# MartinErhardt/RoaringRegex

Hardware: AMD Instinct MI355X
Metric: GB/s input scanned (whole job), 256-state regex (higher is better)
Workload: dtype u32

## Files before the change

include/rrx.h:

```cpp
#ifndef RRX_H
#define RRX_H
#include <stddef.h>
#include <stdint.h>
#ifdef __cplusplus
extern "C" {
#endif

typedef struct rrx_regex rrx_regex;
typedef struct rrx_corpus rrx_corpus;

enum { RRX_OK = 0, RRX_ERR_PATTERN = 1, RRX_ERR_ARG = 2, RRX_ERR_HIP = 3, RRX_ERR_UNSUPPORTED = 4 };

enum { RRX_ENGINE_AUTO = 0, RRX_ENGINE_NFA = 1, RRX_ENGINE_DFA = 2, RRX_ENGINE_DFA_GLOBAL = 3 ,
       RRX_ENGINE_NFA_WAVE = 4 ,
       RRX_ENGINE_DFA2 = 5 ,
       RRX_ENGINE_NFA_BLOCK = 8 ,
       RRX_ENGINE_NFA_SPARSE = 10  };

int rrx_compile(const char *pattern, rrx_regex **out);
int rrx_compile_ex(const char *pattern, int engine, rrx_regex **out);
void rrx_free(rrx_regex *re);
const char *rrx_last_error(void);

uint32_t rrx_num_states(const rrx_regex *re);
int      rrx_set_class(const rrx_regex *re);
uint32_t rrx_ref_initial(const rrx_regex *re);
int      rrx_ref_is_final(const rrx_regex *re, uint32_t state);
uint32_t rrx_ref_row(const rrx_regex *re, uint32_t state, unsigned c, uint32_t *out, uint32_t cap);

int         rrx_engine(const rrx_regex *re);
const char *rrx_engine_name(const rrx_regex *re);
uint32_t    rrx_useful_states(const rrx_regex *re);
uint32_t    rrx_byte_classes(const rrx_regex *re);
int         rrx_table_order(const rrx_regex *re, double *conflict_before, double *conflict_after);
int         rrx_order_table(rrx_regex *re, const void *sample, uint32_t lanes, uint32_t bytes_per_lane);
enum { RRX_OPT_BACKGROUND_ORDER = 1, RRX_OPT_UNITS_PER_WORKGROUP = 2, RRX_OPT_SAMPLED_TABLE = 3, RRX_OPT_FLUSH_SLOTS = 4, RRX_OPT_SEARCH_ANCHORED = 5,
       RRX_OPT_ITEMS_STRIDE2 = 6 };
int         rrx_set_option(rrx_regex *re, int option, int64_t value);
int         rrx_learn_table(rrx_regex *re, const void *text, size_t nbytes);
int         rrx_sampled_table(const rrx_regex *re, uint32_t *table_states, uint32_t *open_transitions);
int         rrx_sampled_escapes(const rrx_regex *re, int device, uint64_t *lines);
uint32_t    rrx_words_per_set(const rrx_regex *re);
int         rrx_accepts_empty(const rrx_regex *re);
#define RRX_PROGRAM_SEARCH_FWD 6
#define RRX_PROGRAM_SEARCH_REV 7
#define RRX_PROGRAM_DFA2_ORDER 11
#define RRX_PROGRAM_SEARCH_LINE 9
#define RRX_PROGRAM_SEARCH_LINE2 14
#define RRX_PROGRAM_SAMPLED_DFA 12
#define RRX_PROGRAM_SAMPLED_DFA2 13
#define RRX_PROGRAM_DFA2_ITEMS 15
#define RRX_PROGRAM_CONTAINS_DFA 16
#define RRX_PROGRAM_CONTAINS_DFA2 17
#define RRX_PROGRAM_CONTAINS_DFA2_ITEMS 18
size_t rrx_program_words(const rrx_regex *re, int kind, uint32_t *out, size_t cap);

int    rrx_corpus_create(int device, const void *d_bytes, size_t nbytes, void *stream, rrx_corpus **out);
int    rrx_corpus_create_ex(int device, const void *d_bytes, size_t nbytes, uint32_t stripe_bytes, void *stream,
                            rrx_corpus **out);
uint32_t rrx_corpus_stripe_bytes(const rrx_corpus *c);
size_t rrx_corpus_num_lines(const rrx_corpus *c);
size_t rrx_corpus_num_bytes(const rrx_corpus *c);
void   rrx_corpus_free(rrx_corpus *c);
size_t rrx_corpus_bitmap_words(const rrx_corpus *c);
int rrx_match_corpus(const rrx_regex *re, const rrx_corpus *c, uint32_t *d_accept_bits, void *stream);
int rrx_match_device(const rrx_regex *re, int device, const void *d_bytes, size_t nbytes, uint32_t *d_accept_bits,
                     size_t cap_words, size_t *nlines, void *stream);
int rrx_bitmap_to_bytes(int device, const uint32_t *d_accept_bits, size_t nlines, uint8_t *d_accept, void *stream);

int rrx_search_corpus(const rrx_regex *re, const rrx_corpus *corpus, uint32_t *d_start, uint32_t *d_end, void *stream);
int         rrx_contains_corpus(const rrx_regex *re, const rrx_corpus *c, uint32_t *d_bits, void *stream);
const char *rrx_contains_engine_name(const rrx_regex *re);
uint32_t    rrx_contains_states(const rrx_regex *re);
int         rrx_bitmap_count(int device, const uint32_t *d_bits, size_t nlines, uint64_t *d_count, void *stream);
int rrx_search_all_count(const rrx_regex *re, const rrx_corpus *corpus, uint32_t *d_count, void *stream);
int rrx_search_all_fill(const rrx_regex *re, const rrx_corpus *corpus, const uint64_t *d_first, uint32_t *d_start,
                        uint32_t *d_end, void *stream);

int rrx_search_all(const rrx_regex *re, const rrx_corpus *corpus, uint64_t *d_first, uint32_t *d_start, uint32_t *d_end,
                   size_t cap, size_t *total, void *stream);

int rrx_match_extents(const rrx_regex *re, int device, const void *d_bytes, const uint64_t *d_off, size_t nitems,
                      uint32_t trim, uint8_t *d_accept, void *stream);

typedef struct rrx_items rrx_items;
int rrx_items_create(int device, const void *d_bytes, const uint64_t *d_off, size_t nitems, uint32_t trim, void *stream,
                     rrx_items **out);
size_t rrx_items_count(const rrx_items *items);
int rrx_items_stripe_wise(const rrx_items *items);
void rrx_items_free(rrx_items *items);
int rrx_match_items(const rrx_regex *re, const rrx_items *items, uint8_t *d_accept, void *stream);

int rrx_contains_extents(const rrx_regex *re, int device, const void *d_bytes, const uint64_t *d_off, size_t nitems, uint32_t trim,
                         uint32_t *d_bits, void *stream);
int rrx_contains_items(const rrx_regex *re, const rrx_items *items, uint32_t *d_bits, void *stream);

int rrx_match_string(const rrx_regex *re, int device, const void *d_bytes, size_t nbytes, uint8_t *d_accept, void *stream);

int rrx_match_host(const rrx_regex *re, int device, const void *bytes, size_t nbytes, uint8_t *accept, size_t cap,
                   size_t *nlines);
int rrx_match_cstr(const rrx_regex *re, int device, const char *text, int *accepted, size_t *len);

#ifdef __cplusplus
}
#endif
#endif
```

roaringregex_amd/__init__.py:

```python
import ctypes as C
import os

_HERE = os.path.dirname(os.path.abspath(__file__))
_SO = os.environ.get("RRX_LIB") or os.path.join(_HERE, "librrx.so")

ENGINE_AUTO, ENGINE_NFA, ENGINE_DFA, ENGINE_DFA_GLOBAL, ENGINE_NFA_WAVE, ENGINE_DFA2 = 0, 1, 2, 3, 4, 5
PROGRAM_SEARCH_FWD, PROGRAM_SEARCH_REV = 6, 7
ENGINE_NFA_BLOCK = 8
ENGINE_NFA_SPARSE = 10
PROGRAM_SEARCH_LINE = 9
PROGRAM_SEARCH_LINE2 = 14
PROGRAM_DFA2_ITEMS = 15
PROGRAM_DFA2_ORDER = 11
PROGRAM_SAMPLED_DFA = 12
PROGRAM_SAMPLED_DFA2 = 13
PROGRAM_CONTAINS_DFA, PROGRAM_CONTAINS_DFA2 = 16, 17
PROGRAM_CONTAINS_DFA2_ITEMS = 18
OPT_BACKGROUND_ORDER = 1
OPT_UNITS_PER_WORKGROUP = 2
OPT_SAMPLED_TABLE = 3
OPT_FLUSH_SLOTS = 4
OPT_SEARCH_ANCHORED = 5
OPT_ITEMS_STRIDE2 = 6

ABI_SYMBOLS = (
    "rrx_compile", "rrx_compile_ex", "rrx_free", "rrx_last_error",
    "rrx_num_states", "rrx_set_class", "rrx_ref_initial", "rrx_ref_is_final", "rrx_ref_row",
    "rrx_engine", "rrx_engine_name", "rrx_useful_states", "rrx_byte_classes", "rrx_table_order", "rrx_order_table", "rrx_set_option", "rrx_learn_table", "rrx_sampled_table", "rrx_sampled_escapes", "rrx_words_per_set", "rrx_accepts_empty",
    "rrx_program_words",
    "rrx_corpus_create", "rrx_corpus_create_ex", "rrx_corpus_stripe_bytes", "rrx_corpus_num_lines", "rrx_corpus_num_bytes", "rrx_corpus_free", "rrx_corpus_bitmap_words",
    "rrx_match_corpus", "rrx_match_device", "rrx_search_corpus", "rrx_search_all_count", "rrx_search_all_fill", "rrx_search_all", "rrx_bitmap_to_bytes",
    "rrx_match_extents", "rrx_items_create", "rrx_items_count", "rrx_items_stripe_wise", "rrx_items_free", "rrx_match_items",
    "rrx_match_string", "rrx_match_host", "rrx_match_cstr",
    "rrx_contains_corpus", "rrx_contains_engine_name", "rrx_contains_states", "rrx_bitmap_count",
    "rrx_contains_extents", "rrx_contains_items",
)


class RRegexError(RuntimeError):
    """The reference throws std::runtime_error (Parser.cpp:36,155); so do we."""


def _load():
    if not os.path.exists(_SO):
        raise ImportError(
            "roaringregex_amd: %s is missing — build it with `python -c 'import __graft_entry__ as g; g.build()'` "
            "(hipcc --offload-arch=gfx950).  There is no CPU fallback." % _SO)
    try:
        import torch
    except ImportError:
        pass
    L = C.CDLL(_SO)
    vp, u32, sz, i32 = C.c_void_p, C.c_uint32, C.c_size_t, C.c_int
    sig = {
        "rrx_compile": (i32, [C.c_char_p, C.POINTER(vp)]),
        "rrx_compile_ex": (i32, [C.c_char_p, i32, C.POINTER(vp)]),
        "rrx_free": (None, [vp]),
        "rrx_last_error": (C.c_char_p, []),
        "rrx_num_states": (u32, [vp]),
        "rrx_set_class": (i32, [vp]),
        "rrx_ref_initial": (u32, [vp]),
        "rrx_ref_is_final": (i32, [vp, u32]),
        "rrx_ref_row": (u32, [vp, u32, C.c_uint, vp, u32]),
        "rrx_engine": (i32, [vp]),
        "rrx_engine_name": (C.c_char_p, [vp]),
        "rrx_useful_states": (u32, [vp]),
        "rrx_byte_classes": (u32, [vp]),
        "rrx_table_order": (i32, [vp, C.POINTER(C.c_double), C.POINTER(C.c_double)]),
        "rrx_set_option": (i32, [vp, i32, C.c_int64]),
        "rrx_learn_table": (i32, [vp, vp, C.c_size_t]),
        "rrx_sampled_table": (i32, [vp, C.POINTER(C.c_uint32), C.POINTER(C.c_uint32)]),
        "rrx_sampled_escapes": (i32, [vp, i32, C.POINTER(C.c_uint64)]),
        "rrx_order_table": (i32, [vp, vp, u32, u32]),
        "rrx_words_per_set": (u32, [vp]),
        "rrx_accepts_empty": (i32, [vp]),
        "rrx_program_words": (sz, [vp, i32, vp, sz]),
        "rrx_corpus_create": (i32, [i32, vp, sz, vp, C.POINTER(vp)]),
        "rrx_corpus_create_ex": (i32, [i32, vp, sz, u32, vp, C.POINTER(vp)]),
        "rrx_corpus_stripe_bytes": (u32, [vp]),
        "rrx_corpus_num_lines": (sz, [vp]),
        "rrx_corpus_num_bytes": (sz, [vp]),
        "rrx_corpus_free": (None, [vp]),
        "rrx_corpus_bitmap_words": (sz, [vp]),
        "rrx_match_corpus": (i32, [vp, vp, vp, vp]),
        "rrx_match_device": (i32, [vp, i32, vp, sz, vp, sz, C.POINTER(sz), vp]),
        "rrx_bitmap_to_bytes": (i32, [i32, vp, sz, vp, vp]),
        "rrx_match_extents": (i32, [vp, i32, vp, vp, sz, u32, vp, vp]),
        "rrx_items_create": (i32, [i32, vp, vp, sz, u32, vp, C.POINTER(vp)]),
        "rrx_items_count": (sz, [vp]),
        "rrx_items_stripe_wise": (i32, [vp]),
        "rrx_items_free": (None, [vp]),
        "rrx_match_items": (i32, [vp, vp, vp, vp]),
        "rrx_match_string": (i32, [vp, i32, vp, sz, vp, vp]),
        "rrx_search_corpus": (i32, [vp, vp, vp, vp, vp]),
        "rrx_search_all_count": (i32, [vp, vp, vp, vp]),
        "rrx_search_all_fill": (i32, [vp, vp, vp, vp, vp, vp]),
        "rrx_search_all": (i32, [vp, vp, vp, vp, vp, sz, C.POINTER(sz), vp]),
        "rrx_match_host": (i32, [vp, i32, vp, sz, vp, sz, C.POINTER(sz)]),
        "rrx_match_cstr": (i32, [vp, i32, C.c_char_p, C.POINTER(i32), C.POINTER(sz)]),
        "rrx_contains_corpus": (i32, [vp, vp, vp, vp]),
        "rrx_contains_engine_name": (C.c_char_p, [vp]),
        "rrx_contains_states": (u32, [vp]),
        "rrx_bitmap_count": (i32, [i32, vp, sz, vp, vp]),
        "rrx_contains_extents": (i32, [vp, i32, vp, vp, sz, u32, vp, vp]),
        "rrx_contains_items": (i32, [vp, vp, vp, vp]),
    }
    for name, (res, args) in sig.items():
        f = getattr(L, name)
        f.restype, f.argtypes = res, args
    return L


_L = _load()


def _check(rc):
    if rc != 0:
        raise RRegexError(_L.rrx_last_error().decode("latin-1"))


class _on:

    def __init__(self, device, stream):
        import torch
        self._dev = torch.cuda.device(device)
        self._st = torch.cuda.stream(stream) if stream is not None else None

    def __enter__(self):
        self._dev.__enter__()
        if self._st is not None:
            self._st.__enter__()

    def __exit__(self, *exc):
        if self._st is not None:
            self._st.__exit__(*exc)
        return self._dev.__exit__(*exc)


def _stream_ptr(stream):
    if stream is None:
        import torch
        stream = torch.cuda.current_stream()
    return C.c_void_p(stream.cuda_stream)


def bitmap_count(bits, nlines, stream=None):
    import torch
    assert bits.is_cuda and bits.dtype in (torch.int32, torch.uint32) and bits.is_contiguous() and bits.numel() * 32 >= nlines
    with _on(bits.device.index, stream):
        count = torch.empty(1, dtype=torch.int64, device=bits.device)
        _check(_L.rrx_bitmap_count(bits.device.index, C.c_void_p(bits.data_ptr() if nlines else 0), nlines, C.c_void_p(count.data_ptr()),
                                   _stream_ptr(stream)))
        return int(count.item())


class Match:

    def __init__(self, buf, start, end):
        self._buf, self.start, self.end = buf, start, end

    def str(self):
        return self._buf[self.start:self.end]


class IteratorWrapper:

    def __init__(self, regex, text, device):
        self._re, self._text, self._device = regex, text, device
        self._consumed = False
        self._accepted = None

    def advance(self):
        if not self._consumed:
            acc, n = C.c_int(0), C.c_size_t(0)
            _check(_L.rrx_match_cstr(self._re._h, self._device, self._text, C.byref(acc), C.byref(n)))
            self._accepted, self._len = bool(acc.value), n.value
            self._consumed = True
        return self

    def value(self):
        if not self._consumed:
            return Match(self._text, 0, 0) if self._re.accepts_empty else None
        return Match(self._text, 0, self._len) if self._accepted else None

    def create_copy(self):
        c = IteratorWrapper(self._re, self._text, self._device)
        c.__dict__.update(self.__dict__)
        return c


class Corpus:

    def __init__(self, data, device=None, stream=None, stripe=0):
        import torch
        if isinstance(data, (bytes, bytearray, memoryview)):
            data = torch.frombuffer(bytearray(data), dtype=torch.uint8) if len(data) else torch.empty(0, dtype=torch.uint8)
        if not data.is_cuda:
            dev = torch.device("cuda", 0 if device is None else device)
            data = data.to(dev)
        assert data.dtype == torch.uint8 and data.is_contiguous()
        self.data = data
        self.device = data.device.index
        self._h = C.c_void_p()
        with _on(self.device, stream):
            _check(_L.rrx_corpus_create_ex(self.device, C.c_void_p(data.data_ptr() if data.numel() else 0), data.numel(),
                                           stripe, _stream_ptr(stream), C.byref(self._h)))

    def __del__(self):
        if getattr(self, "_h", None) and _L is not None:
            _L.rrx_corpus_free(self._h)
            self._h = None

    @property
    def num_lines(self):
        return _L.rrx_corpus_num_lines(self._h)

    @property
    def num_bytes(self):
        return _L.rrx_corpus_num_bytes(self._h)

    @property
    def stripe(self):
        return _L.rrx_corpus_stripe_bytes(self._h)


class Items:

    def __init__(self, data, offsets, trim=0, stream=None):
        import torch
        assert data.is_cuda and data.dtype == torch.uint8 and data.is_contiguous()
        assert offsets.is_cuda and offsets.dtype in (torch.int64, torch.uint64) and offsets.is_contiguous() and offsets.numel() >= 1
        self.data, self.offsets, self.trim = data, offsets, trim
        self.device = data.device.index
        self._h = C.c_void_p()
        with _on(self.device, stream):
            _check(_L.rrx_items_create(self.device, C.c_void_p(data.data_ptr() if data.numel() else 0), C.c_void_p(offsets.data_ptr()),
                                       offsets.numel() - 1, trim, _stream_ptr(stream), C.byref(self._h)))

    def __del__(self):
        if getattr(self, "_h", None) and _L is not None:
            _L.rrx_items_free(self._h)
            self._h = None

    @property
    def num_items(self):
        return _L.rrx_items_count(self._h)

    @property
    def stripe_wise(self):
        return bool(_L.rrx_items_stripe_wise(self._h))


class RRegex:

    def __init__(self, pattern, engine=ENGINE_AUTO, device=0):
        if isinstance(pattern, str):
            pattern = pattern.encode("latin-1")
        self.pattern = pattern
        self.device = device
        self._h = C.c_void_p()
        _check(_L.rrx_compile_ex(pattern, engine, C.byref(self._h)))

    def __del__(self):
        if getattr(self, "_h", None) and _L is not None:
            _L.rrx_free(self._h)
            self._h = None

    def get_acceptance_iter(self, text):
        if isinstance(text, str):
            text = text.encode("latin-1")
        return IteratorWrapper(self, text, self.device)

    def match_corpus_bits(self, corpus, out=None, stream=None):
        import torch
        nw = _L.rrx_corpus_bitmap_words(corpus._h)
        with _on(corpus.device, stream):
            if out is None:
                out = torch.empty(nw, dtype=torch.int32, device=corpus.data.device)
            assert out.is_cuda and out.dtype == torch.int32 and out.numel() >= nw
            _check(_L.rrx_match_corpus(self._h, corpus._h, C.c_void_p(out.data_ptr() if nw else 0), _stream_ptr(stream)))
        return out[:nw]

    def match_device_bits(self, data, cap_lines=None, out=None, stream=None):
        import torch
        assert data.is_cuda and data.dtype == torch.uint8 and data.is_contiguous()
        n = data.numel()
        if cap_lines is None:
            cap_lines = n + 1
        cap_words = (cap_lines + 31) // 32
        with _on(data.device.index, stream):
            if out is None:
                out = torch.empty(cap_words, dtype=torch.int32, device=data.device)
            assert out.is_cuda and out.dtype == torch.int32 and out.numel() >= cap_words
            nlines = C.c_size_t(0)
            _check(_L.rrx_match_device(self._h, data.device.index, C.c_void_p(data.data_ptr() if n else 0), n,
                                       C.c_void_p(out.data_ptr()), cap_words, C.byref(nlines), _stream_ptr(stream)))
        return out[:(nlines.value + 31) // 32], nlines.value

    def match_corpus(self, corpus, out=None, stream=None):
        import torch
        n = corpus.num_lines
        with _on(corpus.device, stream):
            bits = self.match_corpus_bits(corpus, stream=stream)
            if out is None:
                out = torch.empty(n, dtype=torch.uint8, device=corpus.data.device)
            assert out.is_cuda and out.dtype == torch.uint8 and out.numel() >= n
            _check(_L.rrx_bitmap_to_bytes(corpus.device, C.c_void_p(bits.data_ptr() if n else 0), n,
                                          C.c_void_p(out.data_ptr() if n else 0), _stream_ptr(stream)))
        return out[:n]

    def contains_corpus_bits(self, corpus, out=None, stream=None):
        import torch
        nw = _L.rrx_corpus_bitmap_words(corpus._h)
        with _on(corpus.device, stream):
            if out is None:
                out = torch.empty(nw, dtype=torch.int32, device=corpus.data.device)
            assert out.is_cuda and out.dtype == torch.int32 and out.numel() >= nw
            _check(_L.rrx_contains_corpus(self._h, corpus._h, C.c_void_p(out.data_ptr() if nw else 0), _stream_ptr(stream)))
        return out[:nw]

    def contains_corpus(self, corpus, out=None, stream=None):
        import torch
        n = corpus.num_lines
        with _on(corpus.device, stream):
            bits = self.contains_corpus_bits(corpus, stream=stream)
            if out is None:
                out = torch.empty(n, dtype=torch.uint8, device=corpus.data.device)
            assert out.is_cuda and out.dtype == torch.uint8 and out.numel() >= n
            _check(_L.rrx_bitmap_to_bytes(corpus.device, C.c_void_p(bits.data_ptr() if n else 0), n,
                                          C.c_void_p(out.data_ptr() if n else 0), _stream_ptr(stream)))
        return out[:n]

    def search_corpus(self, corpus, stream=None):
        import torch
        n = corpus.num_lines
        with _on(corpus.device, stream):
            start = torch.empty(n, dtype=torch.int32, device=corpus.data.device)
            end = torch.empty(n, dtype=torch.int32, device=corpus.data.device)
            _check(_L.rrx_search_corpus(self._h, corpus._h, C.c_void_p(start.data_ptr() if n else 0), C.c_void_p(end.data_ptr() if n else 0),
                                        _stream_ptr(stream)))
        return start, end

    def search_all(self, corpus, stream=None):
        import torch
        n = corpus.num_lines
        dev = corpus.data.device
        with _on(corpus.device, stream):
            count = torch.zeros(n, dtype=torch.int32, device=dev)
            _check(_L.rrx_search_all_count(self._h, corpus._h, C.c_void_p(count.data_ptr() if n else 0), _stream_ptr(stream)))
            inclusive = torch.cumsum(count, dim=0, dtype=torch.int64)
            first = inclusive - count
            total = int(inclusive[-1].item()) if n else 0
            start = torch.empty(total, dtype=torch.int32, device=dev)
            end = torch.empty(total, dtype=torch.int32, device=dev)
            if total:
                _check(_L.rrx_search_all_fill(self._h, corpus._h, C.c_void_p(first.data_ptr()), C.c_void_p(start.data_ptr() if total else 0),
                                              C.c_void_p(end.data_ptr() if total else 0), _stream_ptr(stream)))
        return count, first, start, end

    def search_all_fused(self, corpus, cap=None, stream=None):
        import torch
        n = corpus.num_lines
        dev = corpus.data.device
        with _on(corpus.device, stream):
            first = torch.empty(n + 1, dtype=torch.int64, device=dev)
            cap = int(cap) if cap is not None else 2 * n + 1024
            while True:
                start = torch.empty(cap, dtype=torch.int32, device=dev)
                end = torch.empty(cap, dtype=torch.int32, device=dev)
                total = C.c_size_t(0)
                _check(_L.rrx_search_all(self._h, corpus._h, C.c_void_p(first.data_ptr()), C.c_void_p(start.data_ptr() if cap else 0),
                                         C.c_void_p(end.data_ptr() if cap else 0), cap, C.byref(total), _stream_ptr(stream)))
                if total.value <= cap:
                    break
                cap = total.value
        return first, start[:total.value], end[:total.value]

    def match_items(self, items, out=None, stream=None):
        import torch
        n = items.num_items
        with _on(items.device, stream):
            if out is None:
                out = torch.empty(n, dtype=torch.uint8, device=items.data.device)
            assert out.is_cuda and out.dtype == torch.uint8 and out.numel() >= n
            _check(_L.rrx_match_items(self._h, items._h, C.c_void_p(out.data_ptr() if n else 0), _stream_ptr(stream)))
        return out[:n]

    def match_extents(self, data, offsets, trim=0, out=None, stream=None):
        import torch
        n = offsets.numel() - 1
        assert data.is_cuda and offsets.is_cuda and offsets.dtype in (torch.int64, torch.uint64)
        with _on(data.device.index, stream):
            if out is None:
                out = torch.empty(n, dtype=torch.uint8, device=data.device)
            _check(_L.rrx_match_extents(self._h, data.device.index, C.c_void_p(data.data_ptr() if data.numel() else 0),
                                        C.c_void_p(offsets.data_ptr()), n, trim, C.c_void_p(out.data_ptr() if n else 0),
                                        _stream_ptr(stream)))
        return out[:n]

    def contains_items_bits(self, items, out=None, stream=None):
        import torch
        n = items.num_items
        nw = (n + 31) // 32
        with _on(items.device, stream):
            if out is None:
                out = torch.empty(nw, dtype=torch.int32, device=items.data.device)
            assert out.is_cuda and out.dtype == torch.int32 and out.is_contiguous() and out.numel() >= nw
            _check(_L.rrx_contains_items(self._h, items._h, C.c_void_p(out.data_ptr() if nw else 0), _stream_ptr(stream)))
        return out[:nw]

    def contains_items(self, items, out=None, stream=None):
        import torch
        n = items.num_items
        with _on(items.device, stream):
            bits = self.contains_items_bits(items, stream=stream)
            if out is None:
                out = torch.empty(n, dtype=torch.uint8, device=items.data.device)
            assert out.is_cuda and out.dtype == torch.uint8 and out.numel() >= n
            _check(_L.rrx_bitmap_to_bytes(items.device, C.c_void_p(bits.data_ptr() if n else 0), n,
                                          C.c_void_p(out.data_ptr() if n else 0), _stream_ptr(stream)))
        return out[:n]

    def contains_extents_bits(self, data, offsets, trim=0, out=None, stream=None):
        import torch
        n = offsets.numel() - 1
        nw = (n + 31) // 32
        assert data.is_cuda and offsets.is_cuda and offsets.dtype in (torch.int64, torch.uint64) and offsets.is_contiguous()
        with _on(data.device.index, stream):
            if out is None:
                out = torch.empty(nw, dtype=torch.int32, device=data.device)
            assert out.is_cuda and out.dtype == torch.int32 and out.is_contiguous() and out.numel() >= nw
            _check(_L.rrx_contains_extents(self._h, data.device.index, C.c_void_p(data.data_ptr() if data.numel() else 0),
                                           C.c_void_p(offsets.data_ptr()), n, trim, C.c_void_p(out.data_ptr() if nw else 0),
                                           _stream_ptr(stream)))
        return out[:nw]

    def contains_extents(self, data, offsets, trim=0, out=None, stream=None):
        import torch
        n = offsets.numel() - 1
        with _on(data.device.index, stream):
            bits = self.contains_extents_bits(data, offsets, trim=trim, stream=stream)
            if out is None:
                out = torch.empty(n, dtype=torch.uint8, device=data.device)
            assert out.is_cuda and out.dtype == torch.uint8 and out.numel() >= n
            _check(_L.rrx_bitmap_to_bytes(data.device.index, C.c_void_p(bits.data_ptr() if n else 0), n,
                                          C.c_void_p(out.data_ptr() if n else 0), _stream_ptr(stream)))
        return out[:n]

    def match_string(self, data, stream=None):
        import torch
        assert data.is_cuda and data.dtype == torch.uint8
        with _on(data.device.index, stream):
            out = torch.zeros(1, dtype=torch.uint8, device=data.device)
            _check(_L.rrx_match_string(self._h, data.device.index, C.c_void_p(data.data_ptr() if data.numel() else 0), data.numel(),
                                       C.c_void_p(out.data_ptr()), _stream_ptr(stream)))
        return bool(out.item())

    def match_host(self, data):
        import numpy as np
        a = np.frombuffer(data, dtype=np.uint8) if not isinstance(data, np.ndarray) else np.ascontiguousarray(data, dtype=np.uint8)
        cap = len(a) + 1
        out = np.empty(cap, dtype=np.uint8)
        n = C.c_size_t(0)
        _check(_L.rrx_match_host(self._h, self.device, C.c_void_p(a.ctypes.data if len(a) else 0), len(a),
                                 C.c_void_p(out.ctypes.data), cap, C.byref(n)))
        return out[:n.value]

    @property
    def states_n(self):
        return _L.rrx_num_states(self._h)

    @property
    def set_class(self):
        return _L.rrx_set_class(self._h)

    @property
    def initial(self):
        return _L.rrx_ref_initial(self._h)

    def finals(self):
        return [s for s in range(self.states_n) if _L.rrx_ref_is_final(self._h, s)]

    def row(self, state, c):
        n = self.states_n
        buf = (C.c_uint32 * max(n, 1))()
        k = _L.rrx_ref_row(self._h, state, c, buf, n)
        return list(buf[:k])

    @property
    def engine(self):
        return _L.rrx_engine(self._h)

    @property
    def engine_name(self):
        return _L.rrx_engine_name(self._h).decode()

    @property
    def contains_engine_name(self):
        name = _L.rrx_contains_engine_name(self._h)
        if name is None:
            raise RRegexError(_L.rrx_last_error().decode("latin-1"))
        return name.decode()

    @property
    def contains_states(self):
        return _L.rrx_contains_states(self._h)

    @property
    def useful_states(self):
        return _L.rrx_useful_states(self._h)

    def order_table(self, sample, lanes, bytes_per_lane):
        import numpy as np
        a = np.ascontiguousarray(sample, dtype=np.uint8)
        assert a.size >= lanes * bytes_per_lane
        _check(_L.rrx_order_table(self._h, C.c_void_p(a.ctypes.data), lanes, bytes_per_lane))
        return self.table_order

    def set_background_order(self, enabled):
        _check(_L.rrx_set_option(self._h, OPT_BACKGROUND_ORDER, 1 if enabled else 0))

    def learn_table(self, text):
        import numpy as np
        a = np.frombuffer(text, dtype=np.uint8) if isinstance(text, (bytes, bytearray)) else np.ascontiguousarray(text, dtype=np.uint8)
        _check(_L.rrx_learn_table(self._h, C.c_void_p(a.ctypes.data), a.size))
        return self.sampled_table

    def set_sampled_table(self, enabled):
        _check(_L.rrx_set_option(self._h, OPT_SAMPLED_TABLE, 1 if enabled else 0))

    @property
    def sampled_table(self):
        n, o = C.c_uint32(0), C.c_uint32(0)
        return (n.value, o.value) if _L.rrx_sampled_table(self._h, C.byref(n), C.byref(o)) == 1 else None

    def sampled_escapes(self):
        n = C.c_uint64(0)
        _check(_L.rrx_sampled_escapes(self._h, self.device, C.byref(n)))
        return n.value

    @property
    def sampled_table_pending(self):
        return _L.rrx_sampled_table(self._h, None, None) == 2

    @property
    def sampled_table_retired(self):
        return _L.rrx_sampled_table(self._h, None, None) == 3

    def set_flush_slots(self, slots):
        _check(_L.rrx_set_option(self._h, OPT_FLUSH_SLOTS, int(slots)))

    def set_search_anchored(self, enabled):
        _check(_L.rrx_set_option(self._h, OPT_SEARCH_ANCHORED, 1 if enabled else 0))

    def set_items_stride2(self, enabled):
        _check(_L.rrx_set_option(self._h, OPT_ITEMS_STRIDE2, 1 if enabled else 0))

    def set_units_per_workgroup(self, units):
        _check(_L.rrx_set_option(self._h, OPT_UNITS_PER_WORKGROUP, int(units)))

    @property
    def table_order(self):
        b, a = C.c_double(0), C.c_double(0)
        return (b.value, a.value) if _L.rrx_table_order(self._h, C.byref(b), C.byref(a)) == 1 else None

    @property
    def table_order_pending(self):
        return _L.rrx_table_order(self._h, None, None) == 2

    @property
    def byte_classes(self):
        return _L.rrx_byte_classes(self._h)

    @property
    def words_per_set(self):
        return _L.rrx_words_per_set(self._h)

    def program(self, kind):
        import numpy as np
        n = _L.rrx_program_words(self._h, kind, None, 0)
        if not n:
            return None
        out = np.zeros(n, dtype=np.uint32)
        _L.rrx_program_words(self._h, kind, C.c_void_p(out.ctypes.data), n)
        return out

    @property
    def accepts_empty(self):
        return bool(_L.rrx_accepts_empty(self._h))
```

roaringregex_amd/csrc/abi.cpp:

```cpp
#include <hip/hip_runtime.h>

#include <atomic>
#include <cstdio>
#include <cstring>
#include <map>
#include <memory>
#include <mutex>
#include <string>
#include <thread>
#include <vector>

#include "../../include/rrx.h"
#include "device.hpp"
#include "frontend.hpp"
#include "lower.hpp"
#include "pack.hpp"
#include "plan.hpp"

using namespace rrx;

namespace {

thread_local std::string g_err;

int fail(int code, const std::string &msg) { g_err = msg; return code; }
int hip_fail(hipError_t e, const char *what) {
    return fail(RRX_ERR_HIP, std::string(what) + ": " + hipGetErrorString(e));
}
int launched(int e, const char *what) { return e ? hip_fail((hipError_t)e, what) : RRX_OK; }
#define HIP_TRY(expr) do { hipError_t e_ = (expr); if (e_ != hipSuccess) return hip_fail(e_, #expr); } while (0)

struct DeviceAlloc {
    int device = -1;
    void *p = nullptr;
    DeviceAlloc() = default;
    DeviceAlloc(DeviceAlloc &&o) noexcept : device(o.device), p(o.p) { o.p = nullptr; }
    ~DeviceAlloc() { reset(); }
    void reset() { if (p) { (void)hipSetDevice(device); (void)hipFree(p); p = nullptr; } }
    hipError_t alloc(int dev, size_t bytes) {
        reset(); device = dev;
        hipError_t e = hipSetDevice(dev);
        if (e == hipSuccess && (e = hipMalloc(&p, bytes)) != hipSuccess) p = nullptr;
        return e;
    }
};

template <class D> struct OnDevice { DeviceAlloc mem; D d; };

hipError_t upload(int device, const Image &img, DeviceAlloc &out, hipStream_t stream = nullptr) {
    const std::vector<uint8_t> &b = img.bytes;
    hipError_t e = out.alloc(device, b.size() + 16);
    if (e == hipSuccess) e = stream ? hipMemcpyAsync(out.p, b.data(), b.size(), hipMemcpyHostToDevice, stream) : hipMemcpy(out.p, b.data(), b.size(), hipMemcpyHostToDevice);
    if (e == hipSuccess && stream) e = hipStreamSynchronize(stream);
    if (e == hipSuccess) img.bind(out.p); else out.reset();
    return e;
}

struct TableSet {
    const char *const word;
    LineTables own;
    LineTables &lt;
    ItemsForms items;
    uint32_t found = ~0u;
    std::map<int, OnDevice<DeviceTables>> on_device;
    std::map<int, OnDevice<dev::LineDfaDevice>> items_on_device;
    std::map<int, OnDevice<dev::Dfa2Device>> items2_on_device;
    explicit TableSet(const char *w) : word(w), lt(own) {}
    TableSet(const char *w, LineTables &of) : word(w), lt(of) {}
};

struct Mailbox {
    volatile uint64_t *host = nullptr;
    uint64_t *dev = nullptr;
    int device = -1, slot = -1;
};
constexpr int kMailSlots = 64, kMailWords = 8;
struct MailPage { uint64_t *host = nullptr, *dev = nullptr; std::vector<int> free_slots; };
std::mutex g_mail_mu;
std::map<int, MailPage> g_mail;
int mailbox_acquire(int device, Mailbox *out) {
    std::lock_guard<std::mutex> lock(g_mail_mu);
    MailPage &pg = g_mail[device];
    if (!pg.host) {
        void *h = nullptr, *d = nullptr;
        hipError_t e = hipHostMalloc(&h, kMailSlots * kMailWords * sizeof(uint64_t), hipHostMallocMapped);
        if (e == hipSuccess) e = hipHostGetDevicePointer(&d, h, 0);
        if (e != hipSuccess) { if (h) (void)hipHostFree(h); return hip_fail(e, "hipHostMalloc(mailbox)"); }
        pg.host = static_cast<uint64_t *>(h); pg.dev = static_cast<uint64_t *>(d);
        for (int i = kMailSlots - 1; i >= 0; i--) pg.free_slots.push_back(i);
    }
    if (pg.free_slots.empty()) return fail(RRX_ERR_HIP, "more than 64 synchronous calls in flight on one device");
    out->slot = pg.free_slots.back(); pg.free_slots.pop_back();
    out->device = device;
    out->host = pg.host + (size_t)out->slot * kMailWords;
    out->dev = pg.dev + (size_t)out->slot * kMailWords;
    return RRX_OK;
}
void mailbox_release(const Mailbox &m) {
    if (m.slot < 0) return;
    std::lock_guard<std::mutex> lock(g_mail_mu);
    g_mail[m.device].free_slots.push_back(m.slot);
}
struct MailboxGuard {
    Mailbox m;
    hipStream_t stream = nullptr;
    bool queued = false;
    bool drained = false;
    ~MailboxGuard() {
        if (queued && !drained && hipStreamSynchronize(stream) != hipSuccess) { (void)hipGetLastError(); return; }
        mailbox_release(m);
    }
};

}

static uint32_t absorbing_accepting_state(const DfaProgram &d) {
    uint32_t found = ~0u;
    for (uint32_t s = 0; s < d.nstates; s++) {
        if (!d.accepting[s]) continue;
        if (found != ~0u) return ~0u;
        found = s;
    }
    if (found != ~0u)
        for (uint32_t k = 0; k < d.ncls; k++)
            if (d.next[(size_t)found * d.ncls + k] != found) return ~0u;
    return found;
}

struct rrx_regex : Programs {
    std::string pattern;
    std::vector<uint32_t> t2_row_slot, t2_col_slot;
    mutable TableOrderSearch t2_order;
    mutable Dfa2OrderStats t2_order_stats;
    std::atomic<int> opt_background_order{1};
    std::atomic<int> opt_search_anchored{1};
    std::atomic<int> opt_units_per_wg{0};
    std::atomic<int> opt_sampled_table{1};
    std::atomic<int> opt_flush_slots{0};
    int requested_engine = 0;
    mutable OnceTask sampled_build;
    mutable std::atomic<bool> sampled_ready{false};
    mutable DfaProgram sampled_dfa;
    mutable Dfa2Program sampled_dfa2;
    mutable SampledTableStats sampled_stats;
    mutable std::map<int, DeviceAlloc> sampled_escapes;
    mutable unsigned long long *h_sampled_seen = nullptr;
    mutable unsigned long long sampled_prev_lines = 0;
    mutable std::atomic<bool> sampled_retired{false};
    static constexpr uint32_t kSampledRelearns = 3;
    mutable uint32_t sampled_gen = 0;
    mutable std::vector<std::unique_ptr<OnceTask>> sampled_relearn;
    mutable std::map<int, OnDevice<dev::Dfa2Device>> sampled_on_device;
    bool sampled_eligible() const { return requested_engine == RRX_ENGINE_AUTO && engine == RRX_ENGINE_NFA && !has_dfa && has_nfa; }
    bool build_sampled(const uint8_t *text, uint32_t pieces, uint32_t piece_bytes, bool replace = false) const {
        const Reduced red = reduce(trimmed);
        DfaProgram d;
        Dfa2Program d2;
        SampledTableStats st;
        bool ok = false;
        for (uint32_t budget = 2048; budget >= 64 && !ok; budget /= 2) {
            if (!lower_dfa_sampled(red, text, pieces, piece_bytes, budget, d, &st)) return false;
            ok = lower_dfa2_that_fits(d, d2);
        }
        if (!ok || d.escaped.empty()) return false;
        if (st.sample_escapes * 50 > st.sample_lines) return false;
        if (replace) {
            std::lock_guard<std::mutex> launches(onepass_mu);
            std::lock_guard<std::mutex> lock(mu);
            for (auto &kv : sampled_on_device) kept.push_back(std::move(kv.second.mem));
            sampled_on_device.clear();
            sampled_dfa = std::move(d); sampled_dfa2 = std::move(d2); sampled_stats = st;
            sampled_gen++;
            sampled_prev_lines = 0;
            sampled_retired.store(false);
            return true;
        }
        std::lock_guard<std::mutex> lock(mu);
        sampled_dfa = std::move(d); sampled_dfa2 = std::move(d2); sampled_stats = st;
        sampled_ready.store(true, std::memory_order_release);
        return true;
    }
    void relearn_sampled(const uint8_t *sample, uint32_t pieces, uint32_t piece_bytes) const {
        OnceTask *task = nullptr;
        {
            std::lock_guard<std::mutex> launches(onepass_mu);
            if (!sampled_retired.load() || sampled_relearn.size() >= kSampledRelearns) return;
            if (!sampled_relearn.empty() && sampled_relearn.back()->state() != OnceTask::kDone) return;
            sampled_relearn.emplace_back(new OnceTask());
            task = sampled_relearn.back().get();
        }
        auto text = std::make_shared<std::vector<uint8_t>>(sample, sample + (size_t)pieces * piece_bytes);
        (void)task->start([this, text, pieces, piece_bytes]() { (void)build_sampled(text->data(), pieces, piece_bytes, true); },
                          opt_background_order.load() != 0);
    }
    int sampled_tables(int device, dev::Dfa2Device *out) const {
        std::lock_guard<std::mutex> lock(mu);
        const dev::Dfa2Device *d = nullptr;
        const int rc = upload_once(sampled_on_device, device, false, [&](Image &img, dev::Dfa2Device &t) { return pack_dfa2(sampled_dfa2, {}, {}, img, t); }, &d);
        if (!rc) *out = *d;
        return rc;
    }
    mutable std::vector<DeviceAlloc> kept;
    bool t2_order_applies() const {
        return match.has_dfa2 && dfa2_table_bytes(match.dfa2) * 2 > dev::kDfa2TableBudget;
    }
    void apply_t2_order(std::vector<uint32_t> &&rows, std::vector<uint32_t> &&cols, const Dfa2OrderStats &st) const {
        std::vector<int> up;
        { std::lock_guard<std::mutex> lock(mu); for (auto &kv : match_set.on_device) up.push_back(kv.first); }
        std::vector<std::pair<int, OnDevice<dev::Dfa2Device>>> done;
        for (int device : up) {
            Image img;
            OnDevice<dev::Dfa2Device> t;
            (void)pack_dfa2(match.dfa2, rows, cols, img, t.d);
            hipStream_t st2 = nullptr;
            bool ok = hipSetDevice(device) == hipSuccess && hipStreamCreateWithFlags(&st2, hipStreamNonBlocking) == hipSuccess &&
                      upload(device, img, t.mem, st2) == hipSuccess;
            if (st2) (void)hipStreamDestroy(st2);
            if (!ok) { (void)hipGetLastError(); continue; }
            done.emplace_back(device, std::move(t));
        }
        std::lock_guard<std::mutex> lock(mu);
        rrx_regex *self = const_cast<rrx_regex *>(this);
        self->t2_row_slot.swap(rows); self->t2_col_slot.swap(cols);
        t2_order_stats = st;
        for (auto &u : done) {
            auto it = match_set.on_device.find(u.first);
            if (it != match_set.on_device.end()) it->second.d.dfa2 = u.second.d;
            kept.push_back(std::move(u.second.mem));
        }
    }
    bool decide_t2_order(const uint8_t *sample, uint32_t lanes, uint32_t bytes_per_lane, bool now) const {
        if (t2_order.decided()) return false;
        if (!t2_order_applies() || !sample || lanes < 32) return t2_order.skip();
        if (!now && !opt_background_order.load()) return true;
        std::vector<uint8_t> copy(sample, sample + (size_t)lanes * bytes_per_lane);
        return t2_order.start(match.dfa2, std::move(copy), lanes, bytes_per_lane, !now,
                              [this](std::vector<uint32_t> &&r, std::vector<uint32_t> &&c, const Dfa2OrderStats &st) { apply_t2_order(std::move(r), std::move(c), st); });
    }
    dev::Dfa2Device dfa2_device(const DeviceTables *t) const { std::lock_guard<std::mutex> lock(mu); return t->dfa2; }
    mutable std::mutex mu;
    mutable TableSet match_set{"match", match}, contains_set{"contains"};
    mutable int search_state = 0;
    mutable SearchPlan search;
    mutable std::map<int, OnDevice<dev::SearchChunkDevice>> search_on_device;
    std::atomic<int> items_stride2{1};
    struct Scratch { DeviceAlloc mem; size_t cap = 0; };
    mutable std::mutex scratch_mu;
    mutable std::map<int, Scratch> scratch;
    int scratch_for(int device, size_t bytes, void **out) const {
        Scratch &sc = scratch[device];
        if (sc.cap < bytes) {
            sc.cap = 0;
            const size_t want = bytes < 4096 ? 4096 : bytes + bytes / 4;
            hipError_t e = sc.mem.alloc(device, want);
            if (e != hipSuccess) return hip_fail(e, "hipMalloc(single-string scratch)");
            sc.cap = want;
        }
        *out = sc.mem.p;
        return RRX_OK;
    }

    struct EventScratch {
        DeviceAlloc mem; size_t cap = 0; hipEvent_t last = nullptr; bool used = false;
        ~EventScratch() { if (last) { (void)hipSetDevice(mem.device); (void)hipEventSynchronize(last); (void)hipEventDestroy(last); } }
    };
    mutable std::mutex onepass_mu;
    mutable std::map<int, EventScratch> onepass_scratch;
    int onepass_for(int device, size_t bytes, void **out, hipStream_t stream) const {
        EventScratch &sc = onepass_scratch[device];
        if (!sc.last) {
            hipError_t e = hipEventCreateWithFlags(&sc.last, hipEventDisableTiming);
            if (e != hipSuccess) { sc.last = nullptr; return hip_fail(e, "hipEventCreate(scratch)"); }
        }
        if (sc.cap < bytes) {
            if (sc.mem.p) { (void)hipEventSynchronize(sc.last); sc.mem.reset(); sc.cap = 0; sc.used = false; }
            hipError_t e = sc.mem.alloc(device, bytes);
            if (e != hipSuccess) return hip_fail(e, "hipMalloc(one-pass scratch)");
            sc.cap = bytes;
        }
        if (sc.used) {
            hipError_t e = hipStreamWaitEvent(stream, sc.last, 0);
            if (e != hipSuccess) return hip_fail(e, "hipStreamWaitEvent(scratch)");
        }
        *out = sc.mem.p;
        return RRX_OK;
    }
    int onepass_done(int device, hipStream_t stream) const {
        EventScratch &sc = onepass_scratch[device];
        hipError_t e = hipEventRecord(sc.last, stream);
        if (e != hipSuccess) return hip_fail(e, "hipEventRecord(scratch)");
        sc.used = true;
        return RRX_OK;
    }

    ~rrx_regex() {
        t2_order.wait();
        sampled_build.wait();
        for (auto &task : sampled_relearn) task->wait();
        if (h_sampled_seen) {
            for (auto &kv : sampled_escapes) { (void)hipSetDevice(kv.first); (void)hipDeviceSynchronize(); }
            (void)hipHostFree(h_sampled_seen);
        }
    }
    template <class D, class Pack> int upload_once(std::map<int, OnDevice<D>> &cache, int device, bool keep_miss, Pack pack, const D **out) const {
        auto it = cache.find(device);
        if (it == cache.end()) {
            Image img;
            OnDevice<D> t;
            const bool packed = pack(img, t.d);
            const hipError_t e = packed ? upload(device, img, t.mem) : hipSuccess;
            if (!keep_miss && !packed) return fail(RRX_ERR_UNSUPPORTED, "automaton too large for the device tables of its engine");
            if (!keep_miss && e != hipSuccess) return hip_fail(e, "device table upload");
            it = cache.emplace(device, std::move(t)).first;
        }
        *out = it->second.mem.p ? &it->second.d : nullptr;
        return RRX_OK;
    }
    bool built(const TableSet &set) const { return &set == &match_set || build_contains() == RRX_OK; }
    const dev::Dfa2Device *items2_table(TableSet &set, int device) const {
        std::lock_guard<std::mutex> lock(mu);
        const dev::Dfa2Device *d = nullptr;
        if (built(set)) (void)upload_once(set.items2_on_device, device, true, [&](Image &img, dev::Dfa2Device &t) { return set.items.pack2(set.lt, img, t); }, &d);
        return d;
    }
    const dev::LineDfaDevice *items_table(TableSet &set, int device) const {
        std::lock_guard<std::mutex> lock(mu);
        const dev::LineDfaDevice *d = nullptr;
        if (built(set)) (void)upload_once(set.items_on_device, device, true, [&](Image &img, dev::LineDfaDevice &t) { return set.items.pack(set.lt, img, t); }, &d);
        return d;
    }

    int build_search() const {
        if (search_state == 0)
            search_state = plan_search(reduce(trimmed), opt_search_anchored.load() != 0, accepts_empty(), dev::search_chunks_lds_bytes, search) ? 1 : -1;
        return search_state == 1 ? RRX_OK
                                 : fail(RRX_ERR_UNSUPPORTED, "search tables too large for the device (the reverse DFA must fit 64 KiB of LDS, the forward "
                                                              "product table 65534 rows and 256 MiB)");
    }
    int search_tables(int device, const dev::SearchChunkDevice **out) const {
        std::lock_guard<std::mutex> lock(mu);
        int rc = build_search();
        if (rc) return rc;
        *out = nullptr;
        if (search.nullable) return RRX_OK;
        auto pack = [&](Image &img, dev::SearchChunkDevice &t) { pack_search(search.line2, search.fwd, search.rev, search.layout, img, t); return true; };
        return upload_once(search_on_device, device, false, pack, out);
    }

    mutable int contains_state = 0;
    int build_contains() const {
        if (contains_state == 0) {
            (void)build_search();
            LineTables &lt = contains_set.lt;
            contains_state = search.fwd.nstates != 0 && contains_dfa(search.fwd, lt.dfa) && lt.decide(requested_engine) ? 1 : -1;
            if (contains_state == 1) contains_set.found = absorbing_accepting_state(lt.dfa);
        }
        return contains_state == 1 ? RRX_OK
                                   : fail(RRX_ERR_UNSUPPORTED, search.fwd.nstates ? "contains table too large for the device (the global form holds 2^24 entries)"
                                                                                  : "no contains table: the forward search automaton does not determinise within the state budget");
    }
    int contains_tables(int device, const DeviceTables **out) const {
        std::lock_guard<std::mutex> lock(mu);
        const int rc = build_contains();
        return rc ? rc : upload_once(contains_set.on_device, device, false, [&](Image &img, DeviceTables &t) { contains_set.lt.pack({}, {}, img, t); return true; }, out);
    }

    int tables(int device, const DeviceTables **out) const {
        std::lock_guard<std::mutex> lock(mu);
        return upload_once(match_set.on_device, device, false, [&](Image &img, DeviceTables &t) {
            if (engine == RRX_ENGINE_NFA_BLOCK || engine == RRX_ENGINE_NFA_SPARSE) {
                const bool sparse = engine == RRX_ENGINE_NFA_SPARSE;
                pack_wave_nfa(nfa_block, trimmed, sparse ? dev::sparse_rows(nfa_block.W) : dev::wave_words_per_lane(nfa_block.W), sparse, img, t.block);
            } else if (engine == RRX_ENGINE_NFA_WAVE) {
                return pack_group_nfa(nfa_wave, trimmed, img, t.group);
            } else if (engine == RRX_ENGINE_NFA) {
                pack_lane_nfa(nfa, img, t.nfa);
            } else {
                match.pack(t2_row_slot, t2_col_slot, img, t);
            }
            return true;
        }, out);
    }
};

struct rrx_corpus {
    int device = 0;
    const uint8_t *d_bytes = nullptr;
    size_t nbytes = 0, nstripes = 0, nlines = 0;
    uint32_t stripe = 0;
    uint32_t *d_counts = nullptr;
    uint64_t *d_base = nullptr;
    bool has_high = false;
    uint8_t *h_sample = nullptr;
    uint32_t sample_lanes = 0;
    mutable std::mutex mu;
    mutable uint64_t *d_line_off = nullptr;
    mutable uint64_t *d_chunk_base = nullptr;
    mutable size_t nchunks = 0;
    mutable void *d_all_scratch = nullptr;
};

static constexpr uint32_t kSampleGroups = 8, kSampleBytes = 256;
static constexpr size_t kSampleMinCorpus = (size_t)64 << 20;

static constexpr size_t kLongStringBytes = 32 * 1024;
static constexpr size_t kLongStringBytesTable = 1024;
static constexpr uint32_t kLongNfaMaxBits = 256;

extern "C" {

const char *rrx_last_error(void) { return g_err.c_str(); }

int rrx_compile_ex(const char *pattern, int engine, rrx_regex **out) {
    if (!pattern || !out) return fail(RRX_ERR_ARG, "null argument");
    if (engine < RRX_ENGINE_AUTO || (engine > RRX_ENGINE_DFA2 && engine != RRX_ENGINE_NFA_BLOCK && engine != RRX_ENGINE_NFA_SPARSE)) return fail(RRX_ERR_ARG, "unknown engine");
    *out = nullptr;
    rrx_regex *re = new rrx_regex();
    try {
        re->pattern = pattern;
        re->requested_engine = engine;
        plan_engines(re->pattern, engine, *re);
    } catch (const PatternError &e) {
        delete re;
        return fail(RRX_ERR_PATTERN, e.what());
    } catch (const BudgetError &e) {
        delete re;
        return fail(RRX_ERR_UNSUPPORTED, e.what());
    } catch (const std::exception &e) {
        delete re;
        return fail(RRX_ERR_PATTERN, std::string("internal: ") + e.what());
    }
    if (!re->engine) {
        char msg[200];
        std::snprintf(msg, sizeof msg, "automaton too large for the requested engine (%u useful states)", re->trimmed.n);
        delete re;
        return fail(RRX_ERR_UNSUPPORTED, msg);
    }
    *out = re;
    return RRX_OK;
}
int rrx_compile(const char *pattern, rrx_regex **out) { return rrx_compile_ex(pattern, RRX_ENGINE_AUTO, out); }
void rrx_free(rrx_regex *re) { delete re; }

uint32_t rrx_num_states(const rrx_regex *re) { return re->ref.states_n; }
int rrx_set_class(const rrx_regex *re) { return re->ref.set_class(); }
uint32_t rrx_ref_initial(const rrx_regex *re) { return re->ref.initial; }
int rrx_ref_is_final(const rrx_regex *re, uint32_t s) { return s < re->ref.states_n && re->ref.is_final[s]; }
uint32_t rrx_ref_row(const rrx_regex *re, uint32_t state, unsigned c, uint32_t *out, uint32_t cap) {
    std::vector<uint32_t> r = re->ref.row(state, c);
    for (size_t i = 0; i < r.size() && i < cap; i++) out[i] = r[i];
    return (uint32_t)r.size();
}
int rrx_engine(const rrx_regex *re) { return re->engine; }
const char *rrx_engine_name(const rrx_regex *re) { return re->engine_name(); }
uint32_t rrx_useful_states(const rrx_regex *re) { return re->trimmed.n; }
int rrx_order_table(rrx_regex *re, const void *sample, uint32_t lanes, uint32_t bytes_per_lane) {
    if (!re || !sample || lanes < 32 || bytes_per_lane < 2) return fail(RRX_ERR_ARG, "sample: at least 32 lanes of 2 bytes");
    if (!re->decide_t2_order(static_cast<const uint8_t *>(sample), lanes, bytes_per_lane, true))
        return fail(RRX_ERR_ARG, "the table order has been decided already");
    return RRX_OK;
}
int rrx_table_order(const rrx_regex *re, double *conflict_before, double *conflict_after) {
    const TableOrderSearch::State st = re->t2_order.state();
    std::lock_guard<std::mutex> lock(re->mu);
    const bool profiled = st == TableOrderSearch::kDone && re->t2_row_slot.size() == re->match.dfa2.nstates && re->match.has_dfa2 && re->t2_order_stats.half_waves;
    if (conflict_before) *conflict_before = profiled ? re->t2_order_stats.before : 0.0;
    if (conflict_after) *conflict_after = profiled ? re->t2_order_stats.after : 0.0;
    return profiled ? 1 : st == TableOrderSearch::kRunning ? 2 : 0;
}
int rrx_learn_table(rrx_regex *re, const void *text, size_t nbytes) {
    if (!re || !text || nbytes < 2 || nbytes > ((size_t)1 << 30)) return fail(RRX_ERR_ARG, "a text sample of 2 bytes to 1 GiB");
    if (!re->sampled_eligible()) return fail(RRX_ERR_UNSUPPORTED, "a sampled table serves automata that AUTO leaves on the NFA lane engine");
    const uint8_t *p = static_cast<const uint8_t *>(text);
    bool built = false;
    if (!re->sampled_build.start([&]() { built = re->build_sampled(p, 1, (uint32_t)nbytes); }, false))
        return fail(RRX_ERR_ARG, "the sampled table has been decided already");
    return built ? RRX_OK : fail(RRX_ERR_UNSUPPORTED, "no sampled table for this automaton and text: none fits the device, or more than 2 % of the text's own lines leave it");
}
int rrx_sampled_table(const rrx_regex *re, uint32_t *table_states, uint32_t *open_transitions) {
    const OnceTask::State st = re->sampled_build.state();
    const bool ready = re->sampled_ready.load(std::memory_order_acquire);
    std::lock_guard<std::mutex> lock(re->mu);
    if (table_states) *table_states = ready ? re->sampled_dfa.nstates : 0;
    if (open_transitions) *open_transitions = ready ? re->sampled_stats.open_transitions : 0;
    return ready ? (re->sampled_retired.load() ? 3 : 1) : st == OnceTask::kRunning ? 2 : 0;
}
int rrx_sampled_escapes(const rrx_regex *re, int device, uint64_t *lines) {
    if (!re || !lines) return fail(RRX_ERR_ARG, "null argument");
    *lines = 0;
    std::lock_guard<std::mutex> lock(re->onepass_mu);
    auto it = re->sampled_escapes.find(device);
    if (it == re->sampled_escapes.end() || !it->second.p) return RRX_OK;
    HIP_TRY(hipSetDevice(device));
    unsigned long long v = 0;
    HIP_TRY(hipMemcpy(&v, it->second.p, sizeof v, hipMemcpyDeviceToHost));
    *lines = v;
    return RRX_OK;
}
int rrx_set_option(rrx_regex *re, int option, int64_t value) {
    if (!re) return fail(RRX_ERR_ARG, "null argument");
    if (option == RRX_OPT_BACKGROUND_ORDER) { re->opt_background_order.store(value ? 1 : 0); return RRX_OK; }
    if (option == RRX_OPT_FLUSH_SLOTS) {
        if (value != 0 && value != 1 && value != 2 && value != 4 && value != 8 && value != 16 && value != 32) return fail(RRX_ERR_ARG, "flush period: 0 (automatic) or 1, 2, 4, 8, 16, 32 slots");
        re->opt_flush_slots.store((int)value);
        return RRX_OK;
    }
    if (option == RRX_OPT_SAMPLED_TABLE) { re->opt_sampled_table.store(value ? 1 : 0); return RRX_OK; }
    if (option == RRX_OPT_ITEMS_STRIDE2) { re->items_stride2.store(value ? 1 : 0); return RRX_OK; }
    if (option == RRX_OPT_SEARCH_ANCHORED) {
        std::lock_guard<std::mutex> lock(re->mu);
        if (re->search_state != 0) return fail(RRX_ERR_ARG, "the search tables of this regex are built already");
        re->opt_search_anchored.store(value ? 1 : 0);
        return RRX_OK;
    }
    if (option == RRX_OPT_UNITS_PER_WORKGROUP) {
        if (value < 0 || value > 65536) return fail(RRX_ERR_ARG, "units per workgroup: 0 (off) or 16 ... 65536");
        re->opt_units_per_wg.store(value && value < 16 ? 16 : (int)value);
        return RRX_OK;
    }
    return fail(RRX_ERR_ARG, "unknown option");
}
uint32_t rrx_byte_classes(const rrx_regex *re) { return re->trimmed.ncls; }
uint32_t rrx_words_per_set(const rrx_regex *re) { return re->has_nfa ? re->nfa.W : re->has_wave ? re->nfa_wave.W : re->has_block ? re->nfa_block.W : 0; }
int rrx_accepts_empty(const rrx_regex *re) { return re->accepts_empty(); }

size_t rrx_program_words(const rrx_regex *re, int kind, uint32_t *out, size_t cap) {
    std::vector<uint32_t> w;
    if (kind == RRX_ENGINE_NFA && re->has_nfa) {
        append_words(w, re->nfa, false);
    } else if (kind == RRX_ENGINE_NFA_WAVE && re->has_wave) {
        append_words(w, re->nfa_wave, false);
    } else if ((kind == RRX_ENGINE_NFA_BLOCK || kind == RRX_ENGINE_NFA_SPARSE) && re->has_block) {
        append_words(w, re->nfa_block, true);
    } else if (kind == RRX_PROGRAM_SEARCH_LINE || kind == RRX_PROGRAM_SEARCH_LINE2 || kind == RRX_PROGRAM_SEARCH_FWD || kind == RRX_PROGRAM_SEARCH_REV) {
        std::lock_guard<std::mutex> lock(re->mu);
        if (re->build_search()) return 0;
        const SearchPlan &s = re->search;
        if (kind == RRX_PROGRAM_SEARCH_FWD) append_words(w, s.fwd);
        else if (kind == RRX_PROGRAM_SEARCH_REV) append_words(w, s.rev);
        else if (kind == RRX_PROGRAM_SEARCH_LINE && s.line.nrows) append_words(w, s.line, s.fwd);
        else if (kind == RRX_PROGRAM_SEARCH_LINE2 && s.line2.nrows) append_words(w, s.line2, s.layout);
    } else if (kind == RRX_PROGRAM_CONTAINS_DFA || kind == RRX_PROGRAM_CONTAINS_DFA2) {
        std::lock_guard<std::mutex> lock(re->mu);
        if (re->build_contains()) return 0;
        if (kind == RRX_PROGRAM_CONTAINS_DFA) append_words(w, re->contains_set.lt.dfa);
        else if (re->contains_set.lt.has_dfa2) append_words(w, re->contains_set.lt.dfa2);
    } else if (kind == RRX_PROGRAM_CONTAINS_DFA2_ITEMS || (kind == RRX_PROGRAM_DFA2_ITEMS && re->match.has_dfa2)) {
        TableSet &set = kind == RRX_PROGRAM_DFA2_ITEMS ? re->match_set : re->contains_set;
        std::lock_guard<std::mutex> lock(re->mu);
        if (re->built(set) && set.items.stride2(set.lt)) append_words(w, set.items.dfa2, true);
    } else if (kind == RRX_PROGRAM_DFA2_ORDER && re->match.has_dfa2) {
        std::lock_guard<std::mutex> lock(re->mu);
        if (re->t2_row_slot.size() != re->match.dfa2.nstates || re->t2_col_slot.size() != re->match.dfa2.ncols) return 0;
        w = {re->match.dfa2.nstates, re->match.dfa2.ncols};
        w.insert(w.end(), re->t2_row_slot.begin(), re->t2_row_slot.end());
        w.insert(w.end(), re->t2_col_slot.begin(), re->t2_col_slot.end());
    } else if (kind == RRX_PROGRAM_SAMPLED_DFA || kind == RRX_PROGRAM_SAMPLED_DFA2) {
        if (!re->sampled_ready.load(std::memory_order_acquire)) return 0;
        std::lock_guard<std::mutex> lock(re->mu);
        if (kind == RRX_PROGRAM_SAMPLED_DFA) append_words(w, re->sampled_dfa, true);
        else append_words(w, re->sampled_dfa2);
    } else if (kind == RRX_ENGINE_DFA2 && re->match.has_dfa2) {
        append_words(w, re->match.dfa2);
    } else if (kind == RRX_ENGINE_DFA && re->has_dfa) {
        append_words(w, re->match.dfa);
    }
    for (size_t i = 0; i < w.size() && i < cap; i++) out[i] = w[i];
    return w.size();
}

int rrx_corpus_create(int device, const void *d_bytes, size_t nbytes, void *stream, rrx_corpus **out) {
    return rrx_corpus_create_ex(device, d_bytes, nbytes, 0, stream, out);
}

int rrx_corpus_create_ex(int device, const void *d_bytes, size_t nbytes, uint32_t stripe_bytes, void *stream, rrx_corpus **out) {
    if (!out || (nbytes && !d_bytes)) return fail(RRX_ERR_ARG, "null argument");
    if (stripe_bytes && (stripe_bytes < dev::kMinStripe || stripe_bytes > dev::kMaxStripe || (stripe_bytes & (stripe_bytes - 1))))
        return fail(RRX_ERR_ARG, "stripe must be a power of two in [1024, 16384]");
    if (reinterpret_cast<uintptr_t>(d_bytes) & 15) return fail(RRX_ERR_ARG, "corpus base must be 16-byte aligned");
    *out = nullptr;
    HIP_TRY(hipSetDevice(device));
    rrx_corpus *c = new rrx_corpus();
    c->device = device;
    c->d_bytes = static_cast<const uint8_t *>(d_bytes);
    c->nbytes = nbytes;
    c->stripe = stripe_bytes ? stripe_bytes : dev::pick_stripe(nbytes);
    constexpr size_t kSample = (size_t)4 << 20;
    if (!stripe_bytes && nbytes >= 16 * kSample) {
        rrx_corpus *sample = nullptr;
        if (rrx_corpus_create_ex(device, d_bytes, kSample, dev::pick_stripe(kSample), stream, &sample) == RRX_OK && sample) {
            if (sample->nlines) c->stripe = dev::stripe_for_lines(nbytes, kSample / sample->nlines);
            rrx_corpus_free(sample);
        }
    }
    c->nstripes = (nbytes + c->stripe - 1) / c->stripe;
    hipError_t e = hipMalloc(reinterpret_cast<void **>(&c->d_counts), (c->nstripes + 1) * sizeof(uint32_t));
    if (e == hipSuccess) e = hipMalloc(reinterpret_cast<void **>(&c->d_base), (c->nstripes + 1 + dev::scan_scratch_words(c->nstripes)) * sizeof(uint64_t));
    if (e != hipSuccess) { rrx_corpus_free(c); return hip_fail(e, "hipMalloc(line index)"); }
    uint32_t *d_flags = c->d_counts + c->nstripes;
    e = hipMemsetAsync(d_flags, 0, sizeof(uint32_t), (hipStream_t)stream);
    if (e != hipSuccess) { rrx_corpus_free(c); return hip_fail(e, "hipMemsetAsync(flags)"); }
    int rc = dev::count_newlines_per_stripe(c->d_bytes, nbytes, c->stripe, c->d_counts, c->nstripes, d_flags, stream);
    if (!rc) rc = dev::scan_counts(c->d_counts, c->d_base, c->d_base + c->nstripes + 1, c->nstripes, stream);
    if (rc) { rrx_corpus_free(c); return hip_fail((hipError_t)rc, "line index launch"); }
    MailboxGuard mail;
    if (int mrc = mailbox_acquire(device, &mail.m)) { rrx_corpus_free(c); return mrc; }
    if (nbytes >= kSampleMinCorpus && c->nstripes >= 64 * kSampleGroups &&
        hipHostMalloc(reinterpret_cast<void **>(&c->h_sample), (size_t)kSampleGroups * 32 * kSampleBytes, hipHostMallocDefault) == hipSuccess) {
        c->sample_lanes = kSampleGroups * 32;
        for (uint32_t g = 0; g < kSampleGroups; g++) {
            const size_t first_stripe = (size_t)g * (c->nstripes / kSampleGroups);
            if (hipMemcpy2DAsync(c->h_sample + (size_t)g * 32 * kSampleBytes, kSampleBytes, c->d_bytes + first_stripe * c->stripe, c->stripe,
                                 kSampleBytes, 32, hipMemcpyDeviceToHost, (hipStream_t)stream) != hipSuccess) {
                (void)hipGetLastError();
                (void)hipStreamSynchronize((hipStream_t)stream);
                (void)hipHostFree(c->h_sample); c->h_sample = nullptr; c->sample_lanes = 0;
                break;
            }
        }
    }
    mail.stream = (hipStream_t)stream; mail.queued = true;
    rc = dev::mail_results(c->d_base + c->nstripes, d_flags, nbytes ? c->d_bytes + nbytes - 1 : nullptr, mail.m.dev, stream);
    if (rc) { rrx_corpus_free(c); return hip_fail((hipError_t)rc, "line index launch"); }
    e = hipStreamSynchronize((hipStream_t)stream);
    if (e != hipSuccess) { rrx_corpus_free(c); return hip_fail(e, "line index readback"); }
    mail.drained = true;
    const uint64_t total = mail.m.host[0];
    const uint32_t flags = (uint32_t)mail.m.host[1];
    const uint8_t last = nbytes ? (uint8_t)mail.m.host[2] : (uint8_t)'\n';
    c->has_high = (flags & 1u) != 0;
    c->nlines = (size_t)total + ((nbytes && last != '\n') ? 1 : 0);
    if (!stripe_bytes && c->nlines) {
        const uint32_t want = dev::stripe_for_lines(nbytes, nbytes / c->nlines);
        if (want != c->stripe) {
            rrx_corpus_free(c);
            return rrx_corpus_create_ex(device, d_bytes, nbytes, want, stream, out);
        }
    }
    *out = c;
    return RRX_OK;
}
size_t rrx_corpus_num_lines(const rrx_corpus *c) { return c->nlines; }
size_t rrx_corpus_num_bytes(const rrx_corpus *c) { return c->nbytes; }
uint32_t rrx_corpus_stripe_bytes(const rrx_corpus *c) { return c->stripe; }
void rrx_corpus_free(rrx_corpus *c) {
    if (!c) return;
    (void)hipSetDevice(c->device);
    if (c->d_counts) (void)hipFree(c->d_counts);
    if (c->d_base) (void)hipFree(c->d_base);
    if (c->d_line_off) (void)hipFree(c->d_line_off);
    if (c->d_chunk_base && c->d_chunk_base != c->d_base) (void)hipFree(c->d_chunk_base);
    if (c->d_all_scratch) (void)hipFree(c->d_all_scratch);
    if (c->h_sample) (void)hipHostFree(c->h_sample);
    delete c;
}

size_t rrx_corpus_bitmap_words(const rrx_corpus *c) { return (c->nlines + 31) / 32; }

static int match_corpus_sampled(const rrx_regex *re, const rrx_corpus *c, const DeviceTables *t, uint32_t *d_accept_bits, void *stream) {
    dev::Dfa2Device d2;
    int rc = re->sampled_tables(c->device, &d2);
    if (rc) return rc;
    hipStream_t st = (hipStream_t)stream;
    const size_t words = rrx_corpus_bitmap_words(c);
    const size_t wide_bytes = (2 * words * sizeof(uint32_t) + 15) & ~(size_t)15, esc_bytes = (words * sizeof(uint32_t) + 15) & ~(size_t)15;
    const size_t cap = std::max<size_t>(words / 2, 1024);
    std::lock_guard<std::mutex> lock(re->onepass_mu);
    void *buf = nullptr;
    rc = re->onepass_for(c->device, wide_bytes + esc_bytes + cap * sizeof(uint64_t), &buf, st);
    if (rc) return rc;
    uint32_t *wide = static_cast<uint32_t *>(buf);
    uint32_t *escaped = reinterpret_cast<uint32_t *>(static_cast<uint8_t *>(buf) + wide_bytes);
    uint64_t *list = reinterpret_cast<uint64_t *>(static_cast<uint8_t *>(buf) + wide_bytes + esc_bytes);
    DeviceAlloc &count = re->sampled_escapes[c->device];
    if (!count.p) HIP_TRY(count.alloc(c->device, 16));
    unsigned long long *total = static_cast<unsigned long long *>(count.p);
    constexpr uint32_t kSlots = rrx_regex::kSampledRelearns + 1;
    if (!re->h_sampled_seen && hipHostMalloc(reinterpret_cast<void **>(&re->h_sampled_seen), kSlots * sizeof(unsigned long long), hipHostMallocDefault) == hipSuccess)
        for (uint32_t k = 0; k < kSlots; k++) re->h_sampled_seen[k] = 0;
    unsigned long long *const seen = re->h_sampled_seen ? re->h_sampled_seen + (re->sampled_gen < kSlots ? re->sampled_gen : kSlots - 1) : nullptr;
    if (seen) {
        const unsigned long long esc_seen = seen[0];
        if (re->sampled_prev_lines >= 1024 && esc_seen * 20 > re->sampled_prev_lines) re->sampled_retired.store(true);
    }
    hipError_t he = hipMemsetAsync(wide, 0, wide_bytes, st);
    if (he == hipSuccess) he = hipMemsetAsync(total, 0, 16, st);
    int e = he != hipSuccess ? (int)he : dev::match_stripes_dfa2_two_bit(d2, c->d_bytes, c->nbytes, c->stripe, c->d_base, c->nstripes, wide, stream);
    if (!e) e = dev::split_two_bit(wide, c->nlines, d_accept_bits, escaped, total, list, cap, stream);
    if (!e) e = dev::recheck_escaped_nfa(t->nfa, c->d_bytes, c->nbytes, c->stripe, c->d_base, c->nstripes, escaped, c->nlines, list, total, cap, d_accept_bits, stream);
    if (!e && seen) {
        if (hipMemcpyAsync(seen, total, sizeof(unsigned long long), hipMemcpyDeviceToHost, st) != hipSuccess) (void)hipGetLastError();
        re->sampled_prev_lines = c->nlines;
    }
    const int rc2 = re->onepass_done(c->device, st);
    if (e) return hip_fail((hipError_t)e, "sampled-table launch");
    return rc2;
}

static int launch_line_tables(const rrx_regex *re, const rrx_corpus *c, const LineTables &lt, const DeviceTables *t, bool stride2_over_high, uint32_t *bits,
                              void *stream) {
    if (!lt.has_dfa2 || (c->has_high && !stride2_over_high)) return dev::match_stripes_dfa(t->line, c->has_high, c->d_bytes, c->nbytes, c->stripe, c->d_base, c->nstripes, bits, stream);
    const dev::Dfa2Device d2 = re->dfa2_device(t);
    const uint32_t flush_mask = re->opt_flush_slots.load() ? (uint32_t)re->opt_flush_slots.load() - 1u : dev::flush_mask_for(c->nbytes, c->nlines);
    return (c->has_high ? dev::match_stripes_dfa2_clean : dev::match_stripes_dfa2)(d2, c->d_bytes, c->nbytes, c->stripe, c->d_base, c->nstripes, bits, stream, flush_mask);
}

int rrx_match_corpus(const rrx_regex *re, const rrx_corpus *c, uint32_t *d_accept_bits, void *stream) {
    if (!re || !c || (c->nlines && !d_accept_bits)) return fail(RRX_ERR_ARG, "null argument");
    if (!re->t2_order.decided() && c->h_sample && !c->has_high) (void)re->decide_t2_order(c->h_sample, c->sample_lanes, kSampleBytes, false);
    const DeviceTables *t;
    int rc = re->tables(c->device, &t);
    if (rc) return rc;
    HIP_TRY(hipSetDevice(c->device));
    if (!c->nlines) return RRX_OK;
    if (re->sampled_eligible() && re->opt_sampled_table.load() && !c->has_high) {
        if (!re->sampled_build.decided() && c->h_sample) {
            auto text = std::make_shared<std::vector<uint8_t>>(c->h_sample, c->h_sample + (size_t)c->sample_lanes * kSampleBytes);
            const uint32_t pieces = c->sample_lanes;
            (void)re->sampled_build.start([re, text, pieces]() { (void)re->build_sampled(text->data(), pieces, kSampleBytes); },
                                          re->opt_background_order.load() != 0);
        }
        if (re->sampled_ready.load(std::memory_order_acquire) && re->sampled_retired.load() && c->h_sample)
            re->relearn_sampled(c->h_sample, c->sample_lanes, kSampleBytes);
        if (re->sampled_ready.load(std::memory_order_acquire) && !re->sampled_retired.load()) return match_corpus_sampled(re, c, t, d_accept_bits, stream);
    }
    HIP_TRY(hipMemsetAsync(d_accept_bits, 0, rrx_corpus_bitmap_words(c) * sizeof(uint32_t), (hipStream_t)stream));
    int e = re->engine == RRX_ENGINE_NFA_SPARSE
                ? dev::match_stripes_sparse_nfa(t->block, c->d_bytes, c->nbytes, c->stripe, c->d_base, c->nstripes, d_accept_bits, stream)
            : re->engine == RRX_ENGINE_NFA_BLOCK
                ? dev::match_stripes_wave_nfa(t->block, c->d_bytes, c->nbytes, c->stripe, c->d_base, c->nstripes, d_accept_bits, stream)
            : re->engine == RRX_ENGINE_NFA_WAVE
                ? dev::match_stripes_group_nfa(t->group, c->d_bytes, c->nbytes, c->stripe, c->d_base, c->nstripes, d_accept_bits, stream)
            : re->engine == RRX_ENGINE_NFA
                ? dev::match_stripes_nfa(t->nfa, c->d_bytes, c->nbytes, c->stripe, c->d_base, c->nstripes, d_accept_bits, stream)
            : (re->match.has_dfa2 && !c->has_high && re->opt_units_per_wg.load())
                ? dev::match_units_dfa2(re->dfa2_device(t), c->d_bytes, c->nbytes, c->stripe, c->d_base, c->nstripes, d_accept_bits, (uint32_t)re->opt_units_per_wg.load(), stream)
                : launch_line_tables(re, c, re->match, t, false, d_accept_bits, stream);
    return launched(e, "match_stripes launch");
}

int rrx_contains_corpus(const rrx_regex *re, const rrx_corpus *c, uint32_t *d_bits, void *stream) {
    if (!re || !c || (c->nlines && !d_bits)) return fail(RRX_ERR_ARG, "null argument");
    const DeviceTables *t;
    int rc = re->contains_tables(c->device, &t);
    if (rc) return rc;
    HIP_TRY(hipSetDevice(c->device));
    if (!c->nlines) return RRX_OK;
    HIP_TRY(hipMemsetAsync(d_bits, 0, rrx_corpus_bitmap_words(c) * sizeof(uint32_t), (hipStream_t)stream));
    return launched(launch_line_tables(re, c, re->contains_set.lt, t, true, d_bits, stream), "contains launch");
}
const char *rrx_contains_engine_name(const rrx_regex *re) {
    if (!re) { (void)fail(RRX_ERR_ARG, "null argument"); return nullptr; }
    std::lock_guard<std::mutex> lock(re->mu);
    return re->build_contains() ? nullptr : re->contains_set.lt.name();
}
uint32_t rrx_contains_states(const rrx_regex *re) {
    if (!re) { (void)fail(RRX_ERR_ARG, "null argument"); return 0; }
    std::lock_guard<std::mutex> lock(re->mu);
    return re->build_contains() ? 0 : re->contains_set.lt.dfa.nstates;
}
int rrx_bitmap_count(int device, const uint32_t *d_bits, size_t nlines, uint64_t *d_count, void *stream) {
    if (!d_count || (nlines && !d_bits)) return fail(RRX_ERR_ARG, "null argument");
    HIP_TRY(hipSetDevice(device));
    static_assert(sizeof(unsigned long long) == sizeof(uint64_t), "64-bit atomics");
    return launched(dev::bitmap_count(d_bits, nlines, reinterpret_cast<unsigned long long *>(d_count), stream), "bitmap_count launch");
}

int rrx_match_device(const rrx_regex *re, int device, const void *d_bytes, size_t nbytes, uint32_t *d_accept_bits, size_t cap_words,
                     size_t *nlines, void *stream) {
    if (!re || (nbytes && !d_bytes) || !nlines || (cap_words && !d_accept_bits)) return fail(RRX_ERR_ARG, "null argument");
    if (reinterpret_cast<uintptr_t>(d_bytes) & 15) return fail(RRX_ERR_ARG, "corpus base must be 16-byte aligned");
    *nlines = 0;
    HIP_TRY(hipSetDevice(device));
    if (!nbytes) return RRX_OK;
    hipStream_t st = static_cast<hipStream_t>(stream);
    const bool sampled = re->sampled_eligible() && re->opt_sampled_table.load() && re->sampled_ready.load(std::memory_order_acquire) && !re->sampled_retired.load();
    if ((re->engine != RRX_ENGINE_DFA && re->engine != RRX_ENGINE_NFA) || sampled) {
        rrx_corpus *c = nullptr;
        int rc = rrx_corpus_create(device, d_bytes, nbytes, stream, &c);
        if (rc) return rc;
        *nlines = c->nlines;
        if (rrx_corpus_bitmap_words(c) > cap_words) rc = fail(RRX_ERR_ARG, "accept bitmap too small for the number of strings");
        if (!rc) rc = rrx_match_corpus(re, c, d_accept_bits, stream);
        const hipError_t e = hipStreamSynchronize(st);
        if (!rc && e != hipSuccess) rc = hip_fail(e, "match_device");
        rrx_corpus_free(c);
        return rc;
    }
    const DeviceTables *t;
    int rc = re->tables(device, &t);
    if (rc) return rc;
    const uint8_t *bytes = static_cast<const uint8_t *>(d_bytes);
    const uint32_t stripe = dev::pick_stripe(nbytes);
    const size_t nstripes = (nbytes + stripe - 1) / stripe;
    const size_t counts_bytes = ((nstripes + 2) * sizeof(uint32_t) + 15) & ~(size_t)15;
    const size_t base_bytes = (nstripes + 1 + dev::scan_scratch_words(nstripes)) * sizeof(uint64_t);
    const size_t slab_bytes = dev::onepass_slab_words(nstripes, stripe) * sizeof(uint32_t);
    std::lock_guard<std::mutex> lock(re->onepass_mu);
    void *buf = nullptr;
    rc = re->onepass_for(device, counts_bytes + base_bytes + slab_bytes, &buf, st);
    if (rc) return rc;
    uint32_t *d_counts = static_cast<uint32_t *>(buf);
    uint64_t *d_base = reinterpret_cast<uint64_t *>(static_cast<uint8_t *>(buf) + counts_bytes);
    uint32_t *d_slabs = reinterpret_cast<uint32_t *>(static_cast<uint8_t *>(buf) + counts_bytes + base_bytes);
    MailboxGuard mail;
    rc = mailbox_acquire(device, &mail.m);
    if (rc) return rc;
    if (cap_words) HIP_TRY(hipMemsetAsync(d_accept_bits, 0, cap_words * sizeof(uint32_t), st));
    int e = re->engine == RRX_ENGINE_NFA ? dev::match_onepass_nfa(t->nfa, bytes, nbytes, stripe, nstripes, d_counts, d_slabs, stream)
            : re->match.has_dfa2         ? dev::match_onepass_dfa2(re->dfa2_device(t), bytes, nbytes, stripe, nstripes, d_counts, d_slabs, stream)
                                         : dev::match_onepass_dfa(t->line, bytes, nbytes, stripe, nstripes, d_counts, d_slabs, stream);
    if (!e) e = dev::scan_counts(d_counts, d_base, d_base + nstripes + 1, nstripes, stream);
    if (!e) e = dev::compact_streams(d_counts, d_base, nstripes, stripe, d_slabs, d_accept_bits, cap_words, stream);
    mail.stream = st; mail.queued = true;
    if (!e) e = dev::mail_results(d_base + nstripes, nullptr, bytes + nbytes - 1, mail.m.dev, stream);
    if (e) return hip_fail((hipError_t)e, "one-pass launch");
    const hipError_t he = hipStreamSynchronize(st);
    if (he != hipSuccess) return hip_fail(he, "one-pass readback");
    mail.drained = true;
    *nlines = (size_t)mail.m.host[0] + ((uint8_t)mail.m.host[2] != '\n' ? 1 : 0);
    if ((*nlines + 31) / 32 > cap_words) return fail(RRX_ERR_ARG, "accept bitmap too small for the number of strings");
    return RRX_OK;
}

static int line_offsets(const rrx_corpus *c, void *stream) {
    {
        std::lock_guard<std::mutex> lock(c->mu);
        if (!c->d_line_off) {
            uint64_t *off = nullptr;
            HIP_TRY(hipMalloc(reinterpret_cast<void **>(&off), (c->nlines + 1) * sizeof(uint64_t)));
            const uint64_t past = (uint64_t)c->nbytes + 1;
            hipError_t he = hipMemcpyAsync(off + c->nlines, &past, sizeof past, hipMemcpyHostToDevice, (hipStream_t)stream);
            if (he == hipSuccess) he = hipStreamSynchronize((hipStream_t)stream);
            int le = he == hipSuccess ? dev::build_line_offsets(c->d_bytes, c->nbytes, c->stripe, c->d_base, c->nstripes, off, stream) : 0;
            if (he == hipSuccess && !le) he = hipStreamSynchronize((hipStream_t)stream);
            if (he != hipSuccess || le) { (void)hipFree(off); return he != hipSuccess ? hip_fail(he, "line offsets") : hip_fail((hipError_t)le, "line_offsets launch"); }
            c->d_line_off = off;
        }
    }
    return RRX_OK;
}

static int chunk_index(const rrx_corpus *c, void *stream) {
    std::lock_guard<std::mutex> lock(c->mu);
    if (c->d_chunk_base) return RRX_OK;
    const size_t chunk = dev::search_chunk_bytes();
    c->nchunks = (c->nbytes + chunk - 1) / chunk;
    if (c->stripe == chunk) { c->d_chunk_base = c->d_base; return RRX_OK; }
    uint32_t *counts = nullptr;
    uint64_t *base = nullptr;
    hipError_t e = hipMalloc(reinterpret_cast<void **>(&counts), (c->nchunks + 1) * sizeof(uint32_t));
    if (e == hipSuccess) e = hipMalloc(reinterpret_cast<void **>(&base), (c->nchunks + 1 + dev::scan_scratch_words(c->nchunks)) * sizeof(uint64_t));
    if (e == hipSuccess) e = hipMemsetAsync(counts + c->nchunks, 0, sizeof(uint32_t), (hipStream_t)stream);
    int le = 0;
    if (e == hipSuccess) le = dev::count_newlines_per_stripe(c->d_bytes, c->nbytes, (uint32_t)chunk, counts, c->nchunks, counts + c->nchunks, stream);
    if (e == hipSuccess && !le) le = dev::scan_counts(counts, base, base + c->nchunks + 1, c->nchunks, stream);
    if (e == hipSuccess && !le) e = hipStreamSynchronize((hipStream_t)stream);
    if (counts) (void)hipFree(counts);
    if (e != hipSuccess || le) { if (base) (void)hipFree(base); return e != hipSuccess ? hip_fail(e, "search chunk index") : hip_fail((hipError_t)le, "search chunk index launch"); }
    c->d_chunk_base = base;
    return RRX_OK;
}

static int search_begin(const rrx_regex *re, const rrx_corpus *c, void *stream, const dev::SearchChunkDevice **ct) {
    const int rc = re->search_tables(c->device, ct);
    if (rc) return rc;
    HIP_TRY(hipSetDevice(c->device));
    return c->nlines && *ct ? chunk_index(c, stream) : RRX_OK;
}

int rrx_search_corpus(const rrx_regex *re, const rrx_corpus *c, uint32_t *d_start, uint32_t *d_end, void *stream) {
    if (!re || !c || (c->nlines && (!d_start || !d_end))) return fail(RRX_ERR_ARG, "null argument");
    const dev::SearchChunkDevice *ct;
    int rc = search_begin(re, c, stream, &ct);
    if (rc || !c->nlines) return rc;
    if (!ct) {
        HIP_TRY(hipMemsetAsync(d_start, 0, c->nlines * sizeof(uint32_t), (hipStream_t)stream));
        HIP_TRY(hipMemsetAsync(d_end, 0, c->nlines * sizeof(uint32_t), (hipStream_t)stream));
        return RRX_OK;
    }
    return launched(dev::search_chunks(*ct, c->has_high, c->d_bytes, c->nbytes, c->d_chunk_base, c->nchunks, c->nlines, d_start, d_end, stream), "search_chunks launch");
}

int rrx_search_all_count(const rrx_regex *re, const rrx_corpus *c, uint32_t *d_count, void *stream) {
    if (!re || !c || (c->nlines && !d_count)) return fail(RRX_ERR_ARG, "null argument");
    const dev::SearchChunkDevice *ct;
    int rc = search_begin(re, c, stream, &ct);
    if (rc || !c->nlines) return rc;
    if (!ct) {
        rc = line_offsets(c, stream);
        if (rc) return rc;
        return launched(dev::empty_matches(c->d_line_off, c->nlines, d_count, nullptr, nullptr, nullptr, stream), "empty_matches launch");
    }
    return launched(dev::search_chunks_count(*ct, c->has_high, c->d_bytes, c->nbytes, c->d_chunk_base, c->nchunks, d_count, stream), "search_chunks_count launch");
}

int rrx_search_all_fill(const rrx_regex *re, const rrx_corpus *c, const uint64_t *d_first, uint32_t *d_start, uint32_t *d_end, void *stream) {
    if (!re || !c || (c->nlines && (!d_first || !d_start || !d_end))) return fail(RRX_ERR_ARG, "null argument");
    const dev::SearchChunkDevice *ct;
    int rc = search_begin(re, c, stream, &ct);
    if (rc || !c->nlines) return rc;
    if (!ct) {
        rc = line_offsets(c, stream);
        if (rc) return rc;
        return launched(dev::empty_matches(c->d_line_off, c->nlines, nullptr, d_first, d_start, d_end, stream), "empty_matches launch");
    }
    return launched(dev::search_chunks_fill(*ct, c->has_high, c->d_bytes, c->nbytes, c->d_chunk_base, c->nchunks, d_first, d_start, d_end, stream), "search_chunks_fill launch");
}

int rrx_search_all(const rrx_regex *re, const rrx_corpus *c, uint64_t *d_first, uint32_t *d_start, uint32_t *d_end, size_t cap, size_t *total,
                   void *stream) {
    if (!re || !c || !total || !d_first || (cap && (!d_start || !d_end))) return fail(RRX_ERR_ARG, "null argument");
    *total = 0;
    const dev::SearchChunkDevice *ct;
    int rc = search_begin(re, c, stream, &ct);
    if (rc) return rc;
    hipStream_t st = (hipStream_t)stream;
    if (!c->nlines) { HIP_TRY(hipMemsetAsync(d_first, 0, sizeof(uint64_t), st)); HIP_TRY(hipStreamSynchronize(st)); return RRX_OK; }
    if (ct) {
        const size_t sb = dev::search_all_scratch_bytes(c->nchunks);
        {
            std::lock_guard<std::mutex> lock(c->mu);
            if (!c->d_all_scratch) HIP_TRY(hipMalloc(&c->d_all_scratch, sb));
        }
        HIP_TRY(hipMemsetAsync(c->d_all_scratch, 0, sb, st));
        int e = dev::search_chunks_all(*ct, c->has_high, c->d_bytes, c->nbytes, c->d_chunk_base, c->nchunks, c->nlines, d_first, d_start, d_end, cap,
                                       c->d_all_scratch, stream);
        if (e) return hip_fail((hipError_t)e, "search_chunks_all launch");
        uint64_t tail[2] = {0, 0};
        HIP_TRY(hipMemcpyAsync(tail, static_cast<uint8_t *>(c->d_all_scratch) + c->nchunks * sizeof(uint64_t), sizeof tail, hipMemcpyDeviceToHost, st));
        HIP_TRY(hipStreamSynchronize(st));
        if (tail[1] >> 32) return fail(RRX_ERR_HIP, "search_all: a chunk's match count was never published (look-back gave up)");
        *total = (size_t)tail[0];
        return RRX_OK;
    }
    rc = line_offsets(c, stream);
    if (rc) return rc;
    uint32_t *d_count = nullptr;
    HIP_TRY(hipMalloc(reinterpret_cast<void **>(&d_count), (c->nlines + 1) * sizeof(uint32_t)));
    uint64_t *d_sums = nullptr;
    hipError_t he = hipMalloc(reinterpret_cast<void **>(&d_sums), dev::scan_scratch_words(c->nlines) * sizeof(uint64_t));
    if (he != hipSuccess) { (void)hipFree(d_count); return hip_fail(he, "hipMalloc"); }
    auto done = [&](int code) { (void)hipFree(d_count); (void)hipFree(d_sums); return code; };
    int e = dev::empty_matches(c->d_line_off, c->nlines, d_count, nullptr, nullptr, nullptr, stream);
    if (!e) e = dev::scan_counts(d_count, d_first, d_sums, c->nlines, stream);
    if (e) return done(hip_fail((hipError_t)e, "empty_matches / scan launch"));
    he = hipMemsetAsync(d_first, 0, sizeof(uint64_t), st);
    uint64_t tot = 0;
    if (he == hipSuccess) he = hipMemcpyAsync(&tot, d_first + c->nlines, sizeof tot, hipMemcpyDeviceToHost, st);
    if (he == hipSuccess) he = hipStreamSynchronize(st);
    if (he != hipSuccess) return done(hip_fail(he, "search_all scan"));
    *total = (size_t)tot;
    if (tot && cap) {
        e = dev::empty_matches(c->d_line_off, c->nlines, nullptr, d_first, d_start, d_end, stream, cap);
        if (e) rc = hip_fail((hipError_t)e, "empty_matches launch");
        if (!rc) { he = hipStreamSynchronize(st); if (he != hipSuccess) rc = hip_fail(he, "search_all fill"); }
    }
    return done(rc);
}

int rrx_bitmap_to_bytes(int device, const uint32_t *d_bits, size_t nlines, uint8_t *d_accept, void *stream) {
    if (nlines && (!d_bits || !d_accept)) return fail(RRX_ERR_ARG, "null argument");
    if (reinterpret_cast<uintptr_t>(d_accept) & 15) return fail(RRX_ERR_ARG, "byte buffer must be 16-byte aligned");
    HIP_TRY(hipSetDevice(device));
    return launched(dev::expand_bits(d_bits, nlines, d_accept, stream), "expand_bits launch");
}

static constexpr size_t kItemsStripesMin = (size_t)1 << 16;
static constexpr size_t kItemsStripesMinBytes = (size_t)8 << 20;
static int extents_lanes(const rrx_regex *re, const TableSet &set, const DeviceTables *t, const uint8_t *b, const uint64_t *d_off, size_t nitems,
                         uint32_t trim, dev::ItemVerdicts out, void *stream, const uint32_t *only_if = nullptr) {
    int e = &set == &re->contains_set ? dev::contains_extents_dfa(t->dfa, set.lt.global, set.found, b, d_off, nitems, trim, out.bits, stream, only_if)
            : re->engine == RRX_ENGINE_NFA_SPARSE ? dev::match_extents_sparse_nfa(t->block, b, d_off, nitems, trim, out.bytes, stream)
            : re->engine == RRX_ENGINE_NFA_BLOCK ? dev::match_extents_wave_nfa(t->block, b, d_off, nitems, trim, out.bytes, stream)
            : re->engine == RRX_ENGINE_NFA_WAVE ? dev::match_extents_group_nfa(t->group, b, d_off, nitems, trim, out.bytes, stream)
            : re->engine == RRX_ENGINE_NFA ? dev::match_extents_nfa(t->nfa, b, d_off, nitems, trim, out.bytes, stream)
                                         : dev::match_extents_dfa(t->dfa, b, d_off, nitems, trim, out.bytes, stream, only_if);
    return e ? hip_fail((hipError_t)e, (std::string(set.word) + "_extents launch").c_str()) : RRX_OK;
}
struct ItemsTable { const dev::LineDfaDevice *items1 = nullptr; const dev::Dfa2Device *items2 = nullptr; };
static ItemsTable pick_items_table(const rrx_regex *re, TableSet &set, int device, uint32_t trim) {
    ItemsTable t;
    if (trim == 1 && re->items_stride2.load()) t.items2 = re->items2_table(set, device);
    if (!t.items2) t.items1 = re->items_table(set, device);
    return t;
}
static int items_extent_bound(const void *d_bytes, const uint64_t *d_off, size_t nitems, void *stream, size_t *out) {
    size_t bound = 0;
    hipDeviceptr_t abase = nullptr;
    size_t asize = 0;
    if (hipMemGetAddressRange(&abase, &asize, const_cast<void *>(d_bytes)) == hipSuccess && abase)
        bound = (size_t)(static_cast<const uint8_t *>(abase) + asize - static_cast<const uint8_t *>(d_bytes));
    else (void)hipGetLastError();
    const size_t plausible = std::max<size_t>(nitems * 128, (size_t)16 << 20);
    if (!bound || bound > plausible) {
        uint64_t first = 0, last = 0;
        HIP_TRY(hipMemcpyAsync(&first, d_off, sizeof first, hipMemcpyDeviceToHost, (hipStream_t)stream));
        HIP_TRY(hipMemcpyAsync(&last, d_off + nitems, sizeof last, hipMemcpyDeviceToHost, (hipStream_t)stream));
        HIP_TRY(hipStreamSynchronize((hipStream_t)stream));
        const size_t extent = last > first ? (size_t)last : 0;
        bound = bound ? std::min(bound, extent) : extent;
    }
    *out = bound;
    return RRX_OK;
}
static int extents_batch(const rrx_regex *re, TableSet &set, const DeviceTables *t, int device, const void *d_bytes, const uint64_t *d_off, size_t nitems,
                         uint32_t trim, bool stripes_ok, dev::ItemVerdicts out, void *stream) {
    const uint8_t *b = static_cast<const uint8_t *>(d_bytes);
    ItemsTable it;
    if (stripes_ok && trim <= 1 && nitems >= kItemsStripesMin) it = pick_items_table(re, set, device, trim);
    const bool items = it.items1 || it.items2;
    size_t bound = 0;
    if (items) {
        const int rc = items_extent_bound(d_bytes, d_off, nitems, stream, &bound);
        if (rc) return rc;
    }
    if (!items || bound < kItemsStripesMinBytes) return extents_lanes(re, set, t, b, d_off, nitems, trim, out, stream);
    hipStream_t st = (hipStream_t)stream;
    std::lock_guard<std::mutex> lock(re->onepass_mu);
    void *buf = nullptr;
    const size_t ib = dev::items_index_bytes(bound, nitems);
    int rc = re->onepass_for(device, ib + dev::items_result_bytes(nitems), &buf, st);
    if (rc) return rc;
    uint32_t *d_flag = nullptr;
    int le = dev::items_index_build(bound, d_off, nitems, trim, buf, &d_flag, stream, b, kItemsStripesMinBytes);
    if (!le) le = it.items2 ? dev::items_match2(*it.items2, b, bound, nitems, buf, static_cast<uint8_t *>(buf) + ib, out, stream, d_off, d_flag)
                            : dev::items_match(*it.items1, b, bound, nitems, trim, buf, static_cast<uint8_t *>(buf) + ib, out, stream, d_off, d_flag);
    if (!le) rc = extents_lanes(re, set, t, b, d_off, nitems, trim, out, stream, d_flag);
    const int rc2 = re->onepass_done(device, st);
    if (le) return hip_fail((hipError_t)le, (std::string(set.word) + "_items_stripes launch").c_str());
    return rc ? rc : rc2;
}
static bool match_stripes_ok(const rrx_regex *re, const uint8_t *d_accept) { return re->engine == RRX_ENGINE_DFA && !(reinterpret_cast<uintptr_t>(d_accept) & 15); }
int rrx_match_extents(const rrx_regex *re, int device, const void *d_bytes, const uint64_t *d_off, size_t nitems, uint32_t trim,
                      uint8_t *d_accept, void *stream) {
    if (!re || (nitems && (!d_off || !d_accept))) return fail(RRX_ERR_ARG, "null argument");
    const DeviceTables *t;
    int rc = re->tables(device, &t);
    if (rc) return rc;
    HIP_TRY(hipSetDevice(device));
    return extents_batch(re, re->match_set, t, device, d_bytes, d_off, nitems, trim, match_stripes_ok(re, d_accept), d_accept, stream);
}

struct rrx_items {
    int device = 0;
    const uint8_t *d_bytes = nullptr;
    const uint64_t *d_off = nullptr;
    size_t nitems = 0, nbytes = 0;
    uint64_t first = 0;
    uint32_t trim = 0;
    bool stripes = false;
    DeviceAlloc d_index;
    mutable std::mutex mu;
    DeviceAlloc d_result;
};
int rrx_items_create(int device, const void *d_bytes, const uint64_t *d_off, size_t nitems, uint32_t trim, void *stream, rrx_items **out) {
    if (!out || (nitems && (!d_bytes || !d_off))) return fail(RRX_ERR_ARG, "null argument");
    *out = nullptr;
    HIP_TRY(hipSetDevice(device));
    std::unique_ptr<rrx_items> it(new rrx_items());
    it->device = device; it->d_bytes = static_cast<const uint8_t *>(d_bytes); it->d_off = d_off; it->nitems = nitems; it->trim = trim;
    hipStream_t st = (hipStream_t)stream;
    if (nitems && trim <= 1) {
        uint64_t first = 0, last = 0;
        hipError_t e = hipMemcpyAsync(&first, d_off, sizeof first, hipMemcpyDeviceToHost, st);
        if (e == hipSuccess) e = hipMemcpyAsync(&last, d_off + nitems, sizeof last, hipMemcpyDeviceToHost, st);
        if (e == hipSuccess) e = hipStreamSynchronize(st);
        if (e != hipSuccess) return hip_fail(e, "items offsets readback");
        it->first = first;
        if (last > first && !(reinterpret_cast<uintptr_t>(it->d_bytes + first) & 15)) {
            it->nbytes = (size_t)(last - first);
            e = it->d_index.alloc(device, dev::items_index_bytes(it->nbytes, nitems));
            if (e == hipSuccess) e = it->d_result.alloc(device, dev::items_result_bytes(nitems));
            if (e != hipSuccess) return hip_fail(e, "hipMalloc(items index)");
            uint32_t *d_flag = nullptr;
            int le = dev::items_index_build(it->nbytes, d_off, nitems, trim, it->d_index.p, &d_flag, stream);
            uint32_t degenerate = 1;
            if (!le) { e = hipMemcpyAsync(&degenerate, d_flag, sizeof degenerate, hipMemcpyDeviceToHost, st); if (e == hipSuccess) e = hipStreamSynchronize(st); }
            if (le || e != hipSuccess) return le ? hip_fail((hipError_t)le, "items index launch") : hip_fail(e, "items index");
            it->stripes = degenerate == 0;
        }
    }
    *out = it.release();
    return RRX_OK;
}
size_t rrx_items_count(const rrx_items *it) { return it ? it->nitems : 0; }
int rrx_items_stripe_wise(const rrx_items *it) { return it && it->stripes ? 1 : 0; }
void rrx_items_free(rrx_items *it) { delete it; }

static int items_batch(const rrx_regex *re, TableSet &set, const DeviceTables *t, const rrx_items *it, bool stripes_ok, dev::ItemVerdicts out, void *stream) {
    const ItemsTable tab = it->stripes && stripes_ok ? pick_items_table(re, set, it->device, it->trim) : ItemsTable();
    if (!tab.items1 && !tab.items2) return extents_lanes(re, set, t, it->d_bytes, it->d_off, it->nitems, it->trim, out, stream);
    std::lock_guard<std::mutex> lock(it->mu);
    const int le = tab.items2 ? dev::items_match2(*tab.items2, it->d_bytes + it->first, it->nbytes, it->nitems, it->d_index.p, it->d_result.p, out, stream)
                              : dev::items_match(*tab.items1, it->d_bytes + it->first, it->nbytes, it->nitems, it->trim, it->d_index.p, it->d_result.p, out, stream);
    return le ? hip_fail((hipError_t)le, (std::string(set.word) + "_items launch").c_str()) : RRX_OK;
}
int rrx_match_items(const rrx_regex *re, const rrx_items *it, uint8_t *d_accept, void *stream) {
    if (!re || !it || (it->nitems && !d_accept)) return fail(RRX_ERR_ARG, "null argument");
    if (!it->nitems) return RRX_OK;
    const DeviceTables *t;
    int rc = re->tables(it->device, &t);
    if (rc) return rc;
    HIP_TRY(hipSetDevice(it->device));
    return items_batch(re, re->match_set, t, it, match_stripes_ok(re, d_accept), d_accept, stream);
}

int rrx_contains_extents(const rrx_regex *re, int device, const void *d_bytes, const uint64_t *d_off, size_t nitems, uint32_t trim,
                         uint32_t *d_bits, void *stream) {
    if (!re || (nitems && (!d_off || !d_bits))) return fail(RRX_ERR_ARG, "null argument");
    const DeviceTables *t;
    int rc = re->contains_tables(device, &t);
    if (rc) return rc;
    HIP_TRY(hipSetDevice(device));
    if (!nitems) return RRX_OK;
    return extents_batch(re, re->contains_set, t, device, d_bytes, d_off, nitems, trim, true, d_bits, stream);
}
int rrx_contains_items(const rrx_regex *re, const rrx_items *it, uint32_t *d_bits, void *stream) {
    if (!re || !it || (it->nitems && !d_bits)) return fail(RRX_ERR_ARG, "null argument");
    const DeviceTables *t;
    int rc = re->contains_tables(it->device, &t);
    if (rc) return rc;
    HIP_TRY(hipSetDevice(it->device));
    if (!it->nitems) return RRX_OK;
    return items_batch(re, re->contains_set, t, it, true, d_bits, stream);
}

struct LongStringPlan {
    enum Kind { kOneItem, kLongDfa, kLongNfa } kind = kOneItem;
    uint32_t chunk = 0, nchunks = 0;
    size_t scratch_bytes = 2 * sizeof(uint64_t);
};
static LongStringPlan long_string_plan(const rrx_regex *re, const DeviceTables *t, size_t nbytes) {
    LongStringPlan p;
    if (re->engine == RRX_ENGINE_DFA && nbytes >= kLongStringBytesTable && t->dfa.nstates && t->dfa.nstates <= dev::kLongMaxStates) {
        p.kind = LongStringPlan::kLongDfa;
        p.scratch_bytes = dev::long_scratch_bytes(t->dfa.nstates, nbytes, &p.chunk);
    } else if (re->engine == RRX_ENGINE_NFA && nbytes >= kLongStringBytes && t->nfa.nbits <= kLongNfaMaxBits) {
        p.kind = LongStringPlan::kLongNfa;
        p.scratch_bytes = dev::long_nfa_scratch_bytes(t->nfa, nbytes, &p.chunk, &p.nchunks);
    }
    return p;
}
static int match_string_with(const rrx_regex *re, int device, const DeviceTables *t, const LongStringPlan &plan, const uint8_t *d_bytes, size_t nbytes,
                             uint8_t *d_accept, uint8_t *scratch, hipStream_t st) {
    if (plan.kind == LongStringPlan::kLongDfa) {
        return launched(dev::match_long_dfa(t->dfa, d_bytes, nbytes, plan.chunk, scratch, d_accept, st), "match_long launch");
    }
    if (plan.kind == LongStringPlan::kLongNfa) {
        return launched(dev::match_long_nfa(t->nfa, d_bytes, nbytes, plan.chunk, plan.nchunks, scratch, d_accept, st), "match_long_nfa launch");
    }
    const uint64_t off[2] = {0, nbytes};
    uint64_t *d_off = reinterpret_cast<uint64_t *>(scratch);
    hipError_t e = hipMemcpyAsync(d_off, off, sizeof off, hipMemcpyHostToDevice, st);
    if (e == hipSuccess) e = hipStreamSynchronize(st);
    if (e != hipSuccess) return hip_fail(e, "extent upload");
    return rrx_match_extents(re, device, d_bytes, d_off, 1, 0, d_accept, st);
}

int rrx_match_string(const rrx_regex *re, int device, const void *d_bytes, size_t nbytes, uint8_t *d_accept, void *stream) {
    if (!re || (nbytes && !d_bytes) || !d_accept) return fail(RRX_ERR_ARG, "null argument");
    const DeviceTables *t;
    int rc = re->tables(device, &t);
    if (rc) return rc;
    HIP_TRY(hipSetDevice(device));
    std::lock_guard<std::mutex> lock(re->scratch_mu);
    void *scratch = nullptr;
    const LongStringPlan plan = long_string_plan(re, t, nbytes);
    rc = re->scratch_for(device, plan.scratch_bytes, &scratch);
    if (rc) return rc;
    rc = match_string_with(re, device, t, plan, static_cast<const uint8_t *>(d_bytes), nbytes, d_accept, static_cast<uint8_t *>(scratch),
                           static_cast<hipStream_t>(stream));
    const hipError_t e = hipStreamSynchronize(static_cast<hipStream_t>(stream));
    if (!rc && e != hipSuccess) rc = hip_fail(e, "match_string");
    return rc;
}

static int match_host_chunk(const rrx_regex *re, int device, uint8_t *d_text, size_t len, hipStream_t st, uint32_t *d_bits,
                            uint8_t *d_acc, uint8_t *accept, size_t cap, size_t line_off, size_t *nlines_out) {
    rrx_corpus *c = nullptr;
    int rc = rrx_corpus_create(device, d_text, len, st, &c);
    if (rc) return rc;
    const size_t n = c->nlines;
    rc = rrx_match_corpus(re, c, d_bits, st);
    if (!rc) rc = rrx_bitmap_to_bytes(device, d_bits, n, d_acc, st);
    if (!rc && line_off < cap) {
        const size_t take = n < cap - line_off ? n : cap - line_off;
        hipError_t e = hipMemcpyAsync(accept + line_off, d_acc, take, hipMemcpyDeviceToHost, st);
        if (e != hipSuccess) rc = hip_fail(e, "accept readback");
    }
    hipError_t e = hipStreamSynchronize(st);
    if (!rc && e != hipSuccess) rc = hip_fail(e, "chunk sync");
    rrx_corpus_free(c);
    *nlines_out = n;
    return rc;
}

int rrx_match_host(const rrx_regex *re, int device, const void *bytes, size_t nbytes, uint8_t *accept, size_t cap, size_t *nlines) {
    if (!re || (nbytes && !bytes) || !nlines) return fail(RRX_ERR_ARG, "null argument");
    HIP_TRY(hipSetDevice(device));
    *nlines = 0;
    if (!nbytes) return RRX_OK;
    const uint8_t *host = static_cast<const uint8_t *>(bytes);
    const size_t kChunk = (size_t)256 << 20;
    const size_t buf_bytes = (nbytes < kChunk ? nbytes : kChunk) + 64;
    const size_t max_lines = buf_bytes;
    uint8_t *d_text[2] = {nullptr, nullptr}, *d_acc[2] = {nullptr, nullptr};
    uint32_t *d_bits[2] = {nullptr, nullptr};
    hipStream_t st[2] = {nullptr, nullptr};
    const int nbuf = nbytes > kChunk ? 2 : 1;
    int rc = RRX_OK;
    hipError_t e = hipSuccess;
    for (int i = 0; i < nbuf && e == hipSuccess; i++) {
        e = hipMalloc(reinterpret_cast<void **>(&d_text[i]), buf_bytes);
        if (e == hipSuccess) e = hipMalloc(reinterpret_cast<void **>(&d_acc[i]), max_lines + 64);
        if (e == hipSuccess) e = hipMalloc(reinterpret_cast<void **>(&d_bits[i]), (max_lines / 32 + 4) * sizeof(uint32_t));
        if (e == hipSuccess) e = hipStreamCreate(&st[i]);
    }
    if (e != hipSuccess) rc = hip_fail(e, "pipeline buffers");

    std::vector<size_t> cuts{0};
    while (!rc && cuts.back() < nbytes) {
        size_t lo = cuts.back(), hi = lo + kChunk < nbytes ? lo + kChunk : nbytes;
        if (hi < nbytes) {
            size_t q = hi;
            while (q > lo && host[q - 1] != '\n') q--;
            if (q == lo) { rc = fail(RRX_ERR_UNSUPPORTED, "a single line longer than 256 MiB: use rrx_corpus_create on a device buffer"); break; }
            hi = q;
        }
        cuts.push_back(hi);
    }
    const size_t nchunks = cuts.size() - 1;
    size_t line_off = 0;
    if (!rc) {
        e = hipMemcpyAsync(d_text[0], host, cuts[1] - cuts[0], hipMemcpyHostToDevice, st[0]);
        if (e != hipSuccess) rc = hip_fail(e, "chunk upload");
    }
    for (size_t i = 0; i < nchunks && !rc; i++) {
        const int cur = (int)(i & 1) % nbuf, nxt = (int)((i + 1) & 1) % nbuf;
        if (i + 1 < nchunks) {
            e = hipMemcpyAsync(d_text[nxt], host + cuts[i + 1], cuts[i + 2] - cuts[i + 1], hipMemcpyHostToDevice, st[nxt]);
            if (e != hipSuccess) { rc = hip_fail(e, "chunk upload"); break; }
        }
        size_t n = 0;
        rc = match_host_chunk(re, device, d_text[cur], cuts[i + 1] - cuts[i], st[cur], d_bits[cur], d_acc[cur], accept, cap, line_off, &n);
        line_off += n;
    }
    for (int i = 0; i < nbuf; i++) if (st[i]) (void)hipStreamSynchronize(st[i]);
    for (int i = 0; i < 2; i++) {
        if (d_text[i]) (void)hipFree(d_text[i]);
        if (d_acc[i]) (void)hipFree(d_acc[i]);
        if (d_bits[i]) (void)hipFree(d_bits[i]);
        if (st[i]) (void)hipStreamDestroy(st[i]);
    }
    *nlines = line_off;
    return rc;
}

int rrx_match_cstr(const rrx_regex *re, int device, const char *text, int *accepted, size_t *len) {
    if (!re || !text || !accepted) return fail(RRX_ERR_ARG, "null argument");
    const size_t n = std::strlen(text);
    if (len) *len = n;
    const DeviceTables *t;
    int rc = re->tables(device, &t);
    if (rc) return rc;
    HIP_TRY(hipSetDevice(device));
    std::lock_guard<std::mutex> lock(re->scratch_mu);
    const size_t acc_at = (n + 15) & ~(size_t)15, scratch_at = acc_at + 16;
    void *buf = nullptr;
    const LongStringPlan plan = long_string_plan(re, t, n);
    rc = re->scratch_for(device, scratch_at + plan.scratch_bytes, &buf);
    if (rc) return rc;
    uint8_t *d = static_cast<uint8_t *>(buf);
    hipError_t e = n ? hipMemcpy(d, text, n, hipMemcpyHostToDevice) : hipSuccess;
    if (e != hipSuccess) return hip_fail(e, "text upload");
    rc = match_string_with(re, device, t, plan, d, n, d + acc_at, d + scratch_at, nullptr);
    uint8_t a = 0;
    if (!rc) { e = hipMemcpy(&a, d + acc_at, 1, hipMemcpyDeviceToHost); if (e != hipSuccess) rc = hip_fail(e, "accept readback"); }
    *accepted = a;
    return rc;
}

}
```

roaringregex_amd/csrc/device.hpp:

```cpp
#pragma once
#include <cstddef>
#include <cstdint>

namespace rrx {
namespace dev {

#ifndef RRX_THREADS
#define RRX_THREADS 1024
#endif
constexpr int kThreads = RRX_THREADS;
constexpr uint32_t kMinStripe = 512, kMaxStripe = 16384, kMinAutoStripe = 2048;
constexpr size_t kTargetLanes = (size_t)1 << 21;
inline uint32_t pick_stripe(size_t nbytes) {
    uint32_t s = kMinStripe;
    while (s < kMinAutoStripe && nbytes / s > ((size_t)1 << 18)) s *= 2;
    while (s < kMaxStripe && nbytes / s > kTargetLanes) s *= 2;
    return s;
}
inline uint32_t stripe_for_lines(size_t nbytes, size_t avg_line) {
    uint32_t want = pick_stripe(nbytes);
    while (want < kMaxStripe && avg_line * 16 > want && nbytes / (2 * (size_t)want) >= ((size_t)1 << 18)) want *= 2;
    while (want > 1024 && (avg_line + 1) * 128 < want) want /= 2;
    return want;
}
constexpr int kRound = 128;
constexpr int kMaxNfaWords = 16;
constexpr uint32_t kWideColumns = 129;
constexpr uint32_t kWideMaxStates = 127;
constexpr uint32_t kClassedMaxEntries = 16384;

struct NfaMasks {
    uint32_t init[kMaxNfaWords], fin[kMaxNfaWords], chain[kMaxNfaWords], self[kMaxNfaWords], excm[kMaxNfaWords];
    uint32_t cgrp[kMaxNfaWords], ctgt[kMaxNfaWords];
};

struct NfaDevice {
    uint32_t W = 0, nbits = 0, any_exc = 0, any_carry = 0, any_self = 0;
    NfaMasks masks;
    const uint32_t *B = nullptr;
    const uint32_t *X = nullptr;
};

constexpr uint32_t kGroupMaxBits = 8192;
struct GroupNfaDevice {
    uint32_t G = 0, K = 0, nbits = 0, n_exc = 0, ncls = 0;
    uint32_t exc_mode = 0;
    uint32_t self_slots = 0;
    uint32_t b_slots = 0;
    uint32_t exc_slots = 0;
    const uint32_t *masks = nullptr;
    const uint32_t *Bcls = nullptr;
    const uint8_t *cls = nullptr;
    const uint16_t *xidx = nullptr;
    const uint32_t *X = nullptr;
};
inline bool group_geometry(uint32_t nbits, uint32_t *G, uint32_t *K) {
    static const uint32_t forms[][2] = {{8, 3}, {8, 4}, {16, 3}, {16, 4}, {32, 3}, {32, 4}, {32, 5}, {32, 8}};
    for (const auto &f : forms)
        if (nbits <= f[0] * f[1] * 32u) { *G = f[0]; *K = f[1]; return true; }
    return false;
}

constexpr uint32_t kBlockMaxBits = 65536;
struct WaveNfaDevice {
    uint32_t WL = 0, nbits = 0;
    uint32_t self_words = 0, exc_words = 0;
    const uint32_t *masks = nullptr;
    const uint32_t *Bbyte = nullptr;
    const uint32_t *xoff = nullptr;
    const uint32_t *xtgt = nullptr;
    uint32_t ncls = 0;
    const uint32_t *Bcls = nullptr;
    const uint8_t *cls = nullptr;
};

struct DfaDevice {
    uint32_t nstates = 0, ncls = 0, start = 0;
    const uint8_t *cls = nullptr;
    const uint16_t *next = nullptr;
    const uint8_t *acc = nullptr;
};

constexpr size_t kPlainDfaLdsBudget = 64 * 1024;

struct LineDfaDevice {
    uint32_t nrows = 0;
    uint32_t stride = 0;
    uint32_t start_off = 0;
    uint32_t wide = 0;
    uint32_t rep_log2 = 0;
    uint32_t in_global = 0;
    const uint32_t *table = nullptr;
    const uint8_t *cls = nullptr;
};

struct Dfa2Device {
    uint32_t nrows = 0, stride = 0, start_off = 0, rep_log2 = 0;
    const uint16_t *P = nullptr;
    const uint32_t *T2 = nullptr;
};
constexpr uint32_t kDfa2PStride = 130;
constexpr uint32_t kDfa2PBytes = 128 * kDfa2PStride * 2;
constexpr uint32_t kDfa2PItemsBytes = (129 * kDfa2PStride * 2 + 15) & ~15u;
constexpr uint32_t kDfa2RegionBytes = 46 * 1024;
constexpr uint32_t kDfa2MaxTable = kDfa2RegionBytes - 4 * 1024;
constexpr uint32_t kDfa2TableBudget = 30 * 1024;


int match_stripes_dfa(const LineDfaDevice &p, bool clamp_high, const uint8_t *bytes, size_t nbytes, uint32_t stripe,
                      const uint64_t *stripe_base, size_t nstripes, uint32_t *accept_bits, void *stream);
uint32_t flush_mask_for(size_t nbytes, size_t nlines);
int match_stripes_dfa2(const Dfa2Device &p, const uint8_t *bytes, size_t nbytes, uint32_t stripe, const uint64_t *stripe_base,
                       size_t nstripes, uint32_t *accept, void *stream, uint32_t flush_mask = 31u);
int match_stripes_dfa2_clean(const Dfa2Device &p, const uint8_t *bytes, size_t nbytes, uint32_t stripe, const uint64_t *stripe_base,
                             size_t nstripes, uint32_t *accept, void *stream, uint32_t flush_mask = 31u);
int match_units_dfa2(const Dfa2Device &p, const uint8_t *bytes, size_t nbytes, uint32_t stripe, const uint64_t *stripe_base,
                     size_t nstripes, uint32_t *accept, uint32_t units_per_wg, void *stream);
int match_stripes_dfa2_two_bit(const Dfa2Device &p, const uint8_t *bytes, size_t nbytes, uint32_t stripe, const uint64_t *stripe_base,
                               size_t nstripes, uint32_t *wide_bits, void *stream);
int split_two_bit(const uint32_t *wide, size_t nlines, uint32_t *accept_bits, uint32_t *escaped_bits, unsigned long long *escaped_total, uint64_t *list,
                  size_t cap, void *stream);

size_t onepass_slab_words(size_t nstripes, uint32_t stripe);
int match_onepass_dfa2(const Dfa2Device &p, const uint8_t *bytes, size_t nbytes, uint32_t stripe, size_t nstripes, uint32_t *counts,
                       uint32_t *slabs, void *stream);
int match_onepass_dfa(const LineDfaDevice &p, const uint8_t *bytes, size_t nbytes, uint32_t stripe, size_t nstripes, uint32_t *counts,
                      uint32_t *slabs, void *stream);
int compact_streams(const uint32_t *counts, const uint64_t *stripe_base, size_t nstripes, uint32_t stripe, const uint32_t *slabs,
                    uint32_t *accept_bits, size_t cap_words, void *stream);
int match_extents_dfa(const DfaDevice &p, const uint8_t *bytes, const uint64_t *off, size_t nitems, uint32_t trim,
                      uint8_t *accept, void *stream, const uint32_t *only_if = nullptr);

int count_newlines_per_stripe(const uint8_t *bytes, size_t nbytes, uint32_t stripe, uint32_t *counts, size_t nstripes, uint32_t *flags, void *stream);
int scan_counts(const uint32_t *counts, uint64_t *base, uint64_t *chunk_sums, size_t n, void *stream);
size_t scan_scratch_words(size_t n);
int expand_bits(const uint32_t *bits, size_t nlines, uint8_t *out, void *stream);
int bitmap_count(const uint32_t *bits, size_t nlines, unsigned long long *count, void *stream);
int mail_results(const uint64_t *total, const uint32_t *flags, const uint8_t *last_byte, uint64_t *mail, void *stream);
int build_line_offsets(const uint8_t *bytes, size_t nbytes, uint32_t stripe, const uint64_t *stripe_base, size_t nstripes,
                       uint64_t *line_off, void *stream);
int empty_matches(const uint64_t *line_off, size_t nlines, uint32_t *count, const uint64_t *first, uint32_t *match_start, uint32_t *match_end,
                  void *stream, size_t cap = ~(size_t)0);

constexpr uint32_t kItemColumns = 131, kItemEndColumn = 129;
size_t items_index_bytes(size_t nbytes, size_t nitems);
size_t items_result_bytes(size_t nitems);
int items_index_build(size_t nbytes, const uint64_t *off, size_t nitems, uint32_t trim, void *index, uint32_t **flag, void *stream,
                      const uint8_t *resolve_base = nullptr, size_t min_bytes = 0);
struct ItemVerdicts {
    uint8_t *bytes = nullptr;
    uint32_t *bits = nullptr;
    ItemVerdicts(uint8_t *b) : bytes(b) {}
    ItemVerdicts(uint32_t *w) : bits(w) {}
};
int items_match2(const Dfa2Device &p, const uint8_t *bytes, size_t nbytes, size_t nitems, const void *index, void *result, ItemVerdicts out, void *stream,
                 const uint64_t *resolve_off = nullptr, const uint32_t *skip_if = nullptr);
int items_match(const LineDfaDevice &p, const uint8_t *bytes, size_t nbytes, size_t nitems, uint32_t trim, const void *index, void *result,
                ItemVerdicts out, void *stream, const uint64_t *resolve_off = nullptr, const uint32_t *skip_if = nullptr);

int contains_extents_dfa(const DfaDevice &p, bool in_global, uint32_t found, const uint8_t *bytes, const uint64_t *off, size_t nitems, uint32_t trim,
                         uint32_t *bits, void *stream, const uint32_t *only_if = nullptr);
int copy_result_bits(const uint32_t *result, size_t nitems, uint32_t *bits, void *stream);

constexpr uint32_t kLongMaxStates = 254;
constexpr uint32_t kLongGroup = 128;
size_t long_scratch_bytes(uint32_t nstates, size_t nbytes, uint32_t *chunk);
int match_long_dfa(const DfaDevice &p, const uint8_t *bytes, size_t nbytes, uint32_t chunk, void *scratch, uint8_t *accept,
                   void *stream);

constexpr uint32_t kSearchP8Stride = 132, kSearchP8Bytes = 128 * kSearchP8Stride;
constexpr uint32_t kSearchP16Stride = 130, kSearchP16Bytes = 128 * kSearchP16Stride * 2;
struct SearchChunkDevice {
    uint32_t nrows = 0, ncols2 = 0, row_bytes = 0, base_row = 0, in_global = 0;
    uint32_t start_row = 0, skip_row = 0;
    uint32_t nr = 0, ncls = 0, start_r = 0;
    const uint8_t *P8 = nullptr;
    const uint16_t *P16 = nullptr;
    const uint16_t *T2 = nullptr, *T2_all = nullptr;
    const uint32_t *G2 = nullptr, *G2_all = nullptr;
    const uint16_t *rev = nullptr;
    const uint8_t *cls = nullptr;
};
constexpr size_t kSearchChunkLdsBudget = 160 * 1024;
size_t search_chunk_bytes();
size_t search_chunks_lds_bytes(const SearchChunkDevice &p);
int search_chunks(const SearchChunkDevice &p, bool clean, const uint8_t *bytes, size_t nbytes, const uint64_t *chunk_base, size_t nchunks, size_t nlines,
                  uint32_t *match_start, uint32_t *match_end, void *stream);
int search_chunks_count(const SearchChunkDevice &p, bool clean, const uint8_t *bytes, size_t nbytes, const uint64_t *chunk_base, size_t nchunks,
                        uint32_t *count, void *stream);
int search_chunks_fill(const SearchChunkDevice &p, bool clean, const uint8_t *bytes, size_t nbytes, const uint64_t *chunk_base, size_t nchunks,
                       const uint64_t *first, uint32_t *match_start, uint32_t *match_end, void *stream);
size_t search_all_scratch_bytes(size_t nchunks);
int search_chunks_all(const SearchChunkDevice &p, bool clean, const uint8_t *bytes, size_t nbytes, const uint64_t *chunk_base, size_t nchunks, size_t nlines,
                      uint64_t *first, uint32_t *match_start, uint32_t *match_end, size_t cap, void *scratch, void *stream);

int match_stripes_nfa(const NfaDevice &p, const uint8_t *bytes, size_t nbytes, uint32_t stripe, const uint64_t *stripe_base,
                      size_t nstripes, uint32_t *accept_bits, void *stream);
int match_onepass_nfa(const NfaDevice &p, const uint8_t *bytes, size_t nbytes, uint32_t stripe, size_t nstripes, uint32_t *counts,
                      uint32_t *slabs, void *stream);
int recheck_escaped_nfa(const NfaDevice &p, const uint8_t *bytes, size_t nbytes, uint32_t stripe, const uint64_t *stripe_base, size_t nstripes,
                        const uint32_t *escaped_bits, size_t nlines, const uint64_t *list, const unsigned long long *escaped_total, size_t cap,
                        uint32_t *accept_bits, void *stream);
int match_extents_nfa(const NfaDevice &p, const uint8_t *bytes, const uint64_t *off, size_t nitems, uint32_t trim,
                      uint8_t *accept, void *stream);
size_t long_nfa_scratch_bytes(const NfaDevice &p, size_t nbytes, uint32_t *chunk, uint32_t *nchunks);
int match_long_nfa(const NfaDevice &p, const uint8_t *bytes, size_t nbytes, uint32_t chunk, uint32_t nchunks, void *scratch, uint8_t *accept,
                   void *stream);

int match_stripes_group_nfa(const GroupNfaDevice &p, const uint8_t *bytes, size_t nbytes, uint32_t stripe, const uint64_t *stripe_base,
                            size_t nstripes, uint32_t *accept_bits, void *stream);
int match_extents_group_nfa(const GroupNfaDevice &p, const uint8_t *bytes, const uint64_t *off, size_t nitems, uint32_t trim,
                            uint8_t *accept, void *stream);

uint32_t wave_words_per_lane(uint32_t words);
uint32_t sparse_rows(uint32_t words);
int match_stripes_sparse_nfa(const WaveNfaDevice &p, const uint8_t *bytes, size_t nbytes, uint32_t stripe, const uint64_t *stripe_base,
                             size_t nstripes, uint32_t *accept_bits, void *stream);
int match_extents_sparse_nfa(const WaveNfaDevice &p, const uint8_t *bytes, const uint64_t *off, size_t nitems, uint32_t trim,
                             uint8_t *accept, void *stream);
int match_stripes_wave_nfa(const WaveNfaDevice &p, const uint8_t *bytes, size_t nbytes, uint32_t stripe, const uint64_t *stripe_base,
                           size_t nstripes, uint32_t *accept_bits, void *stream);
int match_extents_wave_nfa(const WaveNfaDevice &p, const uint8_t *bytes, const uint64_t *off, size_t nitems, uint32_t trim,
                           uint8_t *accept, void *stream);

}
}
```

roaringregex_amd/csrc/kernels_index.hip:

```cpp
#include "kernels_common.hpp"

namespace rrx {
namespace dev {
namespace {

__global__ void mail_results_kernel(const uint64_t *__restrict__ total, const uint32_t *__restrict__ flags, const uint8_t *__restrict__ last_byte,
                                    uint64_t *__restrict__ mail) {
    if (threadIdx.x || blockIdx.x) return;
    mail[0] = line_of(*total);
    mail[1] = flags ? *flags : 0u;
    mail[2] = last_byte ? *last_byte : (uint64_t)'\n';
    __threadfence_system();
}

__global__ __launch_bounds__(256) void count_newlines_kernel(const uint8_t *__restrict__ bytes, size_t nbytes, uint32_t stripe,
                                                              uint32_t *__restrict__ counts, size_t nstripes,
                                                              uint32_t *__restrict__ flags) {
    const size_t g = (size_t)blockIdx.x * 256 + threadIdx.x;
    if (g >= nstripes) return;
    const size_t start = g * (size_t)stripe;
    const size_t end = start + stripe < nbytes ? start + stripe : nbytes;
    const uint4 *src = reinterpret_cast<const uint4 *>(bytes + start);
    const int units = (int)((end - start) / 16);
    uint32_t cnt = 0, high = 0;
    int u = 0;
    for (; u + 4 <= units; u += 4) {
        uint4 v[4];
#pragma unroll
        for (int i = 0; i < 4; i++) v[i] = src[u + i];
#pragma unroll
        for (int i = 0; i < 4; i++) {
            const uint32_t w[4] = {v[i].x, v[i].y, v[i].z, v[i].w};
#pragma unroll
            for (int j = 0; j < 4; j++) {
                uint32_t x = w[j] ^ 0x0a0a0a0au;
                uint32_t z = ~(((x & 0x7f7f7f7fu) + 0x7f7f7f7fu) | x | 0x7f7f7f7fu);
                cnt += __popc(z);
                high |= w[j];
            }
        }
    }
    for (size_t p = start + (size_t)u * 16; p < end; p++) { cnt += bytes[p] == '\n'; high |= bytes[p]; }
    counts[g] = cnt | (bytes[end - 1] == '\n' ? kEndsOnNewline : 0u);
    if (high & 0x80808080u) atomicOr(flags, 1u);
}

__global__ __launch_bounds__(256) void count_newlines_wave_kernel(const uint8_t *__restrict__ bytes, size_t nbytes, uint32_t stripe,
                                                                   uint32_t *__restrict__ counts, size_t nstripes,
                                                                   uint32_t *__restrict__ flags) {
    const int lane = threadIdx.x & 63;
    const size_t nwaves = (size_t)gridDim.x * 4;
    uint32_t high = 0;
    for (size_t g = ((size_t)blockIdx.x * 256 + threadIdx.x) >> 6; g < nstripes; g += nwaves) {
        const size_t start = g * (size_t)stripe;
        const size_t end = start + stripe < nbytes ? start + stripe : nbytes;
        uint32_t cnt = 0, last = 0;
        if (end - start == stripe) {
            const uint4 *src = reinterpret_cast<const uint4 *>(bytes + start) + lane;
            const int n = (int)(stripe >> 10);
            for (int i = 0; i < n; i += 4) {
                uint4 v[4];
#pragma unroll
                for (int k = 0; k < 4; k++)
                    if (i + k < n) v[k] = src[(size_t)(i + k) * 64];
#pragma unroll
                for (int k = 0; k < 4; k++) {
                    if (i + k < n) {
                        const uint32_t w[4] = {v[k].x, v[k].y, v[k].z, v[k].w};
#pragma unroll
                        for (int j = 0; j < 4; j++) {
                            const uint32_t x = w[j] ^ 0x0a0a0a0au;
                            const uint32_t z = ~(((x & 0x7f7f7f7fu) + 0x7f7f7f7fu) | x | 0x7f7f7f7fu);
                            cnt += __popc(z);
                            high |= w[j];
                        }
                        last = v[k].w >> 24;
                    }
                }
            }
            last = __shfl(last, 63, 64);
        } else {
            for (size_t p = start + lane; p < end; p += 64) { const uint32_t b = bytes[p]; cnt += b == '\n'; high |= b; }
            last = bytes[end - 1];
        }
#pragma unroll
        for (int d = 32; d; d >>= 1) cnt += __shfl_xor(cnt, d, 64);
        if (lane == 0) counts[g] = cnt | (last == '\n' ? kEndsOnNewline : 0u);
    }
    if (__ballot((high & 0x80808080u) != 0) && lane == 0) atomicOr(flags, 1u);
}

__global__ __launch_bounds__(256) void expand_bits_kernel(const uint32_t *__restrict__ bits, size_t nlines, uint8_t *__restrict__ out) {
    const size_t w = (size_t)blockIdx.x * 256 + threadIdx.x;
    if (w * 32 >= nlines) return;
    const uint32_t v = bits[w];
    if (w * 32 + 32 <= nlines) {
        uint4 o[2];
        uint32_t *p = reinterpret_cast<uint32_t *>(o);
#pragma unroll
        for (int j = 0; j < 8; j++) {
            uint32_t n = (v >> (4 * j)) & 0xfu;
            p[j] = (n & 1u) | ((n & 2u) << 7) | ((n & 4u) << 14) | ((n & 8u) << 21);
        }
        uint4 *dst = reinterpret_cast<uint4 *>(out + w * 32);
        dst[0] = o[0]; dst[1] = o[1];
    } else {
        for (size_t i = w * 32; i < nlines; i++) out[i] = (uint8_t)((v >> (i & 31)) & 1u);
    }
}

constexpr int kScanChunk = 4096;
__global__ __launch_bounds__(256) void scan_chunk_sums_kernel(const uint32_t *__restrict__ counts, size_t n, uint64_t *__restrict__ sums) {
    __shared__ uint64_t part[4];
    const size_t lo = (size_t)blockIdx.x * kScanChunk;
    uint64_t s = 0;
    for (size_t i = lo + threadIdx.x; i < lo + kScanChunk && i < n; i += 256) s += counts[i] & kCountMask;
#pragma unroll
    for (int d = 32; d; d >>= 1) s += __shfl_down(s, d, 64);
    if ((threadIdx.x & 63) == 0) part[threadIdx.x >> 6] = s;
    __syncthreads();
    if (threadIdx.x == 0) sums[blockIdx.x] = part[0] + part[1] + part[2] + part[3];
}
template <int NW>
__device__ __forceinline__ uint64_t block_exclusive_scan(uint64_t v, uint64_t *wave_tot, uint64_t &total) {
    const int lane = threadIdx.x & 63, wave = threadIdx.x >> 6;
    uint64_t inc = v;
#pragma unroll
    for (int d = 1; d < 64; d <<= 1) {
        const uint64_t o = __shfl_up(inc, d, 64);
        if (lane >= d) inc += o;
    }
    if (lane == 63) wave_tot[wave] = inc;
    __syncthreads();
    uint64_t off = 0, tot = 0;
#pragma unroll
    for (int w = 0; w < NW; w++) {
        const uint64_t t = wave_tot[w];
        if (w < wave) off += t;
        tot += t;
    }
    total = tot;
    return off + inc - v;
}
__global__ __launch_bounds__(1024) void scan_sums_kernel(uint64_t *__restrict__ sums, size_t nchunks, uint64_t *__restrict__ total) {
    __shared__ uint64_t wave_tot[16];
    const size_t per = (nchunks + 1023) / 1024;
    const size_t lo = threadIdx.x * per < nchunks ? threadIdx.x * per : nchunks, hi = lo + per < nchunks ? lo + per : nchunks;
    uint64_t s = 0;
    for (size_t i = lo; i < hi; i++) s += sums[i];
    uint64_t all;
    uint64_t run = block_exclusive_scan<16>(s, wave_tot, all);
    if (threadIdx.x == 0) *total = all;
    for (size_t i = lo; i < hi; i++) { uint64_t v = sums[i]; sums[i] = run; run += v; }
}
__global__ __launch_bounds__(256) void scan_chunks_kernel(const uint32_t *__restrict__ counts, size_t n, const uint64_t *__restrict__ sums,
                                                           uint64_t *__restrict__ base) {
    __shared__ uint64_t wave_tot[4];
    constexpr int kPer = kScanChunk / 256;
    const size_t lo = (size_t)blockIdx.x * kScanChunk + (size_t)threadIdx.x * kPer;
    uint32_t c[kPer];
    uint32_t before = 0;
    if (lo + kPer <= n) {
        const uint4 *src = reinterpret_cast<const uint4 *>(counts + lo);
#pragma unroll
        for (int k = 0; k < kPer / 4; k++) { const uint4 v = src[k]; c[4 * k] = v.x; c[4 * k + 1] = v.y; c[4 * k + 2] = v.z; c[4 * k + 3] = v.w; }
    } else {
#pragma unroll
        for (int k = 0; k < kPer; k++) c[k] = lo + k < n ? counts[lo + k] : 0u;
    }
    if (lo && lo < n) before = counts[lo - 1];
    uint64_t s = 0;
#pragma unroll
    for (int k = 0; k < kPer; k++) s += c[k] & kCountMask;
    uint64_t all;
    uint64_t run = sums[blockIdx.x] + block_exclusive_scan<4>(s, wave_tot, all);
#pragma unroll
    for (int k = 0; k < kPer; k++) {
        if (lo + k < n) {
            const bool fresh = lo + k == 0 || ((k ? c[k - 1] : before) & kEndsOnNewline);
            base[lo + k] = run | (fresh ? kFreshStripe : 0);
        }
        run += c[k] & kCountMask;
    }
}

__global__ __launch_bounds__(256) void line_offsets_kernel(const uint8_t *__restrict__ bytes, size_t nbytes, uint32_t stripe,
                                                           const uint64_t *__restrict__ stripe_base, size_t nstripes,
                                                           uint64_t *__restrict__ line_off) {
    const size_t g = (size_t)blockIdx.x * blockDim.x + threadIdx.x;
    if (g >= nstripes) return;
    const size_t start = g * (size_t)stripe, end = start + stripe < nbytes ? start + stripe : nbytes;
    uint64_t line = line_of(stripe_base[g]);
    if (g == 0) line_off[0] = 0;
    size_t pos = start;
    for (; pos + 16 <= end; pos += 16) {
        const uint4 v = *reinterpret_cast<const uint4 *>(bytes + pos);
        const uint32_t w[4] = {v.x, v.y, v.z, v.w};
#pragma unroll
        for (int j = 0; j < 4; j++) {
            const uint32_t x = w[j] ^ 0x0a0a0a0au;
            uint32_t hit = (x - 0x01010101u) & ~x & 0x80808080u;
            while (hit) {
                const int k = (__ffs((int)hit) - 1) >> 3;
                if (((w[j] >> (8 * k)) & 0xffu) == '\n') line_off[++line] = pos + 4 * j + k + 1;
                hit &= hit - 1;
            }
        }
    }
    for (; pos < end; pos++)
        if (bytes[pos] == '\n') line_off[++line] = pos + 1;
}

template <bool FILL>
__global__ __launch_bounds__(256) void empty_matches_kernel(const uint64_t *__restrict__ line_off, size_t nlines, uint32_t *__restrict__ count,
                                                            const uint64_t *__restrict__ first, uint32_t *__restrict__ match_start,
                                                            uint32_t *__restrict__ match_end, uint64_t cap) {
    const size_t i = (size_t)blockIdx.x * blockDim.x + threadIdx.x;
    if (i >= nlines) return;
    const uint64_t len = line_off[i + 1] - 1 - line_off[i];
    if (!FILL) { count[i] = (uint32_t)(len + 1); return; }
    const uint64_t slot = first[i];
    for (uint64_t k = 0; k <= len && slot + k < cap; k++) { match_start[slot + k] = (uint32_t)k; match_end[slot + k] = (uint32_t)k; }
}

}

int count_newlines_per_stripe(const uint8_t *bytes, size_t nbytes, uint32_t stripe, uint32_t *counts, size_t nstripes, uint32_t *flags,
                              void *stream) {
    if (!nstripes) return 0;
    if (stripe % 1024 == 0 && stripe >= 4096) {
        size_t blocks = (nstripes + 3) / 4;
        if (blocks > 8192) blocks = 8192;
        hipLaunchKernelGGL(count_newlines_wave_kernel, dim3((unsigned)blocks), dim3(256), 0, (hipStream_t)stream, bytes, nbytes, stripe, counts, nstripes, flags);
        return (int)hipGetLastError();
    }
    size_t blocks = (nstripes + 255) / 256;
    hipLaunchKernelGGL(count_newlines_kernel, dim3((unsigned)blocks), dim3(256), 0, (hipStream_t)stream, bytes, nbytes, stripe, counts, nstripes, flags);
    return (int)hipGetLastError();
}
int expand_bits(const uint32_t *bits, size_t nlines, uint8_t *out, void *stream) {
    if (!nlines) return 0;
    size_t words = (nlines + 31) / 32, blocks = (words + 255) / 256;
    hipLaunchKernelGGL(expand_bits_kernel, dim3((unsigned)blocks), dim3(256), 0, (hipStream_t)stream, bits, nlines, out);
    return (int)hipGetLastError();
}
int scan_counts(const uint32_t *counts, uint64_t *base, uint64_t *chunk_sums, size_t n, void *stream) {
    const size_t nchunks = (n + kScanChunk - 1) / kScanChunk;
    hipStream_t st = (hipStream_t)stream;
    if (nchunks) hipLaunchKernelGGL(scan_chunk_sums_kernel, dim3((unsigned)nchunks), dim3(256), 0, st, counts, n, chunk_sums);
    hipLaunchKernelGGL(scan_sums_kernel, dim3(1), dim3(1024), 0, st, chunk_sums, nchunks, base + n);
    if (nchunks) hipLaunchKernelGGL(scan_chunks_kernel, dim3((unsigned)nchunks), dim3(256), 0, st, counts, n, chunk_sums, base);
    return (int)hipGetLastError();
}
size_t scan_scratch_words(size_t n) { return (n + kScanChunk - 1) / kScanChunk + 1; }
__global__ __launch_bounds__(256) void bitmap_count_kernel(const uint32_t *__restrict__ bits, size_t nlines, unsigned long long *__restrict__ count) {
    const size_t words = (nlines + 31) / 32;
    const uint32_t tail = (uint32_t)(nlines & 31u);
    unsigned long long n = 0;
    for (size_t w = (size_t)blockIdx.x * 256 + threadIdx.x; w < words; w += (size_t)gridDim.x * 256) {
        uint32_t v = bits[w];
        if (w + 1 == words && tail) v &= (1u << tail) - 1u;
        n += (uint32_t)__popc(v);
    }
    for (int d = 32; d > 0; d >>= 1) n += __shfl_down(n, d, 64);
    if ((threadIdx.x & 63) == 0 && n) atomicAdd(count, n);
}
int bitmap_count(const uint32_t *bits, size_t nlines, unsigned long long *count, void *stream) {
    hipError_t e = hipMemsetAsync(count, 0, sizeof *count, (hipStream_t)stream);
    if (e != hipSuccess || !nlines) return (int)e;
    size_t blocks = ((nlines + 31) / 32 + 255) / 256;
    if (blocks > 2048) blocks = 2048;
    hipLaunchKernelGGL(bitmap_count_kernel, dim3((unsigned)blocks), dim3(256), 0, (hipStream_t)stream, bits, nlines, count);
    return (int)hipGetLastError();
}
int mail_results(const uint64_t *total, const uint32_t *flags, const uint8_t *last_byte, uint64_t *mail, void *stream) {
    hipLaunchKernelGGL(mail_results_kernel, dim3(1), dim3(64), 0, (hipStream_t)stream, total, flags, last_byte, mail);
    return (int)hipGetLastError();
}
int build_line_offsets(const uint8_t *bytes, size_t nbytes, uint32_t stripe, const uint64_t *stripe_base, size_t nstripes,
                       uint64_t *line_off, void *stream) {
    if (!nstripes) return 0;
    hipLaunchKernelGGL(line_offsets_kernel, dim3((unsigned)((nstripes + 255) / 256)), dim3(256), 0, (hipStream_t)stream, bytes, nbytes, stripe,
                       stripe_base, nstripes, line_off);
    return (int)hipGetLastError();
}
int empty_matches(const uint64_t *line_off, size_t nlines, uint32_t *count, const uint64_t *first, uint32_t *match_start, uint32_t *match_end,
                  void *stream, size_t cap) {
    if (!nlines) return 0;
    const dim3 grid((unsigned)((nlines + 255) / 256));
    if (first) hipLaunchKernelGGL(empty_matches_kernel<true>, grid, dim3(256), 0, (hipStream_t)stream, line_off, nlines, count, first, match_start, match_end, (uint64_t)cap);
    else hipLaunchKernelGGL(empty_matches_kernel<false>, grid, dim3(256), 0, (hipStream_t)stream, line_off, nlines, count, first, match_start, match_end, (uint64_t)cap);
    return (int)hipGetLastError();
}

}
}
```

roaringregex_amd/csrc/kernels_table.hip:

```cpp
#include "table_engines.hpp"

namespace rrx {
namespace dev {
namespace {

struct NoPhaseHook { __device__ __forceinline__ void operator()(int) const {} __device__ __forceinline__ void round(int) const {} };
enum { kPhaseEntry = 0, kPhaseTablesLoaded, kPhaseFirstRound, kPhaseMainDone, kPhaseFollowDone, kPhaseWindowOut, kPhases };
typedef uint32_t u32x4 __attribute__((ext_vector_type(4)));
template <bool ASM>
__device__ __forceinline__ void feed_load(uint4 (&buf)[kRound / 16], const uint4 *p) {
    static_assert(kRound / 16 == 8, "eight slots");
    if constexpr (!ASM) {
#pragma unroll
        for (int i = 0; i < 8; i++) buf[i] = load_text(p + i);
    } else {
        u32x4 a, b, c, d, e, f, g, h;
        asm volatile("global_load_dwordx4 %0, %8, off\n\t"
                     "global_load_dwordx4 %1, %8, off offset:16\n\t"
                     "global_load_dwordx4 %2, %8, off offset:32\n\t"
                     "global_load_dwordx4 %3, %8, off offset:48\n\t"
                     "global_load_dwordx4 %4, %8, off offset:64\n\t"
                     "global_load_dwordx4 %5, %8, off offset:80\n\t"
                     "global_load_dwordx4 %6, %8, off offset:96\n\t"
                     "global_load_dwordx4 %7, %8, off offset:112\n\t"
                     "s_waitcnt vmcnt(0)"
                     : "=&v"(a), "=&v"(b), "=&v"(c), "=&v"(d), "=&v"(e), "=&v"(f), "=&v"(g), "=&v"(h)
                     : "v"(p)
                     : "memory");
        const u32x4 t[8] = {a, b, c, d, e, f, g, h};
#pragma unroll
        for (int i = 0; i < 8; i++) buf[i] = make_uint4(t[i].x, t[i].y, t[i].z, t[i].w);
    }
}
template <bool ONEPASS, class PhaseHook, bool FEED_ASM = false, int KB = 1, bool CLEAN = ONEPASS>
__device__ __forceinline__ void dfa2_stripe(const Dfa2 &eng, const size_t g, const uint64_t window_word, uint32_t *const stage, const uint32_t stage_words,
                                            const uint8_t *__restrict__ bytes, const size_t nbytes, const uint32_t stripe,
                                            const uint64_t *__restrict__ stripe_base, uint32_t *__restrict__ accept_bits,
                                            uint32_t *__restrict__ counts, uint32_t *__restrict__ slabs, const uint32_t slab_row, PhaseHook &phase,
                                            const uint32_t flush_mask = 31u) {
    const size_t start = g * (size_t)stripe;
    if (start < nbytes) {
    const size_t stripe_end = start + stripe;
    const size_t my_end = stripe_end < nbytes ? stripe_end : nbytes;
    bool fresh = true;
    typename std::conditional<ONEPASS, LocalResults, ResultsT<true>>::type res;
    if constexpr (ONEPASS) {
        res.begin(slabs + g, slab_row);
    } else {
        const uint64_t my_base = stripe_base[g];
        fresh = (my_base & kFreshStripe) != 0;
        res.begin_staged(line_of(my_base) * KB, window_word, !fresh, accept_bits, stage);
        res.stage_words = stage_words;
        res.drop_mask = (1u << KB) - 1u;
    }
    Dfa2::State st = fresh ? eng.fresh() : eng.skipping();
    auto clean = [](uint32_t w) -> uint32_t {
        if (CLEAN && __builtin_amdgcn_ballot_w64((w & 0x80808080u) != 0)) {
            const uint32_t hi = (w & 0x80808080u) >> 7;
            w &= ~(hi * 0xffu);
        }
        return w;
    };

    size_t pos = start;
    const uint4 *src = reinterpret_cast<const uint4 *>(bytes + start);
    constexpr int kSlots = kRound / 16;
    const int rounds = (int)((my_end - start) / kRound);
    uint4 buf[kSlots];
    if (rounds > 0) feed_load<FEED_ASM>(buf, src);
    uint32_t last_word = 0;
    bool ahead = false;
    for (int r = 0; r < rounds; r++) {
        if (r == 1) phase(kPhaseFirstRound);
        phase.round(r);
#pragma unroll
        for (int i = 0; i < kSlots; i++) {
            if (CLEAN && __builtin_expect(__builtin_amdgcn_ballot_w64(((buf[i].x | buf[i].y | buf[i].z | buf[i].w) & 0x80808080u) != 0) != 0, 0)) {
                eng.consume_dword(st, clean(buf[i].x), res.bits);
                eng.consume_dword(st, clean(buf[i].y), res.bits);
                eng.consume_dword(st, clean(buf[i].z), res.bits);
                eng.consume_dword(st, clean(buf[i].w), res.bits);
            } else {
                eng.consume_dword(st, buf[i].x, res.bits);
                eng.consume_dword(st, buf[i].y, res.bits);
                if (KB == 2 && (res.bits >> 15)) res.flush();
                eng.consume_dword(st, buf[i].z, res.bits);
                eng.consume_dword(st, buf[i].w, res.bits);
            }
            if ((((uint32_t)r * kSlots + (uint32_t)i) & flush_mask) == flush_mask) res.flush();
            else if (res.bits >> 15) res.flush();
        }
        if (r + 1 < rounds) {
            feed_load<FEED_ASM>(buf, src + (r + 1) * kSlots);
        } else {
            last_word = buf[kSlots - 1].w;
            if (start + (size_t)(rounds + 1) * kRound <= nbytes) {
                feed_load<FEED_ASM>(buf, src + (r + 1) * kSlots);
                ahead = true;
            }
        }
    }
    pos += (size_t)rounds * kRound;
    phase(kPhaseMainDone);
    auto byte_at = [&](size_t q) -> uint32_t { const uint32_t b = bytes[q]; return (CLEAN && b >= 0x80u) ? 0u : b; };

    bool closed_by_end_of_data = false;
    for (; pos + 2 <= my_end; pos += 2) {
        uint32_t lines, verdicts;
        eng.step2(st, byte_at(pos), byte_at(pos + 1), lines, verdicts);
        res.bits = (res.bits << lines) | verdicts;
        if (res.bits >> (31 - 2 * KB)) res.flush();
    }
    if (pos < my_end) {
        const uint32_t b = byte_at(pos);
        uint32_t lines, verdicts;
        eng.step2(st, b, '\n', lines, verdicts);
        if (b == '\n') res.push(KB, verdicts >> KB);
        else { res.push(KB, verdicts); closed_by_end_of_data = true; }
        pos++;
    }
    res.flush();
    const uint32_t newlines = res.seen - (closed_by_end_of_data ? 1u : 0u);

    if (ONEPASS && res.seen == 0) fresh = g == 0 || bytes[start - 1] == '\n';
    const bool started = fresh || res.seen > 0;
    bool followed = false;
    const bool whole_rounds = rounds > 0 && start + (size_t)rounds * kRound == my_end;
    const uint32_t last_byte = whole_rounds ? last_word >> 24 : (uint32_t)bytes[my_end - 1];
    if (!closed_by_end_of_data && started && last_byte != '\n') {
        uint32_t lines = 0, verdicts = 0;
        if (ahead && pos == start + (size_t)(rounds + 1) * kRound - kRound) {
    #pragma unroll
            for (int i = 0; i < kSlots; i++) {
                if (!lines) {
                    const uint32_t w[4] = {clean(buf[i].x), clean(buf[i].y), clean(buf[i].z), clean(buf[i].w)};
#pragma unroll
                    for (int k = 0; k < 8; k++)
                        if (!lines) eng.step2(st, (w[k >> 1] >> (16 * (k & 1))) & 0xffu, (w[k >> 1] >> (16 * (k & 1) + 8)) & 0xffu, lines, verdicts);
                    pos += 16;
                }
            }
        }
        while (pos + 16 <= nbytes && !lines) {
            const uint4 v = *reinterpret_cast<const uint4 *>(bytes + pos);
            const uint32_t w[4] = {clean(v.x), clean(v.y), clean(v.z), clean(v.w)};
#pragma unroll
            for (int k = 0; k < 8; k++)
                if (!lines) eng.step2(st, (w[k >> 1] >> (16 * (k & 1))) & 0xffu, (w[k >> 1] >> (16 * (k & 1) + 8)) & 0xffu, lines, verdicts);
            pos += 16;
        }
        for (; pos + 2 <= nbytes && !lines; pos += 2) eng.step2(st, byte_at(pos), byte_at(pos + 1), lines, verdicts);
        if (!lines) eng.step2(st, pos < nbytes ? byte_at(pos) : '\n', '\n', lines, verdicts);
        res.push(KB, lines == 2 * KB ? verdicts >> KB : verdicts);
        followed = true;
    }
    res.finish();
    phase(kPhaseFollowDone);
    if (ONEPASS)
        counts[g] = newlines | ((followed || closed_by_end_of_data) ? kExtraResult : 0u) | (last_byte == '\n' ? kEndsOnNewline : 0u);
    }
}

template <bool ONEPASS, class PhaseHook = NoPhaseHook, int KB = 1, bool CLEAN = ONEPASS>
__device__ __forceinline__ void dfa2_body(const Dfa2Device &prog, const uint8_t *__restrict__ bytes, size_t nbytes, uint32_t stripe,
                                          const uint64_t *__restrict__ stripe_base, uint32_t *__restrict__ accept_bits,
                                          uint32_t *__restrict__ counts, uint32_t *__restrict__ slabs, PhaseHook phase = PhaseHook(),
                                          uint32_t flush_mask = 31u) {
    phase(kPhaseEntry);
    __shared__ __attribute__((aligned(16))) struct {
        uint8_t t2_and_stage[kDfa2RegionBytes];
        uint16_t p[kDfa2PBytes / 2];
    } lds;
    Dfa2 eng;
    eng.load(prog, lds.p, lds.t2_and_stage);
    const uint32_t stage_off = (uint32_t)((Dfa2::lds_bytes(prog) + 15) & ~(size_t)15);
    uint32_t *const stage = reinterpret_cast<uint32_t *>(lds.t2_and_stage + stage_off);
    const uint32_t stage_words = (kDfa2RegionBytes - stage_off) / 4;
    if (!ONEPASS)
        for (uint32_t i = threadIdx.x; i < stage_words; i += kThreads) stage[i] = 0;
    __syncthreads();
    phase(kPhaseTablesLoaded);

    const size_t g0 = (size_t)blockIdx.x * kThreads;
    uint64_t window_word = 0;
    if (!ONEPASS) window_word = (line_of(stripe_base[g0]) * KB) >> 5;
    dfa2_stripe<ONEPASS, PhaseHook, false, KB, CLEAN>(eng, g0 + threadIdx.x, window_word, stage, stage_words, bytes, nbytes, stripe, stripe_base, accept_bits, counts, slabs,
                         gridDim.x * kThreads, phase, flush_mask);
    if (!ONEPASS) {
        __syncthreads();
        for (uint32_t i = threadIdx.x; i < stage_words; i += kThreads) {
            const uint32_t v = stage[i];
            if (v) atomicOr(&accept_bits[window_word + i], v);
        }
    }
    phase(kPhaseWindowOut);
}
template <class PhaseHook = NoPhaseHook>
__device__ __forceinline__ void dfa2_units_body(const Dfa2Device &prog, const uint8_t *__restrict__ bytes, size_t nbytes, uint32_t stripe,
                                                const uint64_t *__restrict__ stripe_base, uint32_t *__restrict__ accept_bits, uint32_t units_per_wg,
                                                PhaseHook phase = PhaseHook()) {
    phase(kPhaseEntry);
    __shared__ __attribute__((aligned(16))) struct {
        uint8_t t2_and_stage[kDfa2RegionBytes];
        uint16_t p[kDfa2PBytes / 2];
    } lds;
    Dfa2 eng;
    eng.load(prog, lds.p, lds.t2_and_stage);
    const uint32_t stage_off = (uint32_t)((Dfa2::lds_bytes(prog) + 15) & ~(size_t)15);
    uint32_t *const stage = reinterpret_cast<uint32_t *>(lds.t2_and_stage + stage_off);
    const uint32_t stage_words = (kDfa2RegionBytes - stage_off) / 4 - 1;
    uint32_t &next_unit = stage[stage_words];
    for (uint32_t i = threadIdx.x; i < stage_words; i += kThreads) stage[i] = 0;
    if (threadIdx.x == 0) next_unit = kThreads / 64;
    __syncthreads();
    phase(kPhaseTablesLoaded);
    const size_t g_wg = (size_t)blockIdx.x * units_per_wg * 64;
    const uint64_t window_word = line_of(stripe_base[g_wg]) >> 5;
    uint32_t unit = __builtin_amdgcn_readfirstlane(threadIdx.x >> 6);
    while (unit < units_per_wg) {
        uint32_t lane;
        asm volatile("v_and_b32 %0, 63, %1" : "=v"(lane) : "v"(threadIdx.x));
        dfa2_stripe<false, PhaseHook, true>(eng, g_wg + (size_t)unit * 64 + lane, window_word, stage, stage_words, bytes, nbytes, stripe, stripe_base, accept_bits,
                           nullptr, nullptr, 0u, phase);
        uint32_t ticket = 0;
        if (__builtin_amdgcn_mbcnt_hi(~0u, __builtin_amdgcn_mbcnt_lo(~0u, 0u)) == 0) ticket = atomicAdd(&next_unit, 1u);
        unit = __builtin_amdgcn_readfirstlane(ticket);
    }
    __syncthreads();
    for (uint32_t i = threadIdx.x; i < stage_words; i += kThreads) {
        const uint32_t v = stage[i];
        if (v) atomicOr(&accept_bits[window_word + i], v);
    }
    phase(kPhaseWindowOut);
}
__global__ __launch_bounds__(kThreads) __attribute__((amdgpu_waves_per_eu(8, 8))) void match_units2_kernel(
    Dfa2Device prog, const uint8_t *__restrict__ bytes, size_t nbytes, uint32_t stripe, const uint64_t *__restrict__ stripe_base,
    uint32_t *__restrict__ accept_bits, uint32_t units_per_wg) {
    dfa2_units_body(prog, bytes, nbytes, stripe, stripe_base, accept_bits, units_per_wg);
}
__global__ __launch_bounds__(kThreads) void match_stripes2_kernel(Dfa2Device prog, const uint8_t *__restrict__ bytes, size_t nbytes,
                                                                   uint32_t stripe, const uint64_t *__restrict__ stripe_base,
                                                                   uint32_t *__restrict__ accept_bits, uint32_t flush_mask) {
    dfa2_body<false>(prog, bytes, nbytes, stripe, stripe_base, accept_bits, nullptr, nullptr, NoPhaseHook(), flush_mask);
}
__global__ __launch_bounds__(kThreads) void match_stripes2_clean_kernel(
    Dfa2Device prog, const uint8_t *__restrict__ bytes, size_t nbytes, uint32_t stripe, const uint64_t *__restrict__ stripe_base,
    uint32_t *__restrict__ accept_bits, uint32_t flush_mask) {
    dfa2_body<false, NoPhaseHook, 1, true>(prog, bytes, nbytes, stripe, stripe_base, accept_bits, nullptr, nullptr, NoPhaseHook(), flush_mask);
}
__global__ __launch_bounds__(kThreads) void match_stripes2_two_bit_kernel(Dfa2Device prog, const uint8_t *__restrict__ bytes, size_t nbytes,
                                                                           uint32_t stripe, const uint64_t *__restrict__ stripe_base,
                                                                           uint32_t *__restrict__ wide_bits) {
    dfa2_body<false, NoPhaseHook, 2>(prog, bytes, nbytes, stripe, stripe_base, wide_bits, nullptr, nullptr);
}
__global__ __launch_bounds__(kThreads) void match_stripes2_onepass_kernel(Dfa2Device prog, const uint8_t *__restrict__ bytes, size_t nbytes,
                                                                           uint32_t stripe, uint32_t *__restrict__ counts,
                                                                           uint32_t *__restrict__ slabs) {
    dfa2_body<true>(prog, bytes, nbytes, stripe, nullptr, nullptr, counts, slabs);
}

constexpr uint32_t kCompactWindowWords = 8192;
__global__ __launch_bounds__(256) void compact_streams_kernel(const uint32_t *__restrict__ counts, const uint64_t *__restrict__ stripe_base,
                                                               size_t nstripes, uint32_t stripe, const uint32_t *__restrict__ slabs,
                                                               uint32_t *__restrict__ accept_bits, size_t cap_words) {
    __shared__ uint32_t window[kCompactWindowWords];
    const size_t g0 = (size_t)blockIdx.x * 256;
    const size_t g1 = g0 + 256 < nstripes ? g0 + 256 : nstripes;
    const uint64_t window_word = line_of(stripe_base[g0]) >> 5;
    const uint64_t span = (line_of(stripe_base[g1]) >> 5) - window_word + 2;
    const uint32_t used = span < kCompactWindowWords ? (uint32_t)span : kCompactWindowWords;
    for (uint32_t i = threadIdx.x; i < used; i += 256) window[i] = 0;
    __syncthreads();
    const size_t g = g0 + threadIdx.x;
    if (g < nstripes) {
        const uint32_t c = counts[g];
        const uint32_t n = (c & kCountMask) + ((c & kExtraResult) ? 1u : 0u);
        const uint64_t b = stripe_base[g];
        const uint64_t base = line_of(b);
        const bool fresh = (b & kFreshStripe) != 0;
        const size_t row = (nstripes + kThreads - 1) / kThreads * kThreads;
        const uint32_t *src = slabs + g;
        auto put = [&](uint64_t word, uint32_t v) {
            if (!v) return;
            if (word >= cap_words) return;
            const uint64_t rel = word - window_word;
            if (rel < used) atomicOr(&window[(uint32_t)rel], v);
            else atomicOr(&accept_bits[word], v);
        };
        for (uint32_t k = 0; k * 32 < n; k++) {
            uint32_t v = src[(size_t)k * row];
            if (n - k * 32 < 32) v &= (1u << (n - k * 32)) - 1u;
            if (k == 0 && !fresh) v &= ~1u;
            const uint64_t bit = base + (uint64_t)k * 32;
            const uint32_t sh = (uint32_t)bit & 31u;
            put(bit >> 5, v << sh);
            if (sh) put((bit >> 5) + 1, v >> (32u - sh));
        }
    }
    __syncthreads();
    for (uint32_t i = threadIdx.x; i < used; i += 256) {
        const uint32_t v = window[i];
        if (v && window_word + i < cap_words) atomicOr(&accept_bits[window_word + i], v);
    }
}

}

int match_stripes_dfa(const LineDfaDevice &p, bool clamp_high, const uint8_t *bytes, size_t nbytes, uint32_t stripe,
                      const uint64_t *stripe_base, size_t nstripes, uint32_t *accept, void *stream) {
#define GO(WIDE, CLAMP) launch_stripes<LineDfaEngine<WIDE, CLAMP>, LineDfaDevice>(p, LineDfaEngine<WIDE, CLAMP>::lds_bytes(p), bytes, nbytes, stripe, stripe_base, nstripes, accept, stream)
    if (p.in_global) return launch_stripes<LineDfaGlobalEngine, LineDfaDevice>(p, 256, bytes, nbytes, stripe, stripe_base, nstripes, accept, stream);
    if (p.wide) return clamp_high ? GO(true, true) : GO(true, false);
    return GO(false, false);
#undef GO
}
uint32_t flush_mask_for(size_t nbytes, size_t nlines) {
    const size_t avg = nlines ? nbytes / nlines : nbytes;
    uint32_t slots = 1;
    while (slots < 32 && (size_t)slots * 2 * 16 <= avg * 16) slots *= 2;
    return slots - 1;
}
template <class... Params, class... Rest>
static int launch_dfa2(void (*kernel)(Params...), const Dfa2Device &p, const uint8_t *bytes, size_t nbytes, uint32_t stripe, size_t nstripes,
                       size_t stripes_per_wg, void *stream, Rest... rest) {
    if (!nstripes) return 0;
    if (Dfa2::lds_bytes(p) > kDfa2MaxTable) return (int)hipErrorInvalidValue;
    const size_t blocks = (nstripes + stripes_per_wg - 1) / stripes_per_wg;
    hipLaunchKernelGGL(kernel, dim3((unsigned)blocks), dim3(kThreads), 0, (hipStream_t)stream, p, bytes, nbytes, stripe, rest...);
    return (int)hipGetLastError();
}
int match_stripes_dfa2(const Dfa2Device &p, const uint8_t *bytes, size_t nbytes, uint32_t stripe, const uint64_t *stripe_base,
                       size_t nstripes, uint32_t *accept, void *stream, uint32_t flush_mask) {
    return launch_dfa2(match_stripes2_kernel, p, bytes, nbytes, stripe, nstripes, kThreads, stream, stripe_base, accept, flush_mask);
}
int match_stripes_dfa2_clean(const Dfa2Device &p, const uint8_t *bytes, size_t nbytes, uint32_t stripe, const uint64_t *stripe_base,
                             size_t nstripes, uint32_t *accept, void *stream, uint32_t flush_mask) {
    return launch_dfa2(match_stripes2_clean_kernel, p, bytes, nbytes, stripe, nstripes, kThreads, stream, stripe_base, accept, flush_mask);
}
__global__ __launch_bounds__(256) void split_two_bit_kernel(const uint32_t *__restrict__ wide, size_t words, uint32_t *__restrict__ accept_bits,
                                                             uint32_t *__restrict__ escaped_bits, unsigned long long *__restrict__ escaped_total,
                                                             uint64_t *__restrict__ list, size_t cap) {
    constexpr uint32_t kLocal = 4096, kFlushAt = kLocal - 256 * 8;
    __shared__ uint64_t local[kLocal];
    __shared__ uint32_t nlocal;
    __shared__ unsigned long long flush_base;
    if (threadIdx.x == 0) nlocal = 0;
    __syncthreads();
    auto even_bits = [](uint32_t x) -> uint32_t {
        x &= 0x55555555u;
        x = (x | x >> 1) & 0x33333333u;
        x = (x | x >> 2) & 0x0f0f0f0fu;
        x = (x | x >> 4) & 0x00ff00ffu;
        return (x | x >> 8) & 0xffffu;
    };
    auto flush = [&]() {
        __syncthreads();
        const uint32_t n = nlocal;
        if (n) {
            if (threadIdx.x == 0) flush_base = atomicAdd(escaped_total, (unsigned long long)n);
            __syncthreads();
            const unsigned long long base = flush_base;
            for (uint32_t i = threadIdx.x; i < n; i += 256) if (base + i < cap) list[base + i] = local[i];
            __syncthreads();
            if (threadIdx.x == 0) nlocal = 0;
        }
        __syncthreads();
    };
    const size_t turns = (words + (size_t)gridDim.x * 256 - 1) / ((size_t)gridDim.x * 256);
    for (size_t it = 0; it < turns; it++) {
        const size_t w = (it * gridDim.x + blockIdx.x) * 256 + threadIdx.x;
        uint32_t esc = 0;
        if (w < words) {
            const uint2 v = reinterpret_cast<const uint2 *>(wide)[w];
            accept_bits[w] = even_bits(v.x) | even_bits(v.y) << 16;
            esc = even_bits(v.x >> 1) | even_bits(v.y >> 1) << 16;
            escaped_bits[w] = esc;
        }
        while (__syncthreads_or(esc != 0)) {
            uint32_t take = 0;
            for (uint32_t k = 0, m = esc; k < 8 && m; k++) { take |= m & (0u - m); m &= m - 1; }
            const uint32_t c = (uint32_t)__popc(take);
            if (c) {
                uint32_t at = atomicAdd(&nlocal, c);
                for (uint32_t m = take; m; m &= m - 1) local[at++] = (uint64_t)w * 32 + (uint32_t)(__ffs((int)m) - 1);
            }
            esc &= ~take;
            __syncthreads();
            if (nlocal > kFlushAt) flush();
        }
    }
    flush();
}
int match_stripes_dfa2_two_bit(const Dfa2Device &p, const uint8_t *bytes, size_t nbytes, uint32_t stripe, const uint64_t *stripe_base,
                               size_t nstripes, uint32_t *wide_bits, void *stream) {
    return launch_dfa2(match_stripes2_two_bit_kernel, p, bytes, nbytes, stripe, nstripes, kThreads, stream, stripe_base, wide_bits);
}
int split_two_bit(const uint32_t *wide, size_t nlines, uint32_t *accept_bits, uint32_t *escaped_bits, unsigned long long *escaped_total, uint64_t *list,
                  size_t cap, void *stream) {
    const size_t words = (nlines + 31) / 32;
    if (!words) return 0;
    size_t blocks = (words + 255) / 256;
    if (blocks > 2048) blocks = 2048;
    hipLaunchKernelGGL(split_two_bit_kernel, dim3((unsigned)blocks), dim3(256), 0, (hipStream_t)stream, wide, words, accept_bits, escaped_bits, escaped_total,
                       list, cap);
    return (int)hipGetLastError();
}
int match_units_dfa2(const Dfa2Device &p, const uint8_t *bytes, size_t nbytes, uint32_t stripe, const uint64_t *stripe_base,
                     size_t nstripes, uint32_t *accept, uint32_t units_per_wg, void *stream) {
    if (nstripes && !units_per_wg) return (int)hipErrorInvalidValue;
    return launch_dfa2(match_units2_kernel, p, bytes, nbytes, stripe, nstripes, (size_t)64 * units_per_wg, stream, stripe_base, accept, units_per_wg);
}
int match_onepass_dfa(const LineDfaDevice &p, const uint8_t *bytes, size_t nbytes, uint32_t stripe, size_t nstripes, uint32_t *counts,
                      uint32_t *slabs, void *stream) {
    if (p.in_global) return launch_onepass<LineDfaGlobalEngine, LineDfaDevice>(p, 256, bytes, nbytes, stripe, nstripes, counts, slabs, stream);
    if (p.wide) return launch_onepass<LineDfaEngine<true, true>, LineDfaDevice>(p, LineDfaEngine<true, true>::lds_bytes(p), bytes, nbytes, stripe, nstripes, counts, slabs, stream);
    return launch_onepass<LineDfaEngine<false, false>, LineDfaDevice>(p, LineDfaEngine<false, false>::lds_bytes(p), bytes, nbytes, stripe, nstripes, counts, slabs, stream);
}
size_t onepass_slab_words(size_t nstripes, uint32_t stripe) {
    return ((nstripes + kThreads - 1) / kThreads) * slab_words_per_lane(stripe) * kThreads;
}
int match_onepass_dfa2(const Dfa2Device &p, const uint8_t *bytes, size_t nbytes, uint32_t stripe, size_t nstripes, uint32_t *counts,
                       uint32_t *slabs, void *stream) {
    return launch_dfa2(match_stripes2_onepass_kernel, p, bytes, nbytes, stripe, nstripes, kThreads, stream, counts, slabs);
}
int compact_streams(const uint32_t *counts, const uint64_t *stripe_base, size_t nstripes, uint32_t stripe, const uint32_t *slabs,
                    uint32_t *accept_bits, size_t cap_words, void *stream) {
    if (!nstripes) return 0;
    hipLaunchKernelGGL(compact_streams_kernel, dim3((unsigned)((nstripes + 255) / 256)), dim3(256), 0, (hipStream_t)stream, counts, stripe_base, nstripes,
                       stripe, slabs, accept_bits, cap_words);
    return (int)hipGetLastError();
}
int match_extents_dfa(const DfaDevice &p, const uint8_t *bytes, const uint64_t *off, size_t nitems, uint32_t trim, uint8_t *accept,
                      void *stream, const uint32_t *only_if) {
    if (PlainDfaEngine::lds_bytes(p) > kPlainDfaLdsBudget)
        return launch_extents<PlainDfaGlobalEngine, DfaDevice>(p, PlainDfaGlobalEngine::lds_bytes(p), bytes, off, nitems, trim, accept, stream, only_if);
    return launch_extents<PlainDfaEngine, DfaDevice>(p, PlainDfaEngine::lds_bytes(p), bytes, off, nitems, trim, accept, stream, only_if);
}

}
}
```

Measured before the change: 5589.

## Let DFA2 workgroups own bitmap words to skip memset and atomics

Adds a corpus-creation check that decides whether each workgroup's line-bitmap window can be owned outright. When it can, the DFA2 match kernel writes its words directly and uses a per-stream slot array, so the separate bitmap memset and the global atomicOr flush are skipped. It also templates the kernel on a compile-time flush-slot count and removes the units-per-workgroup kernel path. The trade-offs are extra per-stream device allocations, more kernel instantiations and more complex correctness conditions at window boundaries.

```diff
diff --git a/include/rrx.h b/include/rrx.h
--- a/include/rrx.h
+++ b/include/rrx.h
@@ -63,6 +63,8 @@
 size_t rrx_corpus_num_bytes(const rrx_corpus *c);
 void   rrx_corpus_free(rrx_corpus *c);
 size_t rrx_corpus_bitmap_words(const rrx_corpus *c);
+int    rrx_corpus_one_launch(const rrx_corpus *c, uint32_t *span_words);
+uint32_t rrx_match_flush_slots(const rrx_regex *re, const rrx_corpus *c, int *compiled_in);
 int rrx_match_corpus(const rrx_regex *re, const rrx_corpus *c, uint32_t *d_accept_bits, void *stream);
 int rrx_match_device(const rrx_regex *re, int device, const void *d_bytes, size_t nbytes, uint32_t *d_accept_bits,
                      size_t cap_words, size_t *nlines, void *stream);
diff --git a/roaringregex_amd/__init__.py b/roaringregex_amd/__init__.py
--- a/roaringregex_amd/__init__.py
+++ b/roaringregex_amd/__init__.py
@@ -29,6 +29,7 @@
     "rrx_engine", "rrx_engine_name", "rrx_useful_states", "rrx_byte_classes", "rrx_table_order", "rrx_order_table", "rrx_set_option", "rrx_learn_table", "rrx_sampled_table", "rrx_sampled_escapes", "rrx_words_per_set", "rrx_accepts_empty",
     "rrx_program_words",
     "rrx_corpus_create", "rrx_corpus_create_ex", "rrx_corpus_stripe_bytes", "rrx_corpus_num_lines", "rrx_corpus_num_bytes", "rrx_corpus_free", "rrx_corpus_bitmap_words",
+    "rrx_corpus_one_launch", "rrx_match_flush_slots",
     "rrx_match_corpus", "rrx_match_device", "rrx_search_corpus", "rrx_search_all_count", "rrx_search_all_fill", "rrx_search_all", "rrx_bitmap_to_bytes",
     "rrx_match_extents", "rrx_items_create", "rrx_items_count", "rrx_items_stripe_wise", "rrx_items_free", "rrx_match_items",
     "rrx_match_string", "rrx_match_host", "rrx_match_cstr",
@@ -82,6 +83,8 @@
         "rrx_corpus_num_bytes": (sz, [vp]),
         "rrx_corpus_free": (None, [vp]),
         "rrx_corpus_bitmap_words": (sz, [vp]),
+        "rrx_corpus_one_launch": (i32, [vp, C.POINTER(u32)]),
+        "rrx_match_flush_slots": (u32, [vp, vp, C.POINTER(i32)]),
         "rrx_match_corpus": (i32, [vp, vp, vp, vp]),
         "rrx_match_device": (i32, [vp, i32, vp, sz, vp, sz, C.POINTER(sz), vp]),
         "rrx_bitmap_to_bytes": (i32, [i32, vp, sz, vp, vp]),
@@ -223,6 +226,16 @@
     def stripe(self):
         return _L.rrx_corpus_stripe_bytes(self._h)
 
+    @property
+    def one_launch(self):
+        return bool(_L.rrx_corpus_one_launch(self._h, None))
+
+    @property
+    def one_launch_span(self):
+        span = C.c_uint32(0)
+        _L.rrx_corpus_one_launch(self._h, C.byref(span))
+        return span.value
+
 
 class Items:
 
@@ -550,6 +563,11 @@
     def set_flush_slots(self, slots):
         _check(_L.rrx_set_option(self._h, OPT_FLUSH_SLOTS, int(slots)))
 
+    def flush_slots(self, corpus):
+        fixed = C.c_int(0)
+        slots = _L.rrx_match_flush_slots(self._h, corpus._h, C.byref(fixed))
+        return slots, bool(fixed.value)
+
     def set_search_anchored(self, enabled):
         _check(_L.rrx_set_option(self._h, OPT_SEARCH_ANCHORED, 1 if enabled else 0))
 
diff --git a/roaringregex_amd/csrc/abi.cpp b/roaringregex_amd/csrc/abi.cpp
--- a/roaringregex_amd/csrc/abi.cpp
+++ b/roaringregex_amd/csrc/abi.cpp
@@ -134,7 +134,6 @@
     mutable Dfa2OrderStats t2_order_stats;
     std::atomic<int> opt_background_order{1};
     std::atomic<int> opt_search_anchored{1};
-    std::atomic<int> opt_units_per_wg{0};
     std::atomic<int> opt_sampled_table{1};
     std::atomic<int> opt_flush_slots{0};
     int requested_engine = 0;
@@ -391,6 +390,10 @@
     uint32_t *d_counts = nullptr;
     uint64_t *d_base = nullptr;
     bool has_high = false;
+    bool own_words = false;
+    uint32_t own_span = 0;
+    static constexpr size_t kMaxSlotArrays = 64;
+    mutable std::map<hipStream_t, unsigned long long *> slot_arrays;
     uint8_t *h_sample = nullptr;
     uint32_t sample_lanes = 0;
     mutable std::mutex mu;
@@ -515,7 +518,6 @@
     }
     if (option == RRX_OPT_UNITS_PER_WORKGROUP) {
         if (value < 0 || value > 65536) return fail(RRX_ERR_ARG, "units per workgroup: 0 (off) or 16 ... 65536");
-        re->opt_units_per_wg.store(value && value < 16 ? 16 : (int)value);
         return RRX_OK;
     }
     return fail(RRX_ERR_ARG, "unknown option");
@@ -576,7 +578,7 @@
 int rrx_corpus_create_ex(int device, const void *d_bytes, size_t nbytes, uint32_t stripe_bytes, void *stream, rrx_corpus **out) {
     if (!out || (nbytes && !d_bytes)) return fail(RRX_ERR_ARG, "null argument");
     if (stripe_bytes && (stripe_bytes < dev::kMinStripe || stripe_bytes > dev::kMaxStripe || (stripe_bytes & (stripe_bytes - 1))))
-        return fail(RRX_ERR_ARG, "stripe must be a power of two in [1024, 16384]");
+        return fail(RRX_ERR_ARG, "stripe must be a power of two in [512, 16384]");
     if (reinterpret_cast<uintptr_t>(d_bytes) & 15) return fail(RRX_ERR_ARG, "corpus base must be 16-byte aligned");
     *out = nullptr;
     HIP_TRY(hipSetDevice(device));
@@ -594,14 +596,15 @@
         }
     }
     c->nstripes = (nbytes + c->stripe - 1) / c->stripe;
-    hipError_t e = hipMalloc(reinterpret_cast<void **>(&c->d_counts), (c->nstripes + 1) * sizeof(uint32_t));
+    hipError_t e = hipMalloc(reinterpret_cast<void **>(&c->d_counts), (c->nstripes + 3) * sizeof(uint32_t));
     if (e == hipSuccess) e = hipMalloc(reinterpret_cast<void **>(&c->d_base), (c->nstripes + 1 + dev::scan_scratch_words(c->nstripes)) * sizeof(uint64_t));
     if (e != hipSuccess) { rrx_corpus_free(c); return hip_fail(e, "hipMalloc(line index)"); }
     uint32_t *d_flags = c->d_counts + c->nstripes;
-    e = hipMemsetAsync(d_flags, 0, sizeof(uint32_t), (hipStream_t)stream);
+    e = hipMemsetAsync(d_flags, 0, 3 * sizeof(uint32_t), (hipStream_t)stream);
     if (e != hipSuccess) { rrx_corpus_free(c); return hip_fail(e, "hipMemsetAsync(flags)"); }
     int rc = dev::count_newlines_per_stripe(c->d_bytes, nbytes, c->stripe, c->d_counts, c->nstripes, d_flags, stream);
     if (!rc) rc = dev::scan_counts(c->d_counts, c->d_base, c->d_base + c->nstripes + 1, c->nstripes, stream);
+    if (!rc && c->nstripes) rc = dev::own_words_check(c->d_base, c->nstripes, c->d_bytes + nbytes - 1, d_flags + 1, stream);
     if (rc) { rrx_corpus_free(c); return hip_fail((hipError_t)rc, "line index launch"); }
     MailboxGuard mail;
     if (int mrc = mailbox_acquire(device, &mail.m)) { rrx_corpus_free(c); return mrc; }
@@ -620,7 +623,7 @@
         }
     }
     mail.stream = (hipStream_t)stream; mail.queued = true;
-    rc = dev::mail_results(c->d_base + c->nstripes, d_flags, nbytes ? c->d_bytes + nbytes - 1 : nullptr, mail.m.dev, stream);
+    rc = dev::mail_results(c->d_base + c->nstripes, d_flags, nbytes ? c->d_bytes + nbytes - 1 : nullptr, mail.m.dev, stream, d_flags + 1);
     if (rc) { rrx_corpus_free(c); return hip_fail((hipError_t)rc, "line index launch"); }
     e = hipStreamSynchronize((hipStream_t)stream);
     if (e != hipSuccess) { rrx_corpus_free(c); return hip_fail(e, "line index readback"); }
@@ -629,6 +632,8 @@
     const uint32_t flags = (uint32_t)mail.m.host[1];
     const uint8_t last = nbytes ? (uint8_t)mail.m.host[2] : (uint8_t)'\n';
     c->has_high = (flags & 1u) != 0;
+    c->own_words = c->nstripes && mail.m.host[3] == 0;
+    c->own_span = (uint32_t)mail.m.host[4];
     c->nlines = (size_t)total + ((nbytes && last != '\n') ? 1 : 0);
     if (!stripe_bytes && c->nlines) {
         const uint32_t want = dev::stripe_for_lines(nbytes, nbytes / c->nlines);
@@ -643,6 +648,10 @@
 size_t rrx_corpus_num_lines(const rrx_corpus *c) { return c->nlines; }
 size_t rrx_corpus_num_bytes(const rrx_corpus *c) { return c->nbytes; }
 uint32_t rrx_corpus_stripe_bytes(const rrx_corpus *c) { return c->stripe; }
+int rrx_corpus_one_launch(const rrx_corpus *c, uint32_t *span_words) {
+    if (span_words) *span_words = c->own_words ? c->own_span : 0;
+    return c->own_words ? 1 : 0;
+}
 void rrx_corpus_free(rrx_corpus *c) {
     if (!c) return;
     (void)hipSetDevice(c->device);
@@ -652,6 +661,7 @@
     if (c->d_chunk_base && c->d_chunk_base != c->d_base) (void)hipFree(c->d_chunk_base);
     if (c->d_all_scratch) (void)hipFree(c->d_all_scratch);
     if (c->h_sample) (void)hipHostFree(c->h_sample);
+    for (auto &kv : c->slot_arrays) (void)hipFree(kv.second);
     delete c;
 }
 
@@ -697,12 +707,42 @@
     return rc2;
 }
 
+static unsigned long long *own_words_for(const rrx_corpus *c, const dev::Dfa2Device &d2, hipStream_t stream) {
+    if (!c->own_words || c->own_span >= dev::dfa2_window_words(d2)) return nullptr;
+    hipStreamCaptureStatus capture = hipStreamCaptureStatusNone;
+    if (hipStreamIsCapturing(stream, &capture) != hipSuccess) { (void)hipGetLastError(); return nullptr; }
+    if (capture != hipStreamCaptureStatusNone) return nullptr;
+    std::lock_guard<std::mutex> lock(c->mu);
+    auto it = c->slot_arrays.find(stream);
+    if (it != c->slot_arrays.end()) return it->second;
+    if (c->slot_arrays.size() >= rrx_corpus::kMaxSlotArrays) return nullptr;
+    const size_t bytes = ((c->nstripes + dev::kThreads - 1) / dev::kThreads + 1) * sizeof(unsigned long long);
+    unsigned long long *slots = nullptr;
+    if (hipMalloc(reinterpret_cast<void **>(&slots), bytes) != hipSuccess) { (void)hipGetLastError(); return nullptr; }
+    if (hipMemsetAsync(slots, 0, bytes, stream) != hipSuccess) { (void)hipGetLastError(); (void)hipFree(slots); return nullptr; }
+    c->slot_arrays.emplace(stream, slots);
+    return slots;
+}
+static uint32_t flush_mask_of(const rrx_regex *re, const rrx_corpus *c) {
+    return re->opt_flush_slots.load() ? (uint32_t)re->opt_flush_slots.load() - 1u : dev::flush_mask_for(c->nbytes, c->nlines);
+}
+uint32_t rrx_match_flush_slots(const rrx_regex *re, const rrx_corpus *c, int *compiled_in) {
+    const uint32_t mask = flush_mask_of(re, c);
+    if (compiled_in) *compiled_in = dev::dfa2_flush_at_compile_time(mask) ? 1 : 0;
+    return mask + 1;
+}
+
 static int launch_line_tables(const rrx_regex *re, const rrx_corpus *c, const LineTables &lt, const DeviceTables *t, bool stride2_over_high, uint32_t *bits,
                               void *stream) {
-    if (!lt.has_dfa2 || (c->has_high && !stride2_over_high)) return dev::match_stripes_dfa(t->line, c->has_high, c->d_bytes, c->nbytes, c->stripe, c->d_base, c->nstripes, bits, stream);
-    const dev::Dfa2Device d2 = re->dfa2_device(t);
-    const uint32_t flush_mask = re->opt_flush_slots.load() ? (uint32_t)re->opt_flush_slots.load() - 1u : dev::flush_mask_for(c->nbytes, c->nlines);
-    return (c->has_high ? dev::match_stripes_dfa2_clean : dev::match_stripes_dfa2)(d2, c->d_bytes, c->nbytes, c->stripe, c->d_base, c->nstripes, bits, stream, flush_mask);
+    const size_t words = rrx_corpus_bitmap_words(c);
+    const bool stride2 = lt.has_dfa2 && (!c->has_high || stride2_over_high);
+    dev::Dfa2Device d2;
+    unsigned long long *slots = nullptr;
+    if (stride2) { d2 = re->dfa2_device(t); slots = own_words_for(c, d2, (hipStream_t)stream); }
+    if (!slots) HIP_TRY(hipMemsetAsync(bits, 0, words * sizeof(uint32_t), (hipStream_t)stream));
+    if (!stride2) return launched(dev::match_stripes_dfa(t->line, c->has_high, c->d_bytes, c->nbytes, c->stripe, c->d_base, c->nstripes, bits, stream), "match_stripes launch");
+    return launched(dev::match_stripes_dfa2(d2, c->has_high, c->d_bytes, c->nbytes, c->stripe, c->d_base, c->nstripes, bits, stream, flush_mask_of(re, c), slots, words),
+                    "match_stripes launch");
 }
 
 int rrx_match_corpus(const rrx_regex *re, const rrx_corpus *c, uint32_t *d_accept_bits, void *stream) {
@@ -724,6 +764,8 @@
             re->relearn_sampled(c->h_sample, c->sample_lanes, kSampleBytes);
         if (re->sampled_ready.load(std::memory_order_acquire) && !re->sampled_retired.load()) return match_corpus_sampled(re, c, t, d_accept_bits, stream);
     }
+    if (re->engine != RRX_ENGINE_NFA_SPARSE && re->engine != RRX_ENGINE_NFA_BLOCK && re->engine != RRX_ENGINE_NFA_WAVE && re->engine != RRX_ENGINE_NFA)
+        return launch_line_tables(re, c, re->match, t, false, d_accept_bits, stream);
     HIP_TRY(hipMemsetAsync(d_accept_bits, 0, rrx_corpus_bitmap_words(c) * sizeof(uint32_t), (hipStream_t)stream));
     int e = re->engine == RRX_ENGINE_NFA_SPARSE
                 ? dev::match_stripes_sparse_nfa(t->block, c->d_bytes, c->nbytes, c->stripe, c->d_base, c->nstripes, d_accept_bits, stream)
@@ -731,11 +773,7 @@
                 ? dev::match_stripes_wave_nfa(t->block, c->d_bytes, c->nbytes, c->stripe, c->d_base, c->nstripes, d_accept_bits, stream)
             : re->engine == RRX_ENGINE_NFA_WAVE
                 ? dev::match_stripes_group_nfa(t->group, c->d_bytes, c->nbytes, c->stripe, c->d_base, c->nstripes, d_accept_bits, stream)
-            : re->engine == RRX_ENGINE_NFA
-                ? dev::match_stripes_nfa(t->nfa, c->d_bytes, c->nbytes, c->stripe, c->d_base, c->nstripes, d_accept_bits, stream)
-            : (re->match.has_dfa2 && !c->has_high && re->opt_units_per_wg.load())
-                ? dev::match_units_dfa2(re->dfa2_device(t), c->d_bytes, c->nbytes, c->stripe, c->d_base, c->nstripes, d_accept_bits, (uint32_t)re->opt_units_per_wg.load(), stream)
-                : launch_line_tables(re, c, re->match, t, false, d_accept_bits, stream);
+                : dev::match_stripes_nfa(t->nfa, c->d_bytes, c->nbytes, c->stripe, c->d_base, c->nstripes, d_accept_bits, stream);
     return launched(e, "match_stripes launch");
 }
 
@@ -746,8 +784,7 @@
     if (rc) return rc;
     HIP_TRY(hipSetDevice(c->device));
     if (!c->nlines) return RRX_OK;
-    HIP_TRY(hipMemsetAsync(d_bits, 0, rrx_corpus_bitmap_words(c) * sizeof(uint32_t), (hipStream_t)stream));
-    return launched(launch_line_tables(re, c, re->contains_set.lt, t, true, d_bits, stream), "contains launch");
+    return launch_line_tables(re, c, re->contains_set.lt, t, true, d_bits, stream);
 }
 const char *rrx_contains_engine_name(const rrx_regex *re) {
     if (!re) { (void)fail(RRX_ERR_ARG, "null argument"); return nullptr; }
diff --git a/roaringregex_amd/csrc/device.hpp b/roaringregex_amd/csrc/device.hpp
--- a/roaringregex_amd/csrc/device.hpp
+++ b/roaringregex_amd/csrc/device.hpp
@@ -110,12 +110,11 @@
 int match_stripes_dfa(const LineDfaDevice &p, bool clamp_high, const uint8_t *bytes, size_t nbytes, uint32_t stripe,
                       const uint64_t *stripe_base, size_t nstripes, uint32_t *accept_bits, void *stream);
 uint32_t flush_mask_for(size_t nbytes, size_t nlines);
-int match_stripes_dfa2(const Dfa2Device &p, const uint8_t *bytes, size_t nbytes, uint32_t stripe, const uint64_t *stripe_base,
-                       size_t nstripes, uint32_t *accept, void *stream, uint32_t flush_mask = 31u);
-int match_stripes_dfa2_clean(const Dfa2Device &p, const uint8_t *bytes, size_t nbytes, uint32_t stripe, const uint64_t *stripe_base,
-                             size_t nstripes, uint32_t *accept, void *stream, uint32_t flush_mask = 31u);
-int match_units_dfa2(const Dfa2Device &p, const uint8_t *bytes, size_t nbytes, uint32_t stripe, const uint64_t *stripe_base,
-                     size_t nstripes, uint32_t *accept, uint32_t units_per_wg, void *stream);
+int match_stripes_dfa2(const Dfa2Device &p, bool clean, const uint8_t *bytes, size_t nbytes, uint32_t stripe, const uint64_t *stripe_base,
+                       size_t nstripes, uint32_t *accept, void *stream, uint32_t flush_mask = 31u, unsigned long long *slots = nullptr,
+                       size_t nwords = 0);
+uint32_t dfa2_window_words(const Dfa2Device &p);
+bool dfa2_flush_at_compile_time(uint32_t flush_mask);
 int match_stripes_dfa2_two_bit(const Dfa2Device &p, const uint8_t *bytes, size_t nbytes, uint32_t stripe, const uint64_t *stripe_base,
                                size_t nstripes, uint32_t *wide_bits, void *stream);
 int split_two_bit(const uint32_t *wide, size_t nlines, uint32_t *accept_bits, uint32_t *escaped_bits, unsigned long long *escaped_total, uint64_t *list,
@@ -136,7 +135,8 @@
 size_t scan_scratch_words(size_t n);
 int expand_bits(const uint32_t *bits, size_t nlines, uint8_t *out, void *stream);
 int bitmap_count(const uint32_t *bits, size_t nlines, unsigned long long *count, void *stream);
-int mail_results(const uint64_t *total, const uint32_t *flags, const uint8_t *last_byte, uint64_t *mail, void *stream);
+int mail_results(const uint64_t *total, const uint32_t *flags, const uint8_t *last_byte, uint64_t *mail, void *stream, const uint32_t *own = nullptr);
+int own_words_check(const uint64_t *stripe_base, size_t nstripes, const uint8_t *last_byte, uint32_t *own, void *stream);
 int build_line_offsets(const uint8_t *bytes, size_t nbytes, uint32_t stripe, const uint64_t *stripe_base, size_t nstripes,
                        uint64_t *line_off, void *stream);
 int empty_matches(const uint64_t *line_off, size_t nlines, uint32_t *count, const uint64_t *first, uint32_t *match_start, uint32_t *match_end,
diff --git a/roaringregex_amd/csrc/kernels_index.hip b/roaringregex_amd/csrc/kernels_index.hip
--- a/roaringregex_amd/csrc/kernels_index.hip
+++ b/roaringregex_amd/csrc/kernels_index.hip
@@ -5,12 +5,31 @@
 namespace {
 
 __global__ void mail_results_kernel(const uint64_t *__restrict__ total, const uint32_t *__restrict__ flags, const uint8_t *__restrict__ last_byte,
-                                    uint64_t *__restrict__ mail) {
+                                    uint64_t *__restrict__ mail, const uint32_t *__restrict__ own) {
     if (threadIdx.x || blockIdx.x) return;
     mail[0] = line_of(*total);
     mail[1] = flags ? *flags : 0u;
     mail[2] = last_byte ? *last_byte : (uint64_t)'\n';
+    mail[3] = own ? own[0] : 0u;
+    mail[4] = own ? own[1] : 0u;
     __threadfence_system();
+}
+
+__global__ __launch_bounds__(256) void own_words_kernel(const uint64_t *__restrict__ stripe_base, size_t nstripes, size_t nworkgroups,
+                                                        const uint8_t *__restrict__ last_byte, uint32_t *__restrict__ own) {
+    const size_t b = (size_t)blockIdx.x * 256 + threadIdx.x;
+    if (b >= nworkgroups) return;
+    const uint64_t first = line_of(stripe_base[b * kThreads]) >> 5;
+    uint64_t last;
+    if (b + 1 < nworkgroups) {
+        last = line_of(stripe_base[(b + 1) * kThreads]) >> 5;
+        if (last <= first) { atomicOr(&own[0], 1u); return; }
+    } else {
+        const uint64_t nlines = line_of(stripe_base[nstripes]) + (*last_byte != '\n' ? 1u : 0u);
+        last = (nlines - 1) >> 5;
+    }
+    const uint64_t span = last - first;
+    atomicMax(&own[1], span < 0xffffffffull ? (uint32_t)span : 0xffffffffu);
 }
 
 __global__ __launch_bounds__(256) void count_newlines_kernel(const uint8_t *__restrict__ bytes, size_t nbytes, uint32_t stripe,
@@ -273,8 +292,14 @@
     hipLaunchKernelGGL(bitmap_count_kernel, dim3((unsigned)blocks), dim3(256), 0, (hipStream_t)stream, bits, nlines, count);
     return (int)hipGetLastError();
 }
-int mail_results(const uint64_t *total, const uint32_t *flags, const uint8_t *last_byte, uint64_t *mail, void *stream) {
-    hipLaunchKernelGGL(mail_results_kernel, dim3(1), dim3(64), 0, (hipStream_t)stream, total, flags, last_byte, mail);
+int mail_results(const uint64_t *total, const uint32_t *flags, const uint8_t *last_byte, uint64_t *mail, void *stream, const uint32_t *own) {
+    hipLaunchKernelGGL(mail_results_kernel, dim3(1), dim3(64), 0, (hipStream_t)stream, total, flags, last_byte, mail, own);
+    return (int)hipGetLastError();
+}
+int own_words_check(const uint64_t *stripe_base, size_t nstripes, const uint8_t *last_byte, uint32_t *own, void *stream) {
+    const size_t nworkgroups = (nstripes + kThreads - 1) / kThreads;
+    hipLaunchKernelGGL(own_words_kernel, dim3((unsigned)((nworkgroups + 255) / 256)), dim3(256), 0, (hipStream_t)stream, stripe_base, nstripes, nworkgroups,
+                       last_byte, own);
     return (int)hipGetLastError();
 }
 int build_line_offsets(const uint8_t *bytes, size_t nbytes, uint32_t stripe, const uint64_t *stripe_base, size_t nstripes,
diff --git a/roaringregex_amd/csrc/kernels_table.hip b/roaringregex_amd/csrc/kernels_table.hip
--- a/roaringregex_amd/csrc/kernels_table.hip
+++ b/roaringregex_amd/csrc/kernels_table.hip
@@ -6,38 +6,18 @@
 
 struct NoPhaseHook { __device__ __forceinline__ void operator()(int) const {} __device__ __forceinline__ void round(int) const {} };
 enum { kPhaseEntry = 0, kPhaseTablesLoaded, kPhaseFirstRound, kPhaseMainDone, kPhaseFollowDone, kPhaseWindowOut, kPhases };
-typedef uint32_t u32x4 __attribute__((ext_vector_type(4)));
-template <bool ASM>
 __device__ __forceinline__ void feed_load(uint4 (&buf)[kRound / 16], const uint4 *p) {
-    static_assert(kRound / 16 == 8, "eight slots");
-    if constexpr (!ASM) {
 #pragma unroll
-        for (int i = 0; i < 8; i++) buf[i] = load_text(p + i);
-    } else {
-        u32x4 a, b, c, d, e, f, g, h;
-        asm volatile("global_load_dwordx4 %0, %8, off\n\t"
-                     "global_load_dwordx4 %1, %8, off offset:16\n\t"
-                     "global_load_dwordx4 %2, %8, off offset:32\n\t"
-                     "global_load_dwordx4 %3, %8, off offset:48\n\t"
-                     "global_load_dwordx4 %4, %8, off offset:64\n\t"
-                     "global_load_dwordx4 %5, %8, off offset:80\n\t"
-                     "global_load_dwordx4 %6, %8, off offset:96\n\t"
-                     "global_load_dwordx4 %7, %8, off offset:112\n\t"
-                     "s_waitcnt vmcnt(0)"
-                     : "=&v"(a), "=&v"(b), "=&v"(c), "=&v"(d), "=&v"(e), "=&v"(f), "=&v"(g), "=&v"(h)
-                     : "v"(p)
-                     : "memory");
-        const u32x4 t[8] = {a, b, c, d, e, f, g, h};
-#pragma unroll
-        for (int i = 0; i < 8; i++) buf[i] = make_uint4(t[i].x, t[i].y, t[i].z, t[i].w);
-    }
-}
-template <bool ONEPASS, class PhaseHook, bool FEED_ASM = false, int KB = 1, bool CLEAN = ONEPASS>
+    for (int i = 0; i < kRound / 16; i++) buf[i] = load_text(p + i);
+    asm volatile("" : : "v"(p));
+}
+template <bool ONEPASS, class PhaseHook, int FLUSH_SLOTS, int KB = 1, bool CLEAN = ONEPASS>
 __device__ __forceinline__ void dfa2_stripe(const Dfa2 &eng, const size_t g, const uint64_t window_word, uint32_t *const stage, const uint32_t stage_words,
                                             const uint8_t *__restrict__ bytes, const size_t nbytes, const uint32_t stripe,
                                             const uint64_t *__restrict__ stripe_base, uint32_t *__restrict__ accept_bits,
                                             uint32_t *__restrict__ counts, uint32_t *__restrict__ slabs, const uint32_t slab_row, PhaseHook &phase,
-                                            const uint32_t flush_mask = 31u) {
+                                            const uint32_t flush_mask) {
+    static_assert(FLUSH_SLOTS >= 0 && (FLUSH_SLOTS & (FLUSH_SLOTS - 1)) == 0, "0 or a power of two");
     const size_t start = g * (size_t)stripe;
     if (start < nbytes) {
     const size_t stripe_end = start + stripe;
@@ -67,7 +47,7 @@
     constexpr int kSlots = kRound / 16;
     const int rounds = (int)((my_end - start) / kRound);
     uint4 buf[kSlots];
-    if (rounds > 0) feed_load<FEED_ASM>(buf, src);
+    if (rounds > 0) feed_load(buf, src);
     uint32_t last_word = 0;
     bool ahead = false;
     for (int r = 0; r < rounds; r++) {
@@ -87,15 +67,19 @@
                 eng.consume_dword(st, buf[i].z, res.bits);
                 eng.consume_dword(st, buf[i].w, res.bits);
             }
-            if ((((uint32_t)r * kSlots + (uint32_t)i) & flush_mask) == flush_mask) res.flush();
+            bool together;
+            if constexpr (FLUSH_SLOTS == 0) together = (((uint32_t)r * kSlots + (uint32_t)i) & flush_mask) == flush_mask;
+            else if constexpr (FLUSH_SLOTS >= kSlots) together = i == kSlots - 1 && (r & (FLUSH_SLOTS / kSlots - 1)) == FLUSH_SLOTS / kSlots - 1;
+            else together = (i & (FLUSH_SLOTS - 1)) == FLUSH_SLOTS - 1;
+            if (together) res.flush();
             else if (res.bits >> 15) res.flush();
         }
         if (r + 1 < rounds) {
-            feed_load<FEED_ASM>(buf, src + (r + 1) * kSlots);
+            feed_load(buf, src + (r + 1) * kSlots);
         } else {
             last_word = buf[kSlots - 1].w;
             if (start + (size_t)(rounds + 1) * kRound <= nbytes) {
-                feed_load<FEED_ASM>(buf, src + (r + 1) * kSlots);
+                feed_load(buf, src + (r + 1) * kSlots);
                 ahead = true;
             }
         }
@@ -161,11 +145,19 @@
     }
 }
 
-template <bool ONEPASS, class PhaseHook = NoPhaseHook, int KB = 1, bool CLEAN = ONEPASS>
+__device__ __forceinline__ void settle_shared_word(unsigned long long *slot, uint32_t *word, uint32_t mine) {
+    const unsigned long long old = atomicExch(slot, (1ull << 63) | mine);
+    if (old) {
+        *word = (uint32_t)old | mine;
+        *slot = 0;
+    }
+}
+template <bool ONEPASS, int FLUSH_SLOTS, class PhaseHook = NoPhaseHook, int KB = 1, bool CLEAN = ONEPASS, bool OWN_WORDS = false>
 __device__ __forceinline__ void dfa2_body(const Dfa2Device &prog, const uint8_t *__restrict__ bytes, size_t nbytes, uint32_t stripe,
                                           const uint64_t *__restrict__ stripe_base, uint32_t *__restrict__ accept_bits,
                                           uint32_t *__restrict__ counts, uint32_t *__restrict__ slabs, PhaseHook phase = PhaseHook(),
-                                          uint32_t flush_mask = 31u) {
+                                          uint32_t flush_mask = 31u, unsigned long long *__restrict__ slots = nullptr, uint64_t nwords = 0) {
+    static_assert(!OWN_WORDS || (!ONEPASS && KB == 1), "the exchange slots serve the indexed kernels with one bit per line");
     phase(kPhaseEntry);
     __shared__ __attribute__((aligned(16))) struct {
         uint8_t t2_and_stage[kDfa2RegionBytes];
@@ -184,9 +176,21 @@
     const size_t g0 = (size_t)blockIdx.x * kThreads;
     uint64_t window_word = 0;
     if (!ONEPASS) window_word = (line_of(stripe_base[g0]) * KB) >> 5;
-    dfa2_stripe<ONEPASS, PhaseHook, false, KB, CLEAN>(eng, g0 + threadIdx.x, window_word, stage, stage_words, bytes, nbytes, stripe, stripe_base, accept_bits, counts, slabs,
-                         gridDim.x * kThreads, phase, flush_mask);
-    if (!ONEPASS) {
+    dfa2_stripe<ONEPASS, PhaseHook, FLUSH_SLOTS, KB, CLEAN>(eng, g0 + threadIdx.x, window_word, stage, stage_words, bytes, nbytes, stripe, stripe_base, accept_bits,
+                                                            counts, slabs, gridDim.x * kThreads, phase, flush_mask);
+    if constexpr (OWN_WORDS) {
+        __syncthreads();
+        const bool last = blockIdx.x + 1 == gridDim.x;
+        const uint64_t next_word = last ? nwords : line_of(stripe_base[g0 + kThreads]) >> 5;
+        uint64_t span = next_word - window_word;
+        if (span > stage_words) span = stage_words;
+        for (uint32_t i = threadIdx.x + 1; i < (uint32_t)span; i += kThreads) accept_bits[window_word + i] = stage[i];
+        if (threadIdx.x == 0) {
+            if (blockIdx.x == 0) accept_bits[window_word] = stage[0];
+            else settle_shared_word(&slots[blockIdx.x], &accept_bits[window_word], stage[0]);
+        }
+        if (threadIdx.x == 64 && !last && span < stage_words) settle_shared_word(&slots[blockIdx.x + 1], &accept_bits[next_word], stage[(uint32_t)span]);
+    } else if (!ONEPASS) {
         __syncthreads();
         for (uint32_t i = threadIdx.x; i < stage_words; i += kThreads) {
             const uint32_t v = stage[i];
@@ -195,68 +199,30 @@
     }
     phase(kPhaseWindowOut);
 }
-template <class PhaseHook = NoPhaseHook>
-__device__ __forceinline__ void dfa2_units_body(const Dfa2Device &prog, const uint8_t *__restrict__ bytes, size_t nbytes, uint32_t stripe,
-                                                const uint64_t *__restrict__ stripe_base, uint32_t *__restrict__ accept_bits, uint32_t units_per_wg,
-                                                PhaseHook phase = PhaseHook()) {
-    phase(kPhaseEntry);
-    __shared__ __attribute__((aligned(16))) struct {
-        uint8_t t2_and_stage[kDfa2RegionBytes];
-        uint16_t p[kDfa2PBytes / 2];
-    } lds;
-    Dfa2 eng;
-    eng.load(prog, lds.p, lds.t2_and_stage);
-    const uint32_t stage_off = (uint32_t)((Dfa2::lds_bytes(prog) + 15) & ~(size_t)15);
-    uint32_t *const stage = reinterpret_cast<uint32_t *>(lds.t2_and_stage + stage_off);
-    const uint32_t stage_words = (kDfa2RegionBytes - stage_off) / 4 - 1;
-    uint32_t &next_unit = stage[stage_words];
-    for (uint32_t i = threadIdx.x; i < stage_words; i += kThreads) stage[i] = 0;
-    if (threadIdx.x == 0) next_unit = kThreads / 64;
-    __syncthreads();
-    phase(kPhaseTablesLoaded);
-    const size_t g_wg = (size_t)blockIdx.x * units_per_wg * 64;
-    const uint64_t window_word = line_of(stripe_base[g_wg]) >> 5;
-    uint32_t unit = __builtin_amdgcn_readfirstlane(threadIdx.x >> 6);
-    while (unit < units_per_wg) {
-        uint32_t lane;
-        asm volatile("v_and_b32 %0, 63, %1" : "=v"(lane) : "v"(threadIdx.x));
-        dfa2_stripe<false, PhaseHook, true>(eng, g_wg + (size_t)unit * 64 + lane, window_word, stage, stage_words, bytes, nbytes, stripe, stripe_base, accept_bits,
-                           nullptr, nullptr, 0u, phase);
-        uint32_t ticket = 0;
-        if (__builtin_amdgcn_mbcnt_hi(~0u, __builtin_amdgcn_mbcnt_lo(~0u, 0u)) == 0) ticket = atomicAdd(&next_unit, 1u);
-        unit = __builtin_amdgcn_readfirstlane(ticket);
-    }
-    __syncthreads();
-    for (uint32_t i = threadIdx.x; i < stage_words; i += kThreads) {
-        const uint32_t v = stage[i];
-        if (v) atomicOr(&accept_bits[window_word + i], v);
-    }
-    phase(kPhaseWindowOut);
-}
-__global__ __launch_bounds__(kThreads) __attribute__((amdgpu_waves_per_eu(8, 8))) void match_units2_kernel(
-    Dfa2Device prog, const uint8_t *__restrict__ bytes, size_t nbytes, uint32_t stripe, const uint64_t *__restrict__ stripe_base,
-    uint32_t *__restrict__ accept_bits, uint32_t units_per_wg) {
-    dfa2_units_body(prog, bytes, nbytes, stripe, stripe_base, accept_bits, units_per_wg);
-}
+template <int FLUSH_SLOTS, bool OWN_WORDS>
 __global__ __launch_bounds__(kThreads) void match_stripes2_kernel(Dfa2Device prog, const uint8_t *__restrict__ bytes, size_t nbytes,
                                                                    uint32_t stripe, const uint64_t *__restrict__ stripe_base,
-                                                                   uint32_t *__restrict__ accept_bits, uint32_t flush_mask) {
-    dfa2_body<false>(prog, bytes, nbytes, stripe, stripe_base, accept_bits, nullptr, nullptr, NoPhaseHook(), flush_mask);
-}
+                                                                   uint32_t *__restrict__ accept_bits, uint32_t flush_mask,
+                                                                   unsigned long long *__restrict__ slots, uint64_t nwords) {
+    dfa2_body<false, FLUSH_SLOTS, NoPhaseHook, 1, false, OWN_WORDS>(prog, bytes, nbytes, stripe, stripe_base, accept_bits, nullptr, nullptr, NoPhaseHook(), flush_mask,
+                                                                    slots, nwords);
+}
+template <int FLUSH_SLOTS, bool OWN_WORDS>
 __global__ __launch_bounds__(kThreads) void match_stripes2_clean_kernel(
     Dfa2Device prog, const uint8_t *__restrict__ bytes, size_t nbytes, uint32_t stripe, const uint64_t *__restrict__ stripe_base,
-    uint32_t *__restrict__ accept_bits, uint32_t flush_mask) {
-    dfa2_body<false, NoPhaseHook, 1, true>(prog, bytes, nbytes, stripe, stripe_base, accept_bits, nullptr, nullptr, NoPhaseHook(), flush_mask);
+    uint32_t *__restrict__ accept_bits, uint32_t flush_mask, unsigned long long *__restrict__ slots, uint64_t nwords) {
+    dfa2_body<false, FLUSH_SLOTS, NoPhaseHook, 1, true, OWN_WORDS>(prog, bytes, nbytes, stripe, stripe_base, accept_bits, nullptr, nullptr, NoPhaseHook(), flush_mask,
+                                                                   slots, nwords);
 }
 __global__ __launch_bounds__(kThreads) void match_stripes2_two_bit_kernel(Dfa2Device prog, const uint8_t *__restrict__ bytes, size_t nbytes,
                                                                            uint32_t stripe, const uint64_t *__restrict__ stripe_base,
                                                                            uint32_t *__restrict__ wide_bits) {
-    dfa2_body<false, NoPhaseHook, 2>(prog, bytes, nbytes, stripe, stripe_base, wide_bits, nullptr, nullptr);
+    dfa2_body<false, 32, NoPhaseHook, 2>(prog, bytes, nbytes, stripe, stripe_base, wide_bits, nullptr, nullptr);
 }
 __global__ __launch_bounds__(kThreads) void match_stripes2_onepass_kernel(Dfa2Device prog, const uint8_t *__restrict__ bytes, size_t nbytes,
                                                                            uint32_t stripe, uint32_t *__restrict__ counts,
                                                                            uint32_t *__restrict__ slabs) {
-    dfa2_body<true>(prog, bytes, nbytes, stripe, nullptr, nullptr, counts, slabs);
+    dfa2_body<true, 32>(prog, bytes, nbytes, stripe, nullptr, nullptr, counts, slabs);
 }
 
 constexpr uint32_t kCompactWindowWords = 8192;
@@ -329,13 +295,22 @@
     hipLaunchKernelGGL(kernel, dim3((unsigned)blocks), dim3(kThreads), 0, (hipStream_t)stream, p, bytes, nbytes, stripe, rest...);
     return (int)hipGetLastError();
 }
-int match_stripes_dfa2(const Dfa2Device &p, const uint8_t *bytes, size_t nbytes, uint32_t stripe, const uint64_t *stripe_base,
-                       size_t nstripes, uint32_t *accept, void *stream, uint32_t flush_mask) {
-    return launch_dfa2(match_stripes2_kernel, p, bytes, nbytes, stripe, nstripes, kThreads, stream, stripe_base, accept, flush_mask);
-}
-int match_stripes_dfa2_clean(const Dfa2Device &p, const uint8_t *bytes, size_t nbytes, uint32_t stripe, const uint64_t *stripe_base,
-                             size_t nstripes, uint32_t *accept, void *stream, uint32_t flush_mask) {
-    return launch_dfa2(match_stripes2_clean_kernel, p, bytes, nbytes, stripe, nstripes, kThreads, stream, stripe_base, accept, flush_mask);
+uint32_t dfa2_window_words(const Dfa2Device &p) {
+    const size_t stage_off = (Dfa2::lds_bytes(p) + 15) & ~(size_t)15;
+    return stage_off < kDfa2RegionBytes ? (uint32_t)((kDfa2RegionBytes - stage_off) / 4) : 0u;
+}
+bool dfa2_flush_at_compile_time(uint32_t flush_mask) { return flush_mask == 31u; }
+int match_stripes_dfa2(const Dfa2Device &p, bool clean, const uint8_t *bytes, size_t nbytes, uint32_t stripe, const uint64_t *stripe_base,
+                       size_t nstripes, uint32_t *accept, void *stream, uint32_t flush_mask, unsigned long long *slots, size_t nwords) {
+    const bool fixed = dfa2_flush_at_compile_time(flush_mask);
+#define GO(K) launch_dfa2(K, p, bytes, nbytes, stripe, nstripes, kThreads, stream, stripe_base, accept, flush_mask, slots, (uint64_t)nwords)
+    if (clean) {
+        if (slots) return fixed ? GO((match_stripes2_clean_kernel<32, true>)) : GO((match_stripes2_clean_kernel<0, true>));
+        return fixed ? GO((match_stripes2_clean_kernel<32, false>)) : GO((match_stripes2_clean_kernel<0, false>));
+    }
+    if (slots) return fixed ? GO((match_stripes2_kernel<32, true>)) : GO((match_stripes2_kernel<0, true>));
+    return fixed ? GO((match_stripes2_kernel<32, false>)) : GO((match_stripes2_kernel<0, false>));
+#undef GO
 }
 __global__ __launch_bounds__(256) void split_two_bit_kernel(const uint32_t *__restrict__ wide, size_t words, uint32_t *__restrict__ accept_bits,
                                                              uint32_t *__restrict__ escaped_bits, unsigned long long *__restrict__ escaped_total,
@@ -405,11 +380,6 @@
                        list, cap);
     return (int)hipGetLastError();
 }
-int match_units_dfa2(const Dfa2Device &p, const uint8_t *bytes, size_t nbytes, uint32_t stripe, const uint64_t *stripe_base,
-                     size_t nstripes, uint32_t *accept, uint32_t units_per_wg, void *stream) {
-    if (nstripes && !units_per_wg) return (int)hipErrorInvalidValue;
-    return launch_dfa2(match_units2_kernel, p, bytes, nbytes, stripe, nstripes, (size_t)64 * units_per_wg, stream, stripe_base, accept, units_per_wg);
-}
 int match_onepass_dfa(const LineDfaDevice &p, const uint8_t *bytes, size_t nbytes, uint32_t stripe, size_t nstripes, uint32_t *counts,
                       uint32_t *slabs, void *stream) {
     if (p.in_global) return launch_onepass<LineDfaGlobalEngine, LineDfaDevice>(p, 256, bytes, nbytes, stripe, nstripes, counts, slabs, stream);
```

New measurement: 5662 (median of 6 runs). +1.3%, better.
